# Bostanabad-Research-Group/GP-Plus

Measured on AMD Instinct MI355X. Metric: MLL evals/sec (fwd+grad), NxN exact GP, N=20k d=8, higher is better.
Workload: dtype f64; 1 GPU; C2: synthetic Borehole (Sobol seed 0, unique rows, z-scored) N=20000 d=8 fp64, GP_Plus Rough_RBF exact GP at theta1, one replica per GPU (restart-parallel); N=20000, d=8, streams_per_gpu=1

## Files before the change

### gp-plus_amd/_lib.py

```python
from __future__ import annotations

import ctypes
import os
import subprocess
from ctypes import POINTER, c_char_p, c_double, c_int, c_int32, c_int64, c_size_t, c_void_p
from pathlib import Path

import torch

_PKG_DIR = Path(__file__).resolve().parent
_LIB_PATH = _PKG_DIR / "libgpp_hip.so"
_CSRC = _PKG_DIR / "csrc"

_SIGNATURES = {
    "gpp_version": (c_char_p, []),
    "gpp_create": (c_int, [POINTER(c_void_p), c_int]),
    "gpp_destroy": (c_int, [c_void_p]),
    "gpp_set_stream": (c_int, [c_void_p, c_void_p]),
    "gpp_internal_stream": (c_int, [c_void_p, c_int, POINTER(c_void_p)]),
    "gpp_set_option": (c_int, [c_void_p, c_int, c_int]),
    "gpp_workspace_bytes": (c_size_t, [c_void_p, c_int, c_int64, c_int64, c_int, c_int]),
    "gpp_set_workspace": (c_int, [c_void_p, c_void_p, c_size_t]),
    "gpp_kernel_build": (c_int, [c_void_p, c_void_p, c_int64, c_int, c_void_p, c_void_p, c_void_p, c_void_p, c_int,
                                 c_double, c_int, c_int, c_int, c_void_p, c_int64, c_int64, c_int64]),
    "gpp_cross_kernel": (c_int, [c_void_p, c_void_p, c_int64, c_void_p, c_int64, c_int, c_void_p, c_void_p, c_int,
                                 c_int, c_void_p, c_int64]),
    "gpp_potrf": (c_int, [c_void_p, c_void_p, c_int64, c_int64, c_void_p, c_int64, c_void_p]),
    "gpp_potrf_ws": (c_int, [c_void_p, c_void_p, c_int64, c_int64, c_void_p, c_int64, c_void_p, c_int64, c_void_p]),
    "gpp_trtri": (c_int, [c_void_p, c_void_p, c_int64, c_int64, c_void_p, c_int64, c_void_p, c_int64]),
    "gpp_lauum": (c_int, [c_void_p, c_void_p, c_int64, c_int64, c_void_p, c_int64]),
    "gpp_post_cov_train": (c_int, [c_void_p, c_void_p, c_int64, c_int64, c_void_p, c_void_p, c_int, c_void_p, c_double, c_void_p,
                                   c_int64]),
    "gpp_syrk_rows": (c_int, [c_void_p, c_void_p, c_int64, c_void_p, c_int64, c_int64, c_int64, c_int64, c_int64, c_int, c_int]),
    "gpp_gemm_lower_cols": (c_int, [c_void_p, c_void_p, c_int64, c_void_p, c_int64, c_void_p, c_int64, c_int64, c_int64, c_double,
                                    c_double, c_int64, c_int64, c_int, c_int, c_int64, c_int64, c_int]),
    "gpp_shard_list_begin": (c_int, [c_void_p, c_int64, c_int64, c_int, c_int, c_void_p, c_int64, c_void_p, c_void_p, c_int64, c_void_p,
                                     c_void_p, c_void_p, c_void_p, c_int64, c_void_p, c_int, POINTER(c_int)]),
    "gpp_shard_piece_cols": (c_int64, []),
    "gpp_shard_list_gate": (c_int, [c_void_p, c_void_p, c_int, c_int]),
    "gpp_shard_list_signal": (c_int, [c_void_p, c_void_p, c_int, c_int]),
    "gpp_shard_list_end": (c_int, [c_void_p]),
    "gpp_set_comm": (c_int, [c_void_p, c_void_p, c_int, c_int]),
    "gpp_comm_unique_id": (c_int, [c_void_p]),
    "gpp_comm_init_rccl": (c_int, [c_void_p, c_void_p, c_int, c_int]),
    "gpp_shard_buffer_doubles": (c_size_t, [c_int64, c_int64, c_int, c_int, c_int]),
    "gpp_shard_eval": (c_int, [c_void_p, c_int64, c_int64, c_void_p, c_int, c_void_p, c_void_p, c_void_p, c_void_p, c_int, c_int, c_int,
                               c_double, c_int, c_int, c_void_p, POINTER(c_int)]),
    "gpp_push_create": (c_int, [c_int, c_int, c_int, c_int64, POINTER(c_void_p), c_void_p]),
    "gpp_push_connect": (c_int, [c_void_p, c_void_p]),
    "gpp_push_send": (c_int, [c_void_p, c_void_p, c_int64, c_void_p, c_int, c_int, POINTER(c_void_p), POINTER(c_int64), POINTER(c_int64),
                              POINTER(c_int64), POINTER(c_int64), POINTER(c_int64)]),
    "gpp_push_recv": (c_int, [c_void_p, c_void_p, c_int64, c_void_p, c_int, c_int, POINTER(c_void_p), POINTER(c_int64), POINTER(c_int64),
                              POINTER(c_int64), POINTER(c_int64), POINTER(c_int64)]),
    "gpp_push_ack": (c_int, [c_void_p, c_void_p, c_int64]),
    "gpp_push_info": (c_int, [c_void_p, POINTER(c_int64), POINTER(c_int)]),
    "gpp_push_destroy": (c_int, [c_void_p, c_int]),
    "gpp_shard_back_list": (c_int, [c_void_p, c_int64, c_int64, c_int, c_int, c_void_p, c_int64, c_void_p, c_void_p, c_int64, c_void_p,
                                    c_void_p, c_int, POINTER(c_int)]),
    "gpp_trmv_lower_cols": (c_int, [c_void_p, c_void_p, c_int64, c_int64, c_void_p, c_void_p, c_int64, c_int, c_int, c_int, c_int]),
    "gpp_mll_scalars": (c_int, [c_void_p, c_void_p, c_int64, c_int64, c_void_p, c_void_p]),
    "gpp_grad_reduce_cols": (c_int, [c_void_p, c_void_p, c_int64, c_int, c_void_p, c_void_p, c_void_p, c_int, c_int, c_int,
                                     c_void_p, c_void_p, c_int64, c_int, c_int64, c_int, c_int, c_void_p, c_void_p, c_void_p,
                                     c_void_p, c_int]),
    "gpp_lauum_rows": (c_int, [c_void_p, c_void_p, c_int64, c_int64, c_void_p, c_int64, c_int, c_int]),
    "gpp_lauum_rows_range": (c_int, [c_void_p, c_void_p, c_int64, c_int64, c_void_p, c_int64, c_int, c_int, c_int64, c_int64]),
    "gpp_transpose": (c_int, [c_void_p, c_void_p, c_int64, c_int64, c_int64, c_void_p, c_int64]),
    "gpp_mll_reduce": (c_int, [c_void_p, c_void_p, c_int64, c_void_p, c_int64, c_int64, c_void_p, c_void_p, c_void_p]),
    "gpp_alpha": (c_int, [c_void_p, c_void_p, c_int64, c_int64, c_void_p, c_void_p]),
    "gpp_grad_reduce": (c_int, [c_void_p, c_void_p, c_int64, c_int, c_void_p, c_void_p, c_void_p, c_int, c_int, c_int,
                                c_void_p, c_void_p, c_int64, c_int, c_void_p, c_void_p, c_void_p, c_void_p]),
    "gpp_grad_reduce_rows": (c_int, [c_void_p, c_void_p, c_int64, c_int, c_void_p, c_void_p, c_void_p, c_int, c_int, c_int,
                                     c_void_p, c_void_p, c_int64, c_int, c_int64, c_int, c_int, c_void_p, c_void_p, c_void_p,
                                     c_void_p]),
    "gpp_predict": (c_int, [c_void_p, c_void_p, c_int64, c_int64, c_void_p, c_void_p, c_int64, c_int64, c_void_p,
                            c_void_p, c_int64, c_void_p, c_void_p]),
    "gpp_predict_tn": (c_int, [c_void_p, c_void_p, c_int64, c_int64, c_void_p, c_void_p, c_int64, c_int64, c_void_p,
                               c_void_p, c_int64, c_void_p, c_void_p]),
    "gpp_cross_grad": (c_int, [c_void_p, c_void_p, c_int64, c_void_p, c_int64, c_int, c_void_p, c_void_p, c_int, c_int, c_void_p,
                               c_void_p, c_void_p, c_void_p, c_int64, c_void_p, c_int, c_void_p, c_int, c_void_p, c_void_p]),
    "gpp_gemm": (c_int, [c_void_p, c_int, c_int, c_int64, c_int64, c_int64, c_double, c_void_p, c_int64, c_void_p,
                         c_int64, c_double, c_void_p, c_int64, c_int, c_int, c_int, c_int, c_int]),
    "gpp_gemm_batched": (c_int, [c_void_p, c_int, c_int, c_int64, c_int64, c_int64, c_double, c_void_p, c_int64, c_int64,
                                 c_void_p, c_int64, c_int64, c_double, c_void_p, c_int64, c_int64, c_int, c_int, c_int, c_int,
                                 c_int, c_int]),
    "gpp_kernel_build_batched": (c_int, [c_void_p, c_void_p, c_int64, c_int64, c_int, c_void_p, c_void_p, c_void_p, c_void_p, c_int,
                                         c_double, c_int, c_int, c_int, c_void_p, c_int64, c_int64, c_int]),
    "gpp_potrf_batched": (c_int, [c_void_p, c_void_p, c_int64, c_int64, c_int64, c_void_p, c_int64, c_int64, c_void_p, c_int]),
    "gpp_trtri_batched": (c_int, [c_void_p, c_void_p, c_int64, c_int64, c_int64, c_void_p, c_int64, c_int64, c_void_p, c_int64,
                                  c_int64, c_int]),
    "gpp_lauum_batched": (c_int, [c_void_p, c_void_p, c_int64, c_int64, c_int64, c_void_p, c_int64, c_int64, c_int]),
    "gpp_mll_reduce_batched": (c_int, [c_void_p, c_void_p, c_int64, c_int64, c_void_p, c_int64, c_int64, c_int64, c_void_p,
                                       c_void_p, c_int64, c_void_p, c_int]),
    "gpp_alpha_batched": (c_int, [c_void_p, c_void_p, c_int64, c_int64, c_int64, c_void_p, c_void_p, c_int64, c_int]),
    "gpp_grad_reduce_batched": (c_int, [c_void_p, c_void_p, c_int64, c_int64, c_int, c_void_p, c_void_p, c_void_p, c_int, c_int,
                                        c_int, c_void_p, c_int64, c_void_p, c_int64, c_int64, c_int, c_void_p, c_void_p, c_void_p,
                                        c_void_p, c_int]),
}

_lib = None


class GppError(RuntimeError):
    """A libgpp_hip call returned a non-zero status."""


def build(force: bool = False) -> Path:
    if force:
        subprocess.run(["make", "-C", str(_CSRC), "clean"], check=True, capture_output=True)
    proc = subprocess.run(["make", "-C", str(_CSRC), "-j4"], capture_output=True, text=True)
    if proc.returncode != 0:
        raise RuntimeError("building libgpp_hip.so failed:\n" + proc.stdout + proc.stderr)
    return _LIB_PATH


def load() -> ctypes.CDLL:
    global _lib
    if _lib is not None:
        return _lib
    if not _LIB_PATH.exists():
        raise GppError(
            f"{_LIB_PATH} not found: the HIP extension is required (build it with "
            f"`make -C {_CSRC}` or `python -c 'import __graft_entry__ as g; g.build()'`); there is no CPU fallback."
        )
    lib = ctypes.CDLL(os.fspath(_LIB_PATH))
    for name, (restype, argtypes) in _SIGNATURES.items():
        fn = getattr(lib, name)
        fn.restype = restype
        fn.argtypes = argtypes
    _lib = lib
    return lib


def exported_symbols() -> list:
    return sorted(_SIGNATURES)


def check(status: int, what: str) -> None:
    if status == 0:
        return
    if status < 0:
        raise GppError(f"{what}: bad argument #{-status}")
    raise GppError(f"{what}: HIP runtime error {status - 1000}")
```

### gp-plus_amd/backend.py

```python
from __future__ import annotations

import atexit
import ctypes
import os
import threading
import weakref
from typing import Dict, Optional, Tuple

import torch

from . import _lib, settings
from ._lib import GppError, check

KIND_RBF, KIND_MATERN32, KIND_MATERN52 = 0, 1, 2
UPLO_FULL, UPLO_LOWER, UPLO_UPPER = 0, 1, 2
OPT_COOP_PANEL, OPT_PANEL_FAULT, OPT_PANEL_TIMEOUT_MS, OPT_EXEC_SCHED, OPT_DAG_SCHED = 1, 2, 3, 4, 5
OP_MLL_EVAL, OP_PREDICT, OP_PREDICT_GRAD = 0, 1, 2
MAX_FEATURES = 64


def _check_features(D: int) -> None:
    if D < 1 or D > MAX_FEATURES:
        raise GppError(f"the covariance kernels take 1..{MAX_FEATURES} feature columns per point (got {D})")

_contexts: Dict[Tuple[int, int], "GppContext"] = {}
_contexts_lock = threading.Lock()


def _ptr(t: Optional[torch.Tensor]) -> Optional[int]:
    return None if t is None else t.data_ptr()


def _need(t: torch.Tensor, dtype, name: str) -> None:
    if not t.is_cuda:
        raise GppError(f"{name} must live on the GPU (got {t.device}); libgpp_hip has no CPU path")
    if t.dtype != dtype:
        raise GppError(f"{name} must be {dtype} (got {t.dtype})")
    if not t.is_contiguous() and t.dim() == 1:
        raise GppError(f"{name} must be contiguous")


INFO_PANEL_TIMEOUT = 1 << 30
INFO_EXEC_TIMEOUT = (1 << 30) | (1 << 29)


def check_status(info: int) -> None:
    if info >= INFO_PANEL_TIMEOUT:
        what = "an executor launch" if info & (1 << 29) else "the cooperative panel kernel"
        raise GppError(f"gpp_potrf: {what} timed out waiting for one of its work-groups (another kernel holding the stream's CUs "
                       "for seconds, or a caller-supplied CU-masked stream with fewer CUs than the launch assumed); "
                       "GPP_COOP_PANEL=0 selects the leaf-step factorisation, GPP_DAG_SCHED=0 the launch-per-product one")


def panel_timed_out(ctx: "GppContext", info: int) -> bool:
    if info < INFO_PANEL_TIMEOUT:
        return False
    import warnings

    ms = info & 0xFFFFF
    if info & (1 << 29):
        if not ctx.dag_sched:
            check_status(info)
        warnings.warn(f"libgpp_hip: an executor launch timed out after {ms} ms (another tenant of this GPU held part of its CUs, or "
                      "dispatches are serialised); this context now factors with one launch per product", RuntimeWarning)
        ctx.set_option(OPT_DAG_SCHED, 0)
        return True
    if not ctx.coop_panel:
        check_status(info)
    warnings.warn(f"libgpp_hip: a cooperative panel launch timed out after {ms} ms (another tenant of this GPU held part "
                  "of its CUs); this context now factors with leaf-step launches", RuntimeWarning)
    ctx.set_option(OPT_COOP_PANEL, 0)
    return True


def square_buffer(n: int, device) -> torch.Tensor:
    ld = max(16, (n + 15) // 16 * 16)
    return torch.empty((n, ld), dtype=torch.float64, device=device)[:, :n]


def _ld(m: torch.Tensor) -> int:
    if m.dim() != 2 or m.stride(1) != 1:
        raise GppError("matrix must be 2-D with unit column stride")
    return m.stride(0) if m.shape[0] > 1 else max(m.shape[1], m.stride(0))


def _on_own_device(fn):
    import functools

    @functools.wraps(fn)
    def wrapper(self, *args, **kwargs):
        if torch.cuda.current_device() == self.index:
            return fn(self, *args, **kwargs)
        with torch.cuda.device(self.index):
            return fn(self, *args, **kwargs)

    return wrapper


class GppContext:
    def __init__(self, device: torch.device):
        if device.type != "cuda":
            raise GppError("GppContext needs a cuda (HIP) device; there is no CPU fallback")
        if not torch.cuda.is_available():
            raise GppError("no GPU visible to PyTorch: the HIP path cannot run")
        self.lib = _lib.load()
        self.device = device
        self.index = device.index if device.index is not None else torch.cuda.current_device()
        h = ctypes.c_void_p()
        with torch.cuda.device(self.index):
            check(self.lib.gpp_create(ctypes.byref(h), self.index), "gpp_create")
        self.h = h
        self.coop_panel = settings.ENV_COOP_PANEL
        self.dag_sched = settings.ENV_DAG_SCHED
        if any(os.environ.get(v, "0") not in ("", "0") for v in ("HIP_LAUNCH_BLOCKING", "AMD_SERIALIZE_KERNEL", "CUDA_LAUNCH_BLOCKING")):
            self.set_option(OPT_DAG_SCHED, 0)
        self._ws: Optional[torch.Tensor] = None

    def _stream(self) -> None:
        s = torch.cuda.current_stream(self.index).cuda_stream
        check(self.lib.gpp_set_stream(self.h, ctypes.c_void_p(s)), "gpp_set_stream")

    def set_option(self, option: int, value: int) -> None:
        check(self.lib.gpp_set_option(self.h, int(option), int(value)), "gpp_set_option")
        if option == OPT_COOP_PANEL:
            self.coop_panel = bool(value)
        elif option in (OPT_DAG_SCHED, OPT_EXEC_SCHED):
            self.dag_sched = bool(value)

    @_on_own_device
    def internal_streams(self):
        if getattr(self, "_istreams", None) is None:
            out = []
            for which in (0, 1, 2):
                p = ctypes.c_void_p()
                check(self.lib.gpp_internal_stream(self.h, which, ctypes.byref(p)), "gpp_internal_stream")
                out.append(torch.cuda.ExternalStream(p.value, device=self.device))
            self._istreams = tuple(out)
        return self._istreams

    @_on_own_device
    def ensure_workspace(self, op: int, N: int, M: int, D: int, S: int) -> None:
        need = int(self.lib.gpp_workspace_bytes(self.h, op, N, M, D, S))
        if self._ws is None or self._ws.numel() < need:
            self._ws = torch.empty(need, dtype=torch.uint8, device=self.device)
            check(self.lib.gpp_set_workspace(self.h, self._ws.data_ptr(), self._ws.numel()), "gpp_set_workspace")

    def _check_groups(self, grp: torch.Tensor, N: int, S: int) -> None:
        _need(grp, torch.int32, "grp")
        if grp.numel() != N:
            raise GppError(f"noise-group index has {grp.numel()} entries for {N} points (stale fidel_indices?)")
        seen = getattr(self, "_grp_ok", None)
        if seen is None or seen[0]() is not grp or seen[1:] != (grp._version, N, S):
            lo, hi = int(grp.min()), int(grp.max())
            if lo < 0 or hi >= max(S, 1):
                raise GppError(f"noise-group index out of range: values in [{lo}, {hi}] for {S} noise levels")
            self._grp_ok = (weakref.ref(grp), grp._version, N, S)

    @_on_own_device
    def kernel_build(self, U, w, sf2, tau, grp, out, *, jitter=0.0, kind=KIND_RBF, d_split=0, uplo=UPLO_FULL,
                     row0=0, nrows=None):
        N, D = U.shape
        _check_features(D)
        for t, n in ((U, "U"), (w, "w"), (sf2, "sf2"), (out, "Ky")):
            _need(t, torch.float64, n)
        if tau is not None:
            _need(tau, torch.float64, "tau")
        S = 0 if tau is None else tau.numel()
        if grp is not None:
            self._check_groups(grp, N, S)
        if not U.is_contiguous():
            raise GppError("U must be contiguous")
        self._stream()
        check(self.lib.gpp_kernel_build(self.h, U.data_ptr(), N, D, w.data_ptr(), sf2.data_ptr(), _ptr(tau), _ptr(grp), S,
                                        float(jitter), kind, d_split, uplo, out.data_ptr(), _ld(out), row0,
                                        N - row0 if nrows is None else nrows), "gpp_kernel_build")
        return out

    @_on_own_device
    def cross_kernel(self, Ua, Ub, w, sf2, out, *, kind=KIND_RBF, d_split=0):
        _check_features(Ua.shape[1])
        for t, n in ((Ua, "Ua"), (Ub, "Ub"), (w, "w"), (sf2, "sf2"), (out, "Kab")):
            _need(t, torch.float64, n)
        if not (Ua.is_contiguous() and Ub.is_contiguous()):
            raise GppError("Ua/Ub must be contiguous")
        self._stream()
        check(self.lib.gpp_cross_kernel(self.h, Ua.data_ptr(), Ua.shape[0], Ub.data_ptr(), Ub.shape[0], Ua.shape[1],
                                        w.data_ptr(), sf2.data_ptr(), kind, d_split, out.data_ptr(), _ld(out)),
              "gpp_cross_kernel")
        return out

    @_on_own_device
    def potrf(self, A, Linv, info, T=None):
        _need(A, torch.float64, "A"); _need(Linv, torch.float64, "Linv"); _need(info, torch.int32, "info")
        self._stream()
        if T is None:
            check(self.lib.gpp_potrf(self.h, A.data_ptr(), A.shape[0], _ld(A), Linv.data_ptr(), _ld(Linv), info.data_ptr()),
                  "gpp_potrf")
        else:
            check(self.lib.gpp_potrf_ws(self.h, A.data_ptr(), A.shape[0], _ld(A), Linv.data_ptr(), _ld(Linv), T.data_ptr(),
                                        _ld(T), info.data_ptr()), "gpp_potrf_ws")

    @_on_own_device
    def trtri(self, U, Linv, T):
        self._stream()
        check(self.lib.gpp_trtri(self.h, U.data_ptr(), U.shape[0], _ld(U), Linv.data_ptr(), _ld(Linv), T.data_ptr(), _ld(T)),
              "gpp_trtri")

    @_on_own_device
    def lauum(self, Linv, Kinv):
        self._stream()
        check(self.lib.gpp_lauum(self.h, Linv.data_ptr(), Linv.shape[0], _ld(Linv), Kinv.data_ptr(), _ld(Kinv)), "gpp_lauum")

    @_on_own_device
    def post_cov_train(self, Kinv, tau, grp, d, out, *, jitter=0.0):
        N = Kinv.shape[0]
        for t, n in ((Kinv, "Kinv"), (tau, "tau"), (out, "A")):
            _need(t, torch.float64, n)
        if d is not None:
            _need(d, torch.float64, "d")
            if d.numel() != N or not d.is_contiguous():
                raise GppError(f"d must be a contiguous vector of {N} doubles")
        if grp is not None:
            self._check_groups(grp, N, tau.numel())
        if out.shape[0] != N or out.shape[1] != N:
            raise GppError("post_cov_train: shapes do not match")
        self._stream()
        check(self.lib.gpp_post_cov_train(self.h, Kinv.data_ptr(), N, _ld(Kinv), tau.data_ptr(), _ptr(grp), tau.numel(), _ptr(d),
                                          float(jitter), out.data_ptr(), _ld(out)), "gpp_post_cov_train")
        return out

    @_on_own_device
    def syrk_rows(self, Urow, C, nb, first_block, rank, nranks):
        self._stream()
        check(self.lib.gpp_syrk_rows(self.h, Urow.data_ptr(), _ld(Urow), C.data_ptr(), _ld(C), C.shape[0], Urow.shape[0], nb,
                                     first_block, rank, nranks), "gpp_syrk_rows")

    @_on_own_device
    def shard_list_begin(self, N, nb, rank, nranks, A, Kc, Lc, D, W, info, workers=0) -> bool:
        self._stream()
        used = ctypes.c_int(0)
        check(self.lib.gpp_shard_list_begin(self.h, N, nb, rank, nranks, A.data_ptr(), _ld(A), Kc.data_ptr(), Lc.data_ptr(), _ld(Kc),
                                            D.data_ptr(), W[0].data_ptr(), W[1].data_ptr(), W[2].data_ptr(), _ld(W[0]),
                                            info.data_ptr(), int(workers), ctypes.byref(used)), "gpp_shard_list_begin")
        return bool(used.value)

    def shard_messages(self, N: int, nb: int, k: int):
        o, o2 = k * nb, min((k + 2) * nb, N)
        W = int(self.lib.gpp_shard_piece_cols()) or N
        return [(o, o2)] + [(c, min(c + W, N)) for c in range(o2, N, W)]

    @_on_own_device
    def shard_list_gate(self, stream, tail: int, k: int) -> None:
        check(self.lib.gpp_shard_list_gate(self.h, ctypes.c_void_p(stream.cuda_stream), int(tail), k), "gpp_shard_list_gate")

    @_on_own_device
    def shard_list_signal(self, stream, tail: int, k: int) -> None:
        check(self.lib.gpp_shard_list_signal(self.h, ctypes.c_void_p(stream.cuda_stream), int(tail), k), "gpp_shard_list_signal")

    @_on_own_device
    def shard_list_end(self) -> None:
        self._stream()
        check(self.lib.gpp_shard_list_end(self.h), "gpp_shard_list_end")

    @_on_own_device
    def shard_back_list(self, N, nb, rank, nranks, A, Kc, Lc, D, info, workers=0) -> bool:
        self._stream()
        used = ctypes.c_int(0)
        check(self.lib.gpp_shard_back_list(self.h, N, nb, rank, nranks, A.data_ptr(), _ld(A), Kc.data_ptr(), Lc.data_ptr(), _ld(Kc),
                                           D.data_ptr(), info.data_ptr(), int(workers), ctypes.byref(used)), "gpp_shard_back_list")
        return bool(used.value)

    @_on_own_device
    def gemm_lower_cols(self, A, B, C, alpha, beta, nb, first_block, rank, nranks, row0=0, row1=None, compact=False):
        M, K = A.shape[1], A.shape[0]
        if compact:
            if B.shape[0] != K or C.shape[0] != M:
                raise GppError("gemm_lower_cols: shapes do not match")
        elif A.shape != B.shape or C.shape[0] != C.shape[1] or C.shape[0] != M:
            raise GppError("gemm_lower_cols: shapes do not match")
        self._stream()
        check(self.lib.gpp_gemm_lower_cols(self.h, A.data_ptr(), _ld(A), B.data_ptr(), _ld(B), C.data_ptr(), _ld(C), M,
                                           K, float(alpha), float(beta), nb, first_block, rank, nranks, row0,
                                           M if row1 is None else row1, 1 if compact else 0),
              "gpp_gemm_lower_cols")

    @_on_own_device
    def trmv_lower_cols(self, T, x, y, nb, rank, nranks, trans=False, compact=False):
        for t, n in ((x, "x"), (y, "y")):
            _need(t, torch.float64, n)
        if trans:
            self.ensure_workspace(OP_MLL_EVAL, T.shape[0], 0, 1, 1)
        self._stream()
        check(self.lib.gpp_trmv_lower_cols(self.h, T.data_ptr(), _ld(T), T.shape[0], x.data_ptr(), y.data_ptr(), nb, rank, nranks,
                                           1 if trans else 0, 1 if compact else 0), "gpp_trmv_lower_cols")

    @_on_own_device
    def mll_scalars(self, U, z, out3):
        self._stream()
        check(self.lib.gpp_mll_scalars(self.h, U.data_ptr(), _ld(U), U.shape[0], z.data_ptr(), out3.data_ptr()), "gpp_mll_scalars")

    @_on_own_device
    def lauum_rows(self, Linv, Kinv, rank, nranks):
        self._stream()
        check(self.lib.gpp_lauum_rows(self.h, Linv.data_ptr(), Linv.shape[0], _ld(Linv), Kinv.data_ptr(), _ld(Kinv), rank, nranks),
              "gpp_lauum_rows")

    @_on_own_device
    def lauum_rows_range(self, Linv, Kinv, rank, nranks, row0, row1):
        self._stream()
        check(self.lib.gpp_lauum_rows_range(self.h, Linv.data_ptr(), Linv.shape[0], _ld(Linv), Kinv.data_ptr(), _ld(Kinv), rank,
                                            nranks, row0, row1), "gpp_lauum_rows_range")

    @_on_own_device
    def transpose(self, src, dst):
        if src.shape[0] != dst.shape[1] or src.shape[1] != dst.shape[0]:
            raise GppError("transpose: shapes do not match")
        self._stream()
        check(self.lib.gpp_transpose(self.h, src.data_ptr(), src.stride(0), src.shape[0], src.shape[1], dst.data_ptr(), dst.stride(0)),
              "gpp_transpose")

    @_on_own_device
    def mll_reduce(self, L, Linv, r, z, out3):
        for t, n in ((r, "r"), (z, "z"), (out3, "out3")):
            _need(t, torch.float64, n)
        self._stream()
        check(self.lib.gpp_mll_reduce(self.h, L.data_ptr(), _ld(L), Linv.data_ptr(), _ld(Linv), L.shape[0], r.data_ptr(),
                                      z.data_ptr(), out3.data_ptr()), "gpp_mll_reduce")

    @_on_own_device
    def alpha(self, Linv, z, alpha):
        N = Linv.shape[0]
        self._stream()
        check(self.lib.gpp_alpha(self.h, Linv.data_ptr(), _ld(Linv), N, z.data_ptr(), alpha.data_ptr()), "gpp_alpha")

    @_on_own_device
    def grad_reduce(self, U, w, sf2, grp, S, alpha, Kinv, dU, g_w, g_sf2, g_tau, g_U, *, kind=KIND_RBF, d_split=0):
        N, D = U.shape
        if grp is not None:
            self._check_groups(grp, N, S)
        self.ensure_workspace(OP_MLL_EVAL, N, 0, D, S)
        self._stream()
        check(self.lib.gpp_grad_reduce(self.h, U.data_ptr(), N, D, w.data_ptr(), sf2.data_ptr(), _ptr(grp), S, kind,
                                       d_split, alpha.data_ptr(), Kinv.data_ptr(), _ld(Kinv), dU, g_w.data_ptr(),
                                       g_sf2.data_ptr(), g_tau.data_ptr(), _ptr(g_U)), "gpp_grad_reduce")

    @_on_own_device
    def grad_reduce_rows(self, U, w, sf2, grp, S, alpha, Kinv, dU, nb, rank, nranks, g_w, g_sf2, g_tau, g_U, *,
                         kind=KIND_RBF, d_split=0):
        N, D = U.shape
        if grp is not None:
            self._check_groups(grp, N, S)
        self.ensure_workspace(OP_MLL_EVAL, N, 0, D, S)
        self._stream()
        check(self.lib.gpp_grad_reduce_rows(self.h, U.data_ptr(), N, D, w.data_ptr(), sf2.data_ptr(), _ptr(grp), S, kind,
                                            d_split, alpha.data_ptr(), Kinv.data_ptr(), _ld(Kinv), dU, nb, rank, nranks,
                                            g_w.data_ptr(), g_sf2.data_ptr(), g_tau.data_ptr(), _ptr(g_U)),
              "gpp_grad_reduce_rows")

    @_on_own_device
    def grad_reduce_cols(self, U, w, sf2, grp, S, alpha, Kinv, dU, nb, rank, nranks, g_w, g_sf2, g_tau, g_U, *,
                         kind=KIND_RBF, d_split=0, compact=False):
        N, D = U.shape
        if grp is not None:
            self._check_groups(grp, N, S)
# ... 167 lines not shown
```

### gp-plus_amd/csrc/gpp_api.hip

```cpp
#include "../../include/gpp.h"
#include "gpp_internal.h"

#include <algorithm>
#include <cmath>
#include <cstdio>
#include <cstdlib>
#include <cstring>
#include <new>

const GppEnv& gpp_env() {
  static const GppEnv env = [] {
    auto num = [](const char* name, long long unset) { const char* v = getenv(name); return v ? atoll(v) : unset; };
    GppEnv e;
    e.coop_panel = num("GPP_COOP_PANEL", 1) != 0;
    e.dag_sched = num("GPP_DAG_SCHED", 1) != 0;
    e.dag_phased = num("GPP_DAG_PHASED", 0) != 0;
    e.shard_list = num("GPP_SHARD_LIST", 1) != 0;
    e.shard_workers = (int)num("GPP_SHARD_WORKERS", 0);
    e.shard_fill = (int)num("GPP_SHARD_FILL", -1);
    e.shard_timeout_ms = num("GPP_SHARD_TIMEOUT_MS", 60000);
    const int64_t cols = num("GPP_SHARD_PIECE_COLS", 8192);
    e.shard_piece_cols = cols <= 0 ? (int64_t)0 : std::max<int64_t>(GPP_TILE, cols / GPP_TILE * GPP_TILE);
    e.sharded_force_collectives = num("GPP_SHARDED_FORCE_COLLECTIVES", 0) != 0;
    e.exec_verbose = getenv("GPP_EXEC_VERBOSE") != nullptr;
// ... 313 lines not shown
      HIP_TRY(hipStreamWaitEvent(cf, R_prev, 0));
      const int64_t t128 = ((nb + 127) / 128) * ((o + 127) / 128);
      HIP_TRY(trtri_level(cf, cm.A, cm.ld, cm.Li, cm.ldi, T, ldt, 0, o + nb, o, [](int64_t) { return false; }, 1, 0, 0, 0,
                          t128 < 640 ? 64 : 0, D));
    }
    if (rem == 0) {
      if (be_wait) HIP_TRY(hipStreamWaitEvent(cu.s, be_wait, 0));
      break;
    }
    const int64_t nb2 = std::min(bh, rem), rest = rem - nb2;
    auto row_solve = [&](int64_t c0, int64_t nc) -> hipError_t {
      if (!T) return trsm_rec(cu, c0, nc, o, nb);
      GemmArgs gt = mk(cm.Li + o * cm.ldi + o, cm.ldi, cm.A + o * cm.ld + c0, cm.ld, T + o * ldt + c0, ldt, nb, nc, nb, 1.0,
                       0.0);
      gt.a_mask = 1; gt.khi_mode = 1;
      gt.row_reverse = 1;
      HIP_TRY(gpp_launch_gemm(cu.s, 2, gt, 1));
      return hipMemcpy2DAsync(cm.A + o * cm.ld + c0, cm.ld * sizeof(double), T + o * ldt + c0, ldt * sizeof(double),
                              nc * sizeof(double), nb, hipMemcpyDeviceToDevice, cu.s);
    };
    const double* Urow = cm.A + o * cm.ld;
    HIP_TRY(row_solve(o + nb, nb2));
    GemmArgs g = mk(Urow + (o + nb), cm.ld, Urow + (o + nb), cm.ld, cm.A + (o + nb) * cm.ld + (o + nb), cm.ld, nb2, nb2, nb,
                    -1.0, 1.0);
    g.c_lower = 2;
    HIP_TRY(gpp_launch_gemm(cu.s, 2, g, 1));
    hipEvent_t S = next_event(h);
    HIP_TRY(hipEventRecord(S, cu.s));
    if (rest > 0) HIP_TRY(row_solve(o + nb + nb2, rest));
    hipEvent_t R = nullptr;
    if (border) {
      R = next_event(h);
      HIP_TRY(hipEventRecord(R, cu.s));
    }
    const bool merge_upd = nb2 % NBLK == 0;
    if (rest > 0 && !merge_upd) {
      GemmArgs g2 = mk(Urow + (o + nb), cm.ld, Urow + (o + nb + nb2), cm.ld, cm.A + (o + nb) * cm.ld + (o + nb + nb2), cm.ld,
                       nb2, rest, nb, -1.0, 1.0);
      HIP_TRY(gpp_launch_gemm(cu.s, 2, g2, 1));
    }
    HIP_TRY(hipStreamWaitEvent(cp.s, S, 0));
    if (be_wait) {
      HIP_TRY(hipStreamWaitEvent(cu.s, be_wait, 0));
      be_wait = nullptr;
    }
    if (rest > 0 && merge_upd) {
      GemmArgs g3 = mk(Urow + (o + nb), cm.ld, Urow + (o + nb), cm.ld, cm.A + (o + nb) * cm.ld + (o + nb), cm.ld, rem, rem, nb,
                       -1.0, 1.0);
      g3.c_lower = 2;
      g3.skip_lead = (int)nb2;
      int64_t rA = ((SPLIT_ELEMS / rem + NBLK - 1) / NBLK) * NBLK;
      rA = std::max(rA, nb2);
      if (split_upd && rem - rA >= 2048) {
        pend.rows_ready = next_event(h);
        HIP_TRY(hipEventRecord(pend.rows_ready, cu.s));
        GemmArgs a2 = mk(Urow + (o + nb), cm.ld, Urow + (o + nb + rA), cm.ld, cm.A + (o + nb) * cm.ld + (o + nb + rA), cm.ld,
                         rA, rem - rA, nb, -1.0, 1.0);
        HIP_TRY(gpp_launch_gemm(cu.s, 2, a2, 1, NBLK, NBLK));
        GemmArgs a1 = g3;
        a1.M = a1.N = (int)rA;
        HIP_TRY(hipStreamWaitEvent(cf, pend.rows_ready, 0));
        HIP_TRY(gpp_launch_gemm(cf, 2, a1, 1, NBLK, NBLK));
        hipEvent_t A1 = next_event(h);
        HIP_TRY(hipEventRecord(A1, cf));
        HIP_TRY(hipStreamWaitEvent(cu.s, A1, 0));
        pend.g = mk(Urow + (o + nb + rA), cm.ld, Urow + (o + nb + rA), cm.ld, cm.A + (o + nb + rA) * cm.ld + (o + nb + rA),
                    cm.ld, rem - rA, rem - rA, nb, -1.0, 1.0);
        pend.g.c_lower = 2;
        pend.rows_masked = rA;
        pend.on = true;
      } else {
        HIP_TRY(gpp_launch_gemm(cu.s, 2, g3, 1, NBLK, NBLK));
      }
    } else if (rest > 0) {
      GemmArgs g3 = mk(Urow + (o + nb + nb2), cm.ld, Urow + (o + nb + nb2), cm.ld,
                       cm.A + (o + nb + nb2) * cm.ld + (o + nb + nb2), cm.ld, rest, rest, nb, -1.0, 1.0);
      g3.c_lower = 2;
      HIP_TRY(gpp_launch_gemm(cu.s, 2, g3, 1));
    }
    R_prev = R;
  }
  if (pend.on) return hipErrorUnknown;
  hipEvent_t E = next_event(h);
  HIP_TRY(hipEventRecord(E, cu.s));
  HIP_TRY(hipStreamWaitEvent(cm.s, E, 0));
  if (border) {
    hipEvent_t F = next_event(h);
    HIP_TRY(hipEventRecord(F, cf));
    HIP_TRY(hipStreamWaitEvent(cm.s, F, 0));
    h->inv_nblocks = 1;
    h->inv_o[0] = 0;
    h->inv_n[0] = N;
  }
  return hipSuccess;
}

void dag_note_inverted(gpp_handle_s* h, const DagPlan* P, int64_t N) {
  h->inv_nblocks = 0;
  if (P->inv_rows > 0) {
    h->inv_o[0] = 0;
    h->inv_n[0] = std::min(P->inv_rows, N);
    h->inv_nblocks = 1;
  }
  for (int b = 0; b < P->B && h->inv_nblocks < 128; ++b) {
    const int64_t o = (int64_t)P->tb[b] * NBLK, rows = std::min<int64_t>((int64_t)P->tb[b + 1] * NBLK, N) - o;
    if (o < P->inv_rows) continue;
    h->inv_o[h->inv_nblocks] = o;
    h->inv_n[h->inv_nblocks] = rows;
    ++h->inv_nblocks;
  }
}

hipError_t dag_abort(gpp_handle_s* h, const DagPlan* P) {
  if (!h->full_stream || !P || !P->d_counters) return hipErrorInvalidValue;
  HIP_TRY(gpp_launch_fill_i32(h->full_stream, P->d_counters, 1, 1));
  return hipStreamSynchronize(h->full_stream);
}

inline int dag_fuse(int64_t N) { return N >= 14336 ? 4 : N >= 11264 ? 2 : 1; }

struct PlanKey {
  int64_t N, nb, ld, ldi, ldt;
  int flags;
  int64_t inv_rows;
  int rank, nranks, workers;
};
template <typename Make>
DagPlan* dag_plan_cached(gpp_handle_s* h, const PlanKey& k, Make make) {
  DagPlan* P = nullptr;
  int lru = 0;
  for (int i = 0; i < GPP_DAG_PLANS; ++i) {
    DagPlan* q = h->dag_plans[i];
    if (q && q->N == k.N && q->nb == k.nb && q->ld == k.ld && q->ldi == k.ldi && q->ldt == k.ldt && q->flags == k.flags &&
        q->inv_rows == k.inv_rows && q->rank == k.rank && q->nranks == k.nranks && q->workers == k.workers)
      P = q;
    if (!q) lru = i;
    else if (h->dag_plans[lru] && q->stamp < h->dag_plans[lru]->stamp) lru = i;
  }
  if (!P) {
    P = make();
    if (!P) return nullptr;
    if (h->dag_plans[lru]) gpp_dag_free(h->dag_plans[lru]);
    h->dag_plans[lru] = P;
  }
  P->stamp = ++h->dag_clock;
  return P;
}

constexpr int64_t DAG_MIN_N = 6912;
constexpr int64_t DAG_MAX_N = 65536;
constexpr int64_t DAG_INV_MAX_N = 19456;
constexpr int64_t DAG_NB = 1024;

hipError_t potrf_dag(gpp_handle_s* h, const Ctx& cm, int64_t N, double* T, int64_t ldt, bool* used) {
  *used = false;
  if (!gpp_env().dag_sched || !h->dag_sched || !h->coop_panel || !T || N < DAG_MIN_N || N > DAG_MAX_N) return hipSuccess;
  HIP_TRY(ensure_streams(h));
  if (h->cu_split != 1) return hipSuccess;
  const int64_t nb = DAG_NB;
  if (!panel_fits(h, nb) || !panel_fits(h, nb + 256)) return hipSuccess;
  int64_t inv_rows = N;
  if (N > DAG_INV_MAX_N) {
    inv_rows = 0;
    for (int64_t r = 2 * nb; r <= (int64_t)(0.42 * (double)N); r *= 2) inv_rows = r;
  }
  const int flags = inv_rows > 0 ? DAG_INV : 0;
  DagPlan* P = dag_plan_cached(h, PlanKey{N, nb, cm.ld, cm.ldi, ldt, flags, inv_rows, 0, 1, 0}, [&]() -> DagPlan* {
    DagTuning tune = gpp_dag_default_tuning();
    tune.workers = 2 * (h->ncu - h->panel_cus);
    tune.fill = 2 * h->panel_cus;
    tune.inv_rows = inv_rows;
    tune.fuse = dag_fuse(N);
    DagPlan* Q = gpp_dag_plan(N, nb, cm.ld, cm.ldi, ldt, 0, flags, tune);
    if (!Q) return nullptr;
    for (int b = 0; b < Q->B; ++b) {
      const int64_t rows = std::min<int64_t>((int64_t)Q->tb[b + 1] * NBLK, N) - (int64_t)Q->tb[b] * NBLK;
      if (!panel_fits(h, rows)) {
        gpp_dag_free(Q);
        return nullptr;
      }
    }
    if (gpp_dag_upload(Q) != hipSuccess) {
      (void)hipGetLastError();
      gpp_dag_free(Q);
      h->dag_sched = 0;
      return nullptr;
    }
    return Q;
  });
  if (!P) return hipSuccess;
  Ctx cp = cm, cu = cm;
  cp.s = h->panel_stream;
  cu.s = h->upd_stream;
  HIP_TRY(gpp_launch_fill_i32(cm.s, P->d_counters, P->ncounters, 0));
  DagBases bases{{reinterpret_cast<char*>(cm.A), reinterpret_cast<char*>(cm.Li), reinterpret_cast<char*>(T), nullptr}};
  HIP_TRY(gpp_launch_dag_bind(cm.s, P->d_groups, P->d_groups_abs, (int)P->groups.size(), bases));
  hipEvent_t ev = next_event(h);
  HIP_TRY(hipEventRecord(ev, cm.s));
  HIP_TRY(hipStreamWaitEvent(cp.s, ev, 0));
  HIP_TRY(hipStreamWaitEvent(cu.s, ev, 0));
  const long long budget = (long long)(h->panel_timeout_ms > 0 ? h->panel_timeout_ms : 500) * 100000 * 4;
  DagLaunch dl{};
  dl.groups = P->d_groups_abs; dl.tasks = P->d_tasks; dl.ntasks = (int)P->tasks.size();
  dl.counters = P->d_counters; dl.info = cm.info; dl.budget = budget;
  dl.max_tasks = 0; dl.quit_id = -1; dl.quit_val = 0; dl.ticket_limit = 0;
  dl.trace = P->d_trace; dl.tag = 0;
  if (gpp_env().dag_phased) {
    const int wgs = 2 * h->ncu;
    for (int b = 0; b < P->B; ++b) {
      const int64_t o = (int64_t)P->tb[b] * NBLK, rows = std::min<int64_t>((int64_t)P->tb[b + 1] * NBLK, N) - o;
      HIP_TRY(launch_panel(h, cm, o, rows, std::min(64, h->ncu)));
      HIP_TRY(gpp_launch_exec_signal(cm.s, P->d_counters, P->c_pd + b));
      DagLaunch pl = dl;
      pl.ticket_limit = b + 1 < P->B ? P->level_first[b + 1] : 0;
      pl.tag = b;
      if (b + 1 == P->B || pl.ticket_limit > 0) HIP_TRY(gpp_launch_dag(cm.s, wgs, pl));
    }
    HIP_TRY(hipEventRecord(P->last_use, cm.s));
    dag_note_inverted(h, P, N);
    *used = true;
    return hipSuccess;
  }
  HIP_TRY(gpp_launch_dag(cu.s, 2 * (h->ncu - h->panel_cus), dl));
  auto enqueue_panel_stream = [&]() -> hipError_t {
    for (const DagPlan::Op& op : P->stream_ops) {
      const int64_t o = op.kind < 3 ? (int64_t)P->tb[op.arg] * NBLK : 0;
      if (op.kind == 0) {
        HIP_TRY(gpp_launch_exec_gate(cp.s, P->d_counters, P->c_g1d + op.arg, P->gate_target[op.arg], cm.info, budget));
      } else if (op.kind == 1) {
        const int64_t rows = std::min<int64_t>((int64_t)P->tb[op.arg + 1] * NBLK, N) - o;
        HIP_TRY(launch_panel(h, cp, o, rows, h->panel_cus));
      } else if (op.kind == 2) {
        HIP_TRY(gpp_launch_exec_signal(cp.s, P->d_counters, P->c_pd + op.arg));
      } else {
        DagLaunch fl = dl;
        fl.max_tasks = op.arg;
        fl.quit_id = op.n >= 0 ? P->c_g1d + op.n : -1;
        fl.quit_val = 1;
        fl.ticket_limit = op.lim;
        fl.tag = op.n >= 0 ? op.n : P->B;
        HIP_TRY(gpp_launch_dag(cp.s, 2 * h->panel_cus, fl));
      }
    }
    return hipSuccess;
  };
  const hipError_t perr = enqueue_panel_stream();
  if (perr != hipSuccess) {
    (void)hipGetLastError();
    (void)dag_abort(h, P);
  }
  hipEvent_t E = next_event(h), F = next_event(h);
  HIP_TRY(hipEventRecord(E, cu.s));
  HIP_TRY(hipEventRecord(F, cp.s));
  HIP_TRY(hipStreamWaitEvent(cm.s, E, 0));
  HIP_TRY(hipStreamWaitEvent(cm.s, F, 0));
  HIP_TRY(hipEventRecord(P->last_use, cm.s));
  if (perr != hipSuccess) return perr;
  dag_note_inverted(h, P, N);
  *used = true;
  return hipSuccess;
}

inline int64_t owned_cols(int64_t N, int64_t nb, int rank, int nranks) {
  const int64_t nblk = (N + nb - 1) / nb;
  int64_t cols = 0;
  for (int64_t b = rank; b < nblk; b += nranks) cols += std::min(nb, N - b * nb);
  return cols;
}

int check_mat(const void* p, int64_t ld, int64_t n, int argi) {
  if (!p) return -argi;
  if (!aligned16(p) || (ld & 1) || ld < n) return -(argi + 1);
  return 0;
}

}

extern "C" {

#ifndef GPP_SRC_HASH
#define GPP_SRC_HASH "unknown"
#endif
const char* gpp_version(void) { return "gpp_hip 0.3 (gfx950, fp64 MFMA) src " GPP_SRC_HASH; }

#ifdef GPP_PANEL_STAMP
int gpp_debug_panel_flags(gpp_handle_t h, int* out, int nints, int* next_slot) {
  if (next_slot) *next_slot = h->panel_next % GPP_PANEL_RING;
  return (int)hipMemcpy(out, h->panel_flags, (size_t)nints * sizeof(int), hipMemcpyDeviceToHost);
}
#endif

static DagPlan* dag_mru(gpp_handle_t h) {
  DagPlan* P = nullptr;
  if (h)
    for (int i = 0; i < GPP_DAG_PLANS; ++i)
      if (h->dag_plans[i] && (!P || h->dag_plans[i]->stamp > P->stamp)) P = h->dag_plans[i];
  return P;
}
int gpp_debug_dag_info(gpp_handle_t h, int64_t* info8) {
  const DagPlan* P = dag_mru(h);
  if (!P) return -1;
  info8[8] = P->inv_rows;
  info8[9] = P->N;
  info8[0] = (int64_t)P->tasks.size(); info8[1] = (int64_t)P->groups.size(); info8[2] = P->B; info8[3] = P->nt;
  info8[4] = P->ncounters; info8[5] = (int64_t)(P->sim_ms * 1000.0); info8[6] = (int64_t)(P->sim_busy * 1000.0); info8[7] = P->flags;
  return 0;
}
int gpp_debug_dag_counters(gpp_handle_t h, int* out, int nmax) {
  DagPlan* P = dag_mru(h);
  if (!P || !P->d_counters) return -1;
  if (hipDeviceSynchronize() != hipSuccess) return 1;
  std::vector<int> c(P->ncounters);
  if (hipMemcpy(c.data(), P->d_counters, c.size() * sizeof(int), hipMemcpyDeviceToHost) != hipSuccess) return 2;
  int n = 0;
  auto put = [&](int v) { if (n < nmax) out[n++] = v; };
  put(c[0]); put(c[1]); put(P->B);
  for (int b = 0; b < P->B; ++b) put(c[P->c_pd + b]);
  for (int b = 0; b < P->B; ++b) put(c[P->c_g1d + b]);
  if (P->flags & DAG_SHARD) {
    for (int b = 0; b < P->B; ++b) put(c[P->c_cph + b]);
    for (int b = 0; b < P->B; ++b) put(c[P->c_cpt + b * P->GP]);
    for (int b = 0; b < P->B; ++b) put(c[P->c_art + b * P->GP]);
  }
  return n;
}
int gpp_debug_dag_trace(gpp_handle_t h, int on) {
  DagPlan* P = dag_mru(h);
  if (!P) return -1;
  if (hipDeviceSynchronize() != hipSuccess) return 1;
  if (on && !P->d_trace) {
    if (hipMalloc(&P->d_trace, 4 * P->tasks.size() * sizeof(unsigned long long)) != hipSuccess) return 2;
    (void)hipMemset(P->d_trace, 0, 4 * P->tasks.size() * sizeof(unsigned long long));
  } else if (!on && P->d_trace) {
    (void)hipFree(P->d_trace);
    P->d_trace = nullptr;
  }
  return 0;
}
int gpp_debug_dag_fetch(gpp_handle_t h, void* tasks, void* trace) {
  const DagPlan* P = dag_mru(h);
  if (!P) return -1;
  if (hipDeviceSynchronize() != hipSuccess) return 1;
  if (tasks) memcpy(tasks, P->tasks.data(), P->tasks.size() * sizeof(DagTask));
  if (trace) {
    if (!P->d_trace) return 2;
    if (hipMemcpy(trace, P->d_trace, 4 * P->tasks.size() * sizeof(unsigned long long), hipMemcpyDeviceToHost) != hipSuccess) return 3;
  }
  return 0;
}

int gpp_create(gpp_handle_t* out, int device) {
  if (!out) return -1;
  int ndev = 0;
  hipError_t e = hipGetDeviceCount(&ndev);
  if (e != hipSuccess) return rc(e);
  if (device < 0 || device >= ndev) return -2;
  e = hipSetDevice(device);
  if (e != hipSuccess) return rc(e);
  gpp_handle_s* h = new (std::nothrow) gpp_handle_s();
  if (!h) return rc(hipErrorOutOfMemory);
  h->device = device;
  h->stream = nullptr;
  h->ws = nullptr;
  h->ws_bytes = 0;
  h->panel_stream = nullptr;
  h->upd_stream = nullptr;
  h->fill_stream = nullptr;
  h->full_stream = nullptr;
  h->cu_split = -1;
  h->panel_cus = 0;
  h->n_events = 0;
  h->ev_next = 0;
  h->inv_N = 0;
  h->inv_nblocks = 0;
  h->panel_flags = nullptr;
  h->panel_next = 0;
  h->coop_panel = gpp_env().coop_panel ? 1 : 0;
  h->panel_fault = 0;
  h->panel_timeout_ms = 500;
  for (int i = 0; i < GPP_DAG_PLANS; ++i) h->dag_plans[i] = nullptr;
  h->shard_cur = nullptr;
  h->shard_info = nullptr;
  h->shard_ready = nullptr;
  h->dag_clock = 0;
  h->dag_sched = 1;
  h->ncu = 0;
  if (hipDeviceGetAttribute(&h->ncu, hipDeviceAttributeMultiprocessorCount, device) != hipSuccess || h->ncu < 2) {
    (void)hipGetLastError();
    h->ncu = 0;
  }
  h->cap_next = 0;
  h->handoff = nullptr;
  if (hipMalloc(reinterpret_cast<void**>(&h->panel_flags), (GPP_PANEL_RING + GPP_PANEL_CAP_RING) * gpp_panel_flag_bytes()) != hipSuccess ||
      hipMemset(h->panel_flags, 0, (GPP_PANEL_RING + GPP_PANEL_CAP_RING) * gpp_panel_flag_bytes()) != hipSuccess) {
    (void)hipGetLastError();
    if (h->panel_flags) (void)hipFree(h->panel_flags);
    h->panel_flags = nullptr;
  }
  *out = h;
  return 0;
}

int gpp_destroy(gpp_handle_t h) {
  if (!h) return -1;
  for (hipStream_t s : {h->panel_stream, h->upd_stream, h->fill_stream, h->full_stream})
    if (s) (void)hipStreamSynchronize(s);
  if (h->full_stream) (void)hipStreamDestroy(h->full_stream);
  if (h->fill_stream) (void)hipStreamDestroy(h->fill_stream);
  if (h->upd_stream) (void)hipStreamDestroy(h->upd_stream);
  if (h->panel_stream) (void)hipStreamDestroy(h->panel_stream);
  for (int i = 0; i < h->n_events; ++i) (void)hipEventDestroy(h->events[i]);
  if (h->handoff) (void)hipEventDestroy(h->handoff);
  if (h->shard_ready) (void)hipEventDestroy(h->shard_ready);
  if (h->panel_flags) (void)hipFree(h->panel_flags);
  for (int i = 0; i < GPP_DAG_PLANS; ++i)
    if (h->dag_plans[i]) gpp_dag_free(h->dag_plans[i]);
  gpp_shard_release_comm(h);
  delete h;
  return 0;
}

int gpp_set_stream(gpp_handle_t h, void* stream) {
  if (!h) return -1;
  hipStream_t s = reinterpret_cast<hipStream_t>(stream);
  if (s != h->stream) {
    hipStreamCaptureStatus a = hipStreamCaptureStatusNone, b = hipStreamCaptureStatusNone;
    if (hipStreamIsCapturing(h->stream, &a) != hipSuccess || hipStreamIsCapturing(s, &b) != hipSuccess) {
      (void)hipGetLastError();
      a = b = hipStreamCaptureStatusActive;
    }
    auto internal = [&](hipStream_t q) { return q && (q == h->panel_stream || q == h->upd_stream || q == h->fill_stream || q == h->full_stream); };
    if (a == hipStreamCaptureStatusNone && b == hipStreamCaptureStatusNone && !internal(s) && !internal(h->stream)) {
      if (!h->handoff) GPP_TRY(hipEventCreateWithFlags(&h->handoff, hipEventDisableTiming));
      GPP_TRY(hipEventRecord(h->handoff, h->stream));
      GPP_TRY(hipStreamWaitEvent(s, h->handoff, 0));
    }
    h->stream = s;
  }
  return 0;
}

int gpp_set_option(gpp_handle_t h, int option, int value) {
  if (!h) return -1;
  if (option == GPP_OPT_COOP_PANEL) h->coop_panel = value ? 1 : 0;
  else if (option == GPP_OPT_PANEL_FAULT) h->panel_fault = value ? 1 : 0;
  else if (option == GPP_OPT_DAG_SCHED || option == GPP_OPT_EXEC_SCHED) h->dag_sched = value ? 1 : 0;
  else if (option == GPP_OPT_PANEL_TIMEOUT_MS) {
    if (value < 1 || value > 60000) return -3;
    h->panel_timeout_ms = value;
  } else return -2;
  return 0;
// ... 61 lines not shown
  hipStream_t sm = h->stream, sp = h->panel_stream, su = h->upd_stream;
  GPP_TRY(gpp_launch_fill_i32(sm, P->d_counters, P->ncounters, 0));
  DagBases bases{{reinterpret_cast<char*>(A), reinterpret_cast<char*>(Kc), reinterpret_cast<char*>(Lc), reinterpret_cast<char*>(D),
                  reinterpret_cast<char*>(W0), reinterpret_cast<char*>(W1), reinterpret_cast<char*>(W2), nullptr}};
  GPP_TRY(gpp_launch_dag_bind(sm, P->d_groups, P->d_groups_abs, (int)P->groups.size(), bases));
  if (!h->shard_ready) GPP_TRY(hipEventCreateWithFlags(&h->shard_ready, hipEventDisableTiming));
  hipEvent_t ev = h->shard_ready;
  GPP_TRY(hipEventRecord(ev, sm));
  GPP_TRY(hipStreamWaitEvent(sp, ev, 0));
  GPP_TRY(hipStreamWaitEvent(su, ev, 0));
  const long long budget = shard_budget(h);
  DagLaunch dl{};
  dl.groups = P->d_groups_abs; dl.tasks = P->d_tasks; dl.ntasks = (int)P->tasks.size();
  dl.counters = P->d_counters; dl.info = info; dl.budget = budget;
  dl.max_tasks = 0; dl.quit_id = -1; dl.quit_val = 0; dl.ticket_limit = 0;
  dl.trace = P->d_trace; dl.tag = 0;
  if (dl.ntasks > 0) GPP_TRY(gpp_launch_dag(su, nworkers, dl));
  Ctx cp{sp, A, ld, D, nb, info};
  auto enqueue_panel_stream = [&]() -> int {
    for (const DagPlan::Op& op : P->stream_ops) {
      const int b = op.arg;
      const int64_t o = (int64_t)b * nb, rows = std::min(nb, N - o);
      if (op.kind == 0) {
        GPP_TRY(gpp_launch_exec_gate(sp, P->d_counters, P->c_g1d + b, P->gate_target[b], info, budget));
      } else if (op.kind == 1) {
        Ctx cb = cp;
        cb.A = A + o * ld + o;
        cb.Li = D + (int64_t)b * nb * nb;
        GPP_TRY(launch_panel_at(h, cb, o, rows, h->panel_cus));
      } else if (op.kind == 2) {
        GPP_TRY(gpp_launch_exec_signal(sp, P->d_counters, P->c_pd + b));
      } else {
        DagLaunch fl = dl;
        fl.max_tasks = op.arg;
        fl.quit_id = op.n >= 0 ? P->c_g1d + op.n : -1;
        fl.quit_val = 1;
        fl.ticket_limit = op.lim;
        fl.tag = op.n >= 0 ? op.n : P->B;
        GPP_TRY(gpp_launch_dag(sp, std::max(P->fill, 1), fl));
      }
    }
    return 0;
  };
  const int erc = enqueue_panel_stream();
  h->shard_cur = P;
  h->shard_info = info;
  if (erc != 0) {
    (void)hipGetLastError();
    (void)dag_abort(h, P);
    return erc;
  }
  *used = 1;
  return 0;
}

static int shard_pieces(const DagPlan* P, int k) {
  const int hi = P->tb[std::min(k + 2, P->B)];
  return hi >= P->nt ? 0 : (P->nt - hi + P->piece_tiles - 1) / P->piece_tiles;
}
int gpp_shard_list_gate(gpp_handle_t h, void* stream, int tail, int k) {
  if (!h || !h->shard_cur) return -1;
  const DagPlan* P = h->shard_cur;
  if (k < 0 || k >= P->B || k % P->nranks != P->rank) return -4;
  if (tail < 0 || tail > shard_pieces(P, k)) return -3;
  hipStream_t s = reinterpret_cast<hipStream_t>(stream);
  const long long budget = shard_budget(h);
  GPP_TRY(hipStreamWaitEvent(s, h->shard_ready, 0));
  GPP_TRY(gpp_launch_exec_gate(s, P->d_counters, P->c_pd + k, 1, h->shard_info, budget));
  const int piece = k * P->GP + tail - 1;
  const int target = tail ? P->cpt_target[piece] : P->cph_target[k];
  if (target > 0) GPP_TRY(gpp_launch_exec_gate(s, P->d_counters, tail ? P->c_cpt + piece : P->c_cph + k, target, h->shard_info, budget));
  return 0;
}

int gpp_shard_list_signal(gpp_handle_t h, void* stream, int tail, int k) {
  if (!h || !h->shard_cur) return -1;
  const DagPlan* P = h->shard_cur;
  if (k < 0 || k >= P->B || k % P->nranks == P->rank) return -4;
  if (tail < 0 || tail > shard_pieces(P, k)) return -3;
  GPP_TRY(hipStreamWaitEvent(reinterpret_cast<hipStream_t>(stream), h->shard_ready, 0));
  return rc(gpp_launch_exec_signal(reinterpret_cast<hipStream_t>(stream), P->d_counters, tail ? P->c_art + k * P->GP + tail - 1 : P->c_pd + k));
}

int gpp_shard_list_end(gpp_handle_t h) {
  if (!h || !h->shard_cur) return -1;
  DagPlan* P = h->shard_cur;
  h->shard_cur = nullptr;
  hipEvent_t E = next_event(h), F = next_event(h);
  GPP_TRY(hipEventRecord(E, h->upd_stream));
  GPP_TRY(hipEventRecord(F, h->panel_stream));
  GPP_TRY(hipStreamWaitEvent(h->stream, E, 0));
  GPP_TRY(hipStreamWaitEvent(h->stream, F, 0));
  GPP_TRY(hipEventRecord(P->last_use, h->stream));
  return 0;
}

int gpp_shard_back_list(gpp_handle_t h, int64_t N, int64_t nb, int rank, int nranks, const double* A, int64_t ld, double* Kc, double* Lc,
                        int64_t ldc, const double* D, int32_t* info, int workers, int* used) {
  if (!h) return -1;
  if (!used) return -14;
  *used = 0;
  if (N < 2 || nb < 128 || nb % 128 != 0) return -2;
  if (rank < 0 || nranks < 1 || rank >= nranks) return -4;
  if (int e = check_mat(A, ld, N, 6)) return e;
  if (!Kc || !aligned16(Kc)) return -8;
  if (!Lc || !aligned16(Lc)) return -9;
  const int64_t wc = ((N + nb - 1) / nb - rank + nranks - 1) / nranks * nb;
  if ((ldc & 1) || ldc < wc) return -10;
  if (!D || !aligned16(D)) return -11;
  if (!info) return -12;
  const GppEnv& env = gpp_env();
  if (!env.shard_list || !h->dag_sched || N < SHARD_LIST_MIN_N || N > DAG_MAX_N || h->shard_cur) return 0;
  if (workers <= 0 && env.shard_workers > 0) workers = 2 * env.shard_workers;
  GPP_TRY(ensure_streams(h));
  const int flags = DAG_SHARD | DAG_BACK;
  const int nworkers = workers > 0 ? workers : 2 * h->ncu;
  DagPlan* P = dag_plan_cached(h, PlanKey{N, nb, ld, ldc, ld, flags, 0, rank, nranks, workers}, [&]() -> DagPlan* {
    DagTuning tune = gpp_dag_default_tuning();
    tune.workers = nworkers;
    tune.fill = 0;
    tune.inv_rows = 0;
    tune.fuse = dag_fuse(N);
    DagPlan* Q = gpp_dag_plan(N, nb, ld, ldc, ld, 0, flags, tune, rank, nranks);
    if (!Q) return nullptr;
    Q->workers = workers;
    if (Q->tasks.empty() || gpp_dag_upload(Q) != hipSuccess) {
      (void)hipGetLastError();
      gpp_dag_free(Q);
      return nullptr;
    }
    return Q;
  });
  if (!P) return 0;
  hipStream_t sm = h->stream;
  GPP_TRY(gpp_launch_fill_i32(sm, P->d_counters, P->ncounters, 0));
  DagBases bases{{const_cast<char*>(reinterpret_cast<const char*>(A)), reinterpret_cast<char*>(Kc), reinterpret_cast<char*>(Lc),
                  const_cast<char*>(reinterpret_cast<const char*>(D)), nullptr, nullptr, nullptr, nullptr}};
  GPP_TRY(gpp_launch_dag_bind(sm, P->d_groups, P->d_groups_abs, (int)P->groups.size(), bases));
  DagLaunch dl{};
  dl.groups = P->d_groups_abs; dl.tasks = P->d_tasks; dl.ntasks = (int)P->tasks.size();
  dl.counters = P->d_counters; dl.info = info;
  dl.budget = shard_budget(h);
  dl.max_tasks = 0; dl.quit_id = -1; dl.quit_val = 0; dl.ticket_limit = 0;
  dl.trace = P->d_trace; dl.tag = 0;
  GPP_TRY(gpp_launch_dag(sm, nworkers, dl));
  GPP_TRY(hipEventRecord(P->last_use, sm));
  *used = 1;
  return 0;
}

size_t gpp_workspace_bytes(gpp_handle_t h, int op, int64_t N, int64_t M, int D, int S) {
  (void)h;
  if (op == GPP_OP_MLL_EVAL) {
    return std::max(gpp_grad_ws_bytes(N, D, S, D), gpp_trmv_t_ws_bytes(N)) + 256;
  }
  if (op == GPP_OP_PREDICT) return 256;
  if (op == GPP_OP_PREDICT_GRAD) return gpp_pgrad_ws_bytes(M, N, D, D, S) + 256;
  return 0;
}

int gpp_set_workspace(gpp_handle_t h, void* ws, size_t bytes) {
  if (!h) return -1;
  if (ws && !aligned16(ws)) return -2;
  h->ws = ws;
  h->ws_bytes = bytes;
  return 0;
}

int gpp_kernel_build(gpp_handle_t h, const double* U, int64_t N, int D, const double* w, const double* sf2,
                     const double* tau, const int32_t* grp, int S, double jitter, int kind, int d_split, int uplo,
                     double* Ky, int64_t ld, int64_t row0, int64_t nrows) {
  if (!h) return -1;
  if (!U) return -2;
  if (N < 0) return -3;
  if (D < 1 || D > 64) return -4;
  if (!w) return -5;
  if (!sf2) return -6;
  if (tau && S < 1) return -9;
  if (kind < 0 || kind > 2) return -11;
  if (d_split < 0 || d_split > D) return -12;
  if (uplo != GPP_UPLO_FULL && uplo != GPP_UPLO_LOWER && uplo != GPP_UPLO_UPPER) return -13;
  if (!Ky) return -14;
  if (ld < N) return -15;
  if (row0 < 0 || nrows < 0 || row0 + nrows > N || (row0 % 64) != 0) return -16;
  if (uplo == GPP_UPLO_UPPER && (row0 != 0 || nrows != N)) return -16;
  GPP_TRY(gpp_launch_kernel_build(h->stream, U, N, D, w, sf2, tau, grp, S, jitter, kind, d_split, uplo, Ky, ld, row0, nrows));
  return 0;
}

int gpp_cross_kernel(gpp_handle_t h, const double* Ua, int64_t Ma, const double* Ub, int64_t Nb, int D, const double* w,
                     const double* sf2, int kind, int d_split, double* Kab, int64_t ld) {
  if (!h) return -1;
  if (!Ua) return -2;
  if (Ma < 0) return -3;
  if (!Ub) return -4;
  if (Nb < 0) return -5;
  if (D < 1 || D > 64) return -6;
  if (!w) return -7;
  if (!sf2) return -8;
  if (kind < 0 || kind > 2) return -9;
  if (d_split < 0 || d_split > D) return -10;
  if (!Kab) return -11;
  if (ld < Nb) return -12;
  GPP_TRY(gpp_launch_cross_kernel(h->stream, Ua, Ma, Ub, Nb, D, w, sf2, kind, d_split, Kab, ld));
  return 0;
}

int gpp_potrf_ws(gpp_handle_t h, double* A, int64_t N, int64_t ld, double* Linv, int64_t ldi, double* T, int64_t ldt,
                 int32_t* info_dev) {
  if (!h) return -1;
  if (N < 0) return -3;
  if (int r = check_mat(A, ld, N, 2)) return r;
  if (int r = check_mat(Linv, ldi, N, 5)) return r;
  if (T) {
    if (int r = check_mat(T, ldt, N, 7)) return r;
  }
  if (!info_dev) return -9;
  GPP_TRY(gpp_launch_fill_i32(h->stream, info_dev, 1, 0));
  Ctx c{h->stream, A, ld, Linv, ldi, info_dev};
  h->inv_N = N;
  h->inv_nblocks = 0;
  const int64_t la_min = T ? BORDER_MIN_N : 6 * LOOKAHEAD_NB;
  bool dag_used = false;
  GPP_TRY(potrf_dag(h, c, N, T, ldt, &dag_used));
  if (dag_used) return 0;
  if (N >= la_min) {
    GPP_TRY(potrf_lookahead(h, c, N, LOOKAHEAD_NB, T, ldt));
  } else if (panel_fits(h, N)) {
    int wgs = h->ncu;
    if (h->cu_split == 1 && h->stream == h->panel_stream) wgs = h->panel_cus;
    else if (h->cu_split == 1 && (h->stream == h->upd_stream || h->stream == h->fill_stream)) wgs = h->ncu - h->panel_cus;
    else if (h->stream) {
      uint32_t mask[32] = {0};
      if (hipExtStreamGetCUMask(h->stream, 32, mask) == hipSuccess) {
        int cus = 0;
        for (int c = 0; c < h->ncu && c < 1024; ++c) cus += (mask[c >> 5] >> (c & 31)) & 1u;
        if (cus >= 2 && cus < wgs) wgs = cus;
      } else {
        (void)hipGetLastError();
      }
    }
    GPP_TRY(launch_panel(h, c, 0, N, wgs));
    h->inv_nblocks = 1;
    h->inv_o[0] = 0;
    h->inv_n[0] = N;
  } else {
    GPP_TRY(potrf_rec(c, 0, N));
  }
  return 0;
}

int gpp_potrf(gpp_handle_t h, double* A, int64_t N, int64_t ld, double* Linv, int64_t ldi, int32_t* info_dev) {
  const int r = gpp_potrf_ws(h, A, N, ld, Linv, ldi, nullptr, 0, info_dev);
  return r == -9 ? -7 : r;
}

int gpp_trtri(gpp_handle_t h, const double* U, int64_t N, int64_t ld, double* Linv, int64_t ldi, double* T, int64_t ldt) {
  if (!h) return -1;
  if (N < 0) return -3;
  if (int r = check_mat(U, ld, N, 2)) return r;
  if (int r = check_mat(Linv, ldi, N, 5)) return r;
  if (int r = check_mat(T, ldt, N, 7)) return r;
  const bool have = (h->inv_N == N && h->inv_nblocks > 0);
  for (int64_t s = NBLK; s < N; s *= 2) {
    auto skip = [&](int64_t b) {
      if (!have) return false;
      for (int i = 0; i < h->inv_nblocks; ++i)
        if (b >= h->inv_o[i] && b + 2 * s <= h->inv_o[i] + h->inv_n[i]) return true;
      for (int i = 0; i < h->inv_nblocks; ++i)
        if (b >= h->inv_o[i] && h->inv_o[i] + h->inv_n[i] == N && b + s < N) return true;
      return false;
    };
    GPP_TRY(trtri_level(h->stream, U, ld, Linv, ldi, T, ldt, 0, N, s, skip));
  }
  h->inv_N = 0;
  return 0;
}

int gpp_lauum(gpp_handle_t h, const double* Linv, int64_t N, int64_t ldi, double* Kinv, int64_t ldk) {
  if (!h) return -1;
  if (N < 0) return -3;
  if (int r = check_mat(Linv, ldi, N, 2)) return r;
  if (int r = check_mat(Kinv, ldk, N, 5)) return r;
  GemmArgs g = mk(Linv, ldi, Linv, ldi, Kinv, ldk, N, N, N, 1.0, 0.0);
  g.a_mask = 2; g.b_mask = 2; g.klo_mode = 3; g.c_lower = 1; g.tag = 1;
  const int t = N <= 2560 ? 32 : N <= 5120 ? 64 : NBLK;
  GPP_TRY(gpp_launch_gemm(h->stream, 2, g, 1, t, t));
  return 0;
}

int gpp_post_cov_train(gpp_handle_t h, const double* Kinv, int64_t N, int64_t ldk, const double* tau, const int32_t* grp, int S,
                       const double* d, double jitter, double* A, int64_t lda) {
  if (!h) return -1;
  if (N < 0) return -3;
  if (int r = check_mat(Kinv, ldk, N, 2)) return r;
  if (!tau) return -5;
  if (S < 1) return -7;
  if (int r = check_mat(A, lda, N, 10)) return r;
  if (A == Kinv && lda != ldk) return -11;
  GPP_TRY(gpp_launch_post_cov_train(h->stream, Kinv, ldk, N, tau, grp, d, jitter, A, lda));
  return 0;
}

int gpp_lauum_rows(gpp_handle_t h, const double* Linv, int64_t N, int64_t ldi, double* Kinv, int64_t ldk, int rank, int nranks) {
  if (!h) return -1;
  if (N < 0) return -3;
  if (int r = check_mat(Linv, ldi, N, 2)) return r;
  if (int r = check_mat(Kinv, ldk, N, 5)) return r;
  if (nranks < 1 || rank < 0 || rank >= nranks) return -7;
  GemmArgs g = mk(Linv, ldi, Linv, ldi, Kinv, ldk, N, N, N, 1.0, 0.0);
  g.a_mask = 2; g.b_mask = 2; g.klo_mode = 3; g.c_lower = 1; g.tag = 1;
  g.row_mod = nranks; g.row_off = rank;
  GPP_TRY(gpp_launch_gemm(h->stream, 2, g, 1, NBLK, NBLK));
  return 0;
}

int gpp_lauum_rows_range(gpp_handle_t h, const double* Linv, int64_t N, int64_t ldi, double* Kinv, int64_t ldk, int rank,
                         int nranks, int64_t row0, int64_t row1) {
  if (!h) return -1;
  if (N < 0) return -3;
  if (int r = check_mat(Linv, ldi, N, 2)) return r;
  if (int r = check_mat(Kinv, ldk, N, 5)) return r;
  if (nranks < 1 || rank < 0 || rank >= nranks) return -7;
  if (row0 < 0 || row1 < row0 || row1 > N || (row0 % NBLK) != 0) return -9;
  if (row1 == row0) return 0;
  GemmArgs g = mk(Linv, ldi, Linv, ldi, Kinv, ldk, N, N, N, 1.0, 0.0);
  g.a_mask = 2; g.b_mask = 2; g.klo_mode = 3; g.c_lower = 1; g.tag = 1;
  g.row_mod = nranks; g.row_off = rank;
  const int64_t t0 = row0 / NBLK, t1 = (row1 + NBLK - 1) / NBLK;
  auto first_i = [&](int64_t t) { return t <= rank ? (int64_t)0 : (t - rank + nranks - 1) / nranks; };
  g.row_i0 = (int)first_i(t0);
  g.row_i1 = (int)first_i(t1);
  if (g.row_i1 <= g.row_i0) return 0;
  GPP_TRY(gpp_launch_gemm(h->stream, 2, g, 1, NBLK, NBLK));
  return 0;
}

int gpp_transpose(gpp_handle_t h, const double* src, int64_t lds, int64_t rows, int64_t cols, double* dst, int64_t ldd) {
  if (!h) return -1;
  if (!src || lds < cols) return -2;
  if (rows < 0 || cols < 0) return -4;
  if (!dst || ldd < rows) return -6;
  GPP_TRY(gpp_launch_transpose(h->stream, src, lds, rows, cols, dst, ldd));
  return 0;
}

int gpp_syrk_rows(gpp_handle_t h, const double* Urow, int64_t ldu, double* C, int64_t ldc, int64_t Nt, int64_t K, int64_t nb,
                  int64_t first_block, int rank, int nranks) {
  if (!h) return -1;
  if (!Urow || !aligned16(Urow) || (ldu & 1)) return -2;
  if (!C || !aligned16(C) || (ldc & 1)) return -4;
  if (Nt < 0 || K < 0) return -6;
  if (nb < NBLK || nb % NBLK != 0) return -8;
  if (first_block < 0) return -9;
  if (nranks < 1 || rank < 0 || rank >= nranks) return -10;
  if (Nt == 0 || K == 0) return 0;
  GemmArgs g = mk(Urow, ldu, Urow, ldu, C, ldc, Nt, Nt, K, -1.0, 1.0);
  g.c_lower = 2;
  g.own_mod = nranks;
  g.own_bt = (int)(nb / NBLK);
  g.own_off = (int)(((first_block - rank) % nranks + nranks) % nranks);
  GPP_TRY(gpp_launch_gemm(h->stream, 2, g, 1, NBLK, NBLK));
  return 0;
}

int gpp_gemm_lower_cols(gpp_handle_t h, const double* A, int64_t lda, const double* B, int64_t ldb, double* C, int64_t ldc,
                        int64_t M, int64_t K, double alpha, double beta, int64_t nb, int64_t first_block, int rank, int nranks,
                        int64_t row0, int64_t row1, int compact) {
  if (!h) return -1;
  if (!A || !aligned16(A) || (lda & 1)) return -2;
  if (!B || !aligned16(B) || (ldb & 1)) return -4;
  if (!C || !aligned16(C) || (ldc & 1)) return -6;
  if (M < 0 || K < 0) return -8;
  if (nb < NBLK || nb % NBLK != 0) return -12;
  if (first_block < 0) return -13;
  if (nranks < 1 || rank < 0 || rank >= nranks) return -14;
  if (row0 < 0 || row1 < row0 || row1 > M || row0 % NBLK != 0) return -16;
  if (M == 0 || K == 0 || row1 == row0) return 0;
  GemmArgs g = mk(A, lda, B, ldb, C, ldc, M, M, K, alpha, beta);
  g.c_lower = 1;
  g.row_t0 = (int)(row0 / NBLK);
  g.row_t1 = (int)((row1 + NBLK - 1) / NBLK);
  g.own_mod = nranks;
  g.own_bt = (int)(nb / NBLK);
  g.own_off = (int)(((first_block - rank) % nranks + nranks) % nranks);
  g.compact_bc = compact ? 1 : 0;
  GPP_TRY(gpp_launch_gemm(h->stream, 2, g, 1, NBLK, NBLK));
  return 0;
}

int gpp_trmv_lower_cols(gpp_handle_t h, const double* T, int64_t ldt, int64_t N, const double* x, double* y, int64_t nb, int rank,
                        int nranks, int trans, int compact) {
  if (!h) return -1;
  if (N < 0) return -4;
  if (int q = check_mat(T, ldt, compact ? std::min<int64_t>(N, ldt) : N, 2)) return q;
  if (!x || !aligned16(x)) return -5;
  if (!y) return -6;
  if (nb < 64 || nb % 64 != 0) return -7;
  if (nranks < 1 || rank < 0 || rank >= nranks) return -8;
  if (trans != 0 && trans != 1) return -10;
  if (trans && (!h->ws || h->ws_bytes < gpp_trmv_t_ws_bytes(N))) return -1;
  if (compact && nranks >= 1 && rank >= 0 && ldt < owned_cols(N, nb, rank, nranks)) return -3;
  GPP_TRY(gpp_launch_trmv_lower_cols(h->stream, T, ldt, N, x, y, nb, rank, nranks, trans, h->ws, h->ws_bytes, compact));
  return 0;
}

int gpp_mll_scalars(gpp_handle_t h, const double* U, int64_t ld, int64_t N, const double* z, double* out3) {
  if (!h) return -1;
  if (N < 0) return -4;
  if (int q = check_mat(U, ld, N, 2)) return q;
  if (!z) return -5;
  if (!out3) return -6;
  GPP_TRY(gpp_launch_mll_scalars(h->stream, U, ld, N, z, out3));
  return 0;
}

int gpp_mll_reduce(gpp_handle_t h, const double* U, int64_t ld, const double* Linv, int64_t ldi, int64_t N,
                   const double* r, double* z, double* out3) {
  if (!h) return -1;
  if (N < 0) return -6;
  if (int q = check_mat(U, ld, N, 2)) return q;
  if (int q = check_mat(Linv, ldi, N, 4)) return q;
  if (!r || !aligned16(r)) return -7;
  if (!z) return -8;
  if (!out3) return -9;
  GPP_TRY(gpp_launch_trmv_lower(h->stream, Linv, ldi, N, r, z));
  GPP_TRY(gpp_launch_mll_scalars(h->stream, U, ld, N, z, out3));
  return 0;
}

int gpp_alpha(gpp_handle_t h, const double* Linv, int64_t ldi, int64_t N, const double* z, double* alpha) {
  if (!h) return -1;
  if (N < 0) return -4;
  if (int q = check_mat(Linv, ldi, N, 2)) return q;
  if (!z || !aligned16(z)) return -5;
  if (!alpha) return -6;
  GPP_TRY(gpp_launch_trmv_upper(h->stream, Linv, ldi, N, z, alpha));
  return 0;
}

// ... 320 lines not shown
```

### gp-plus_amd/csrc/gpp_build.hip

```cpp
#include "gpp_internal.h"

#include <atomic>

namespace {

constexpr int TB = 64;
constexpr int DMAX = 64;

__device__ __forceinline__ double kfun(double r2_rbf, double r2_mat, int kind, const GppExpConsts& ec) {
  double v = gpp_exp_nonpos(-r2_rbf, ec);
  if (kind == 1) {
    const double r = sqrt(3.0 * 2.0 * r2_mat);
    v *= (1.0 + r) * gpp_exp_nonpos(-r, ec);
  } else if (kind == 2) {
    const double r = sqrt(5.0 * 2.0 * r2_mat);
    v *= (1.0 + r + r * r * (1.0 / 3.0)) * gpp_exp_nonpos(-r, ec);
  }
  return v;
}

template <bool MAT>
__global__ __launch_bounds__(256) void gpp_cov_tile(const double* __restrict__ Ua, int64_t Ma, const double* __restrict__ Ub,
                                                    int64_t Nb, int D, const double* __restrict__ w,
                                                    const double* __restrict__ sf2p, const double* __restrict__ tau,
                                                    const int32_t* __restrict__ grp, double jitter, int kind, int d_split,
                                                    int lower, int add_diag, double* __restrict__ K, int64_t ld,
                                                    int64_t row0, int tiles_n, int64_t tile_row0, int64_t sU, int64_t sK,
                                                    int S) {
  extern __shared__ __attribute__((aligned(16))) double cov_smem[];
  double* sa = cov_smem;
  double* sb = cov_smem + (size_t)D * TB;
  {
    const int64_t b = blockIdx.y;
    Ua += b * sU;
    Ub += b * sU;
    w += b * D;
    sf2p += b;
    if (tau) tau += b * S;
    K += b * sK;
  }
  int64_t ti, tj;
  {
    const int64_t t = blockIdx.x;
    if (lower) {
      const double base = 0.5 * (double)tile_row0 * (double)(tile_row0 + 1);
      int64_t r = (int64_t)((sqrt(8.0 * ((double)t + base) + 1.0) - 1.0) * 0.5);
      while ((r + 1) * (r + 2) / 2 - (int64_t)base <= t) ++r;
      while (r * (r + 1) / 2 - (int64_t)base > t) --r;
      ti = r;
      tj = t - (r * (r + 1) / 2 - (int64_t)base);
      if (lower == 2) {
        const int64_t q = ti;
        ti = tj;
        tj = q;
      }
    } else {
      ti = tile_row0 + t / tiles_n;
      tj = t % tiles_n;
    }
  }
  const int tid = threadIdx.x;
  const int64_t i0 = ti * TB, j0 = tj * TB;

  for (int e = tid; e < D * TB; e += 256) {
    const int d = e / TB, r = e - d * TB;
    const double sw = sqrt(w[d]);
    sa[d * TB + r] = (i0 + r < Ma) ? Ua[(i0 + r) * D + d] * sw : 0.0;
    sb[d * TB + r] = (j0 + r < Nb) ? Ub[(j0 + r) * D + d] * sw : 0.0;
  }
  __syncthreads();

  const int ty = tid >> 4, tx = tid & 15;
  double r2a[4][4], r2b[MAT ? 4 : 1][MAT ? 4 : 1];
#pragma unroll
  for (int a = 0; a < 4; ++a)
#pragma unroll
    for (int b = 0; b < 4; ++b) {
      r2a[a][b] = 0.0;
      if (MAT) r2b[a][b] = 0.0;
    }
  const int dsp = (!MAT || kind == 0) ? D : d_split;
  for (int d = 0; d < D; ++d) {
    typedef double v2d __attribute__((ext_vector_type(2)));
    const v2d a01 = reinterpret_cast<const v2d*>(sa + d * TB + 4 * ty)[0], a23 = reinterpret_cast<const v2d*>(sa + d * TB + 4 * ty)[1];
    const v2d b01 = *reinterpret_cast<const v2d*>(sb + d * TB + 2 * tx), b23 = *reinterpret_cast<const v2d*>(sb + d * TB + 32 + 2 * tx);
    const double ua[4] = {a01.x, a01.y, a23.x, a23.y}, ub[4] = {b01.x, b01.y, b23.x, b23.y};
    if (!MAT || d < dsp) {
#pragma unroll
      for (int a = 0; a < 4; ++a)
#pragma unroll
        for (int b = 0; b < 4; ++b) {
          const double df = ua[a] - ub[b];
          r2a[a][b] = fma(df, df, r2a[a][b]);
        }
    } else if constexpr (MAT) {
#pragma unroll
      for (int a = 0; a < 4; ++a)
#pragma unroll
        for (int b = 0; b < 4; ++b) {
          const double df = ua[a] - ub[b];
          r2b[a][b] = fma(df, df, r2b[a][b]);
        }
    }
  }
  const double sf2 = *sf2p;
  const GppExpConsts ec = gpp_exp_consts();
#pragma unroll
  for (int a = 0; a < 4; ++a) {
    const int64_t i = i0 + 4 * ty + a;
    if (i >= Ma || i < row0) continue;
    double v[4];
#pragma unroll
    for (int b = 0; b < 4; ++b) {
      const int64_t j = j0 + 2 * tx + (b & 1) + ((b >> 1) << 5);
      double x = sf2 * (MAT ? kfun(r2a[a][b], r2b[MAT ? a : 0][MAT ? b : 0], kind, ec) : gpp_exp_nonpos(-r2a[a][b], ec));
      if (add_diag && i == j) x += (tau ? tau[grp ? grp[i] : 0] : 0.0) + jitter;
      v[b] = x;
    }
#pragma unroll
    for (int h = 0; h < 2; ++h) {
      double* out = K + i * ld + j0 + 2 * tx + 32 * h;
      const int64_t jrem = Nb - (j0 + 2 * tx + 32 * h);
      if (jrem >= 2 && ((reinterpret_cast<uintptr_t>(out) & 15) == 0)) {
        typedef double v2d __attribute__((ext_vector_type(2)));
        v2d p0 = {v[2 * h], v[2 * h + 1]};
        *reinterpret_cast<v2d*>(out) = p0;
      } else {
        if (jrem >= 1) out[0] = v[2 * h];
        if (jrem >= 2) out[1] = v[2 * h + 1];
      }
    }
  }
}

}

static hipError_t cov_lds_optin(int D) {
  if ((size_t)2 * D * TB * sizeof(double) <= 48 * 1024) return hipSuccess;
  static std::atomic<bool> done[64];
  int dev = 0;
  hipError_t e = hipGetDevice(&dev);
  if (e != hipSuccess) return e;
  if (dev >= 0 && dev < 64 && done[dev]) return hipSuccess;
  e = hipFuncSetAttribute(reinterpret_cast<const void*>(gpp_cov_tile<false>), hipFuncAttributeMaxDynamicSharedMemorySize,
                          2 * DMAX * TB * (int)sizeof(double));
  if (e == hipSuccess)
    e = hipFuncSetAttribute(reinterpret_cast<const void*>(gpp_cov_tile<true>), hipFuncAttributeMaxDynamicSharedMemorySize,
                            2 * DMAX * TB * (int)sizeof(double));
  if (e == hipSuccess && dev >= 0 && dev < 64) done[dev] = true;
  return e;
}

hipError_t gpp_launch_kernel_build(hipStream_t s, const double* U, int64_t N, int D, const double* w, const double* sf2,
                                   const double* tau, const int32_t* grp, int S, double jitter, int kind, int d_split,
                                   int uplo, double* Ky, int64_t ld, int64_t row0, int64_t nrows, int batch, int64_t sU,
                                   int64_t sK) {
  if (N <= 0 || nrows <= 0 || batch <= 0) return hipSuccess;
  if (D > DMAX) return hipErrorInvalidValue;
  if (hipError_t e = cov_lds_optin(D); e != hipSuccess) return e;
  const int64_t tr0 = row0 / TB;
  const int64_t tr1 = (row0 + nrows + TB - 1) / TB;
  const int tiles_n = (int)((N + TB - 1) / TB);
  int64_t nt;
  if (uplo) nt = tr1 * (tr1 + 1) / 2 - tr0 * (tr0 + 1) / 2;
  else nt = (tr1 - tr0) * tiles_n;
  auto* fn = kind == 0 ? gpp_cov_tile<false> : gpp_cov_tile<true>;
  hipLaunchKernelGGL(fn, dim3((unsigned)nt, (unsigned)batch), dim3(256), (size_t)2 * D * TB * sizeof(double), s, U, row0 + nrows, U, N, D, w, sf2, tau,
                     grp, jitter, kind, d_split, uplo, 1, Ky, ld, row0, tiles_n, tr0, sU, sK, S);
  return hipGetLastError();
}

hipError_t gpp_launch_cross_kernel(hipStream_t s, const double* Ua, int64_t Ma, const double* Ub, int64_t Nb, int D,
                                   const double* w, const double* sf2, int kind, int d_split, double* Kab, int64_t ld) {
  if (Ma <= 0 || Nb <= 0) return hipSuccess;
  if (D > DMAX) return hipErrorInvalidValue;
  if (hipError_t e = cov_lds_optin(D); e != hipSuccess) return e;
  const int tiles_n = (int)((Nb + TB - 1) / TB);
  const int64_t tiles_m = (Ma + TB - 1) / TB;
  auto* fn = kind == 0 ? gpp_cov_tile<false> : gpp_cov_tile<true>;
  hipLaunchKernelGGL(fn, dim3((unsigned)(tiles_m * tiles_n)), dim3(256), (size_t)2 * D * TB * sizeof(double), s, Ua, Ma, Ub, Nb, D, w, sf2,
                     (const double*)nullptr, (const int32_t*)nullptr, 0.0, kind, d_split, 0, 0, Kab, ld, (int64_t)0,
                     tiles_n, (int64_t)0, (int64_t)0, (int64_t)0, 0);
  return hipGetLastError();
}

namespace {

constexpr int PC_T = 128;
constexpr int PC_Q = 64;

__global__ __launch_bounds__(256) void gpp_post_cov_tile(const double* Kinv, int64_t ldk, int64_t N, const double* __restrict__ tau,
                                                         const int32_t* __restrict__ grp, const double* __restrict__ d,
                                                         double jitter, double* A, int64_t lda) {
  __shared__ double s[PC_Q][PC_Q + 1];
  typedef double v2d __attribute__((ext_vector_type(2)));
  int64_t ti, tj;
  {
    const int64_t t = blockIdx.x;
    int64_t r = (int64_t)((sqrt(8.0 * (double)t + 1.0) - 1.0) * 0.5);
    while ((r + 1) * (r + 2) / 2 <= t) ++r;
    while (r * (r + 1) / 2 > t) --r;
    tj = r;
    ti = t - r * (r + 1) / 2;
  }
  const int tid = threadIdx.x;
  const int lc = (tid & 31) * 2, lr = tid >> 5;
  for (int q = 0; q < 4; ++q) {
    const int qa = q >> 1, qb = q & 1;
    if (ti == tj && qa > qb) continue;
    const int64_t i0 = ti * PC_T + qa * PC_Q, j0 = tj * PC_T + qb * PC_Q;
    if (i0 >= N || j0 >= N) continue;
    __syncthreads();
#pragma unroll
    for (int k = 0; k < 8; ++k) {
      const int jr = lr + 8 * k;
      const int64_t j = j0 + jr, i = i0 + lc;
      double x0 = 0.0, x1 = 0.0;
      if (j < N) {
        const double* p = Kinv + j * ldk + i;
        if (i + 1 < N && i + 1 <= j) {
          const v2d v = *reinterpret_cast<const v2d*>(p);
          x0 = v.x;
          x1 = v.y;
        } else {
          if (i < N && i <= j) x0 = p[0];
          if (i + 1 < N && i + 1 <= j) x1 = p[1];
        }
      }
      s[lc][jr] = x0;
      s[lc + 1][jr] = x1;
    }
    __syncthreads();
    const int64_t j = j0 + lc;
    const double tj0 = j < N ? tau[grp ? grp[j] : 0] : 0.0;
    const double tj1 = j + 1 < N ? tau[grp ? grp[j + 1] : 0] : 0.0;
#pragma unroll
    for (int k = 0; k < 8; ++k) {
      const int ir = lr + 8 * k;
      const int64_t i = i0 + ir;
      if (i >= N) continue;
      const double tv = tau[grp ? grp[i] : 0];
      double v0 = -tv * s[ir][lc] * tj0, v1 = -tv * s[ir][lc + 1] * tj1;
      const double dg = tv + (d ? d[i] : 0.0) + jitter;
      if (i == j) v0 += dg;
      if (i == j + 1) v1 += dg;
      double* o = A + i * lda + j;
      const bool w0 = j < N && j >= i, w1 = j + 1 < N && j + 1 >= i;
      if (w0 && w1) {
        const v2d v = {v0, v1};
        *reinterpret_cast<v2d*>(o) = v;
      } else {
        if (w0) o[0] = v0;
        if (w1) o[1] = v1;
      }
    }
  }
}

}

hipError_t gpp_launch_post_cov_train(hipStream_t s, const double* Kinv, int64_t ldk, int64_t N, const double* tau, const int32_t* grp,
                                     const double* d, double jitter, double* A, int64_t lda) {
  if (N <= 0) return hipSuccess;
  const int64_t nt = (N + PC_T - 1) / PC_T;
  hipLaunchKernelGGL(gpp_post_cov_tile, dim3((unsigned)(nt * (nt + 1) / 2)), dim3(256), 0, s, Kinv, ldk, N, tau, grp, d, jitter, A,
                     lda);
  return hipGetLastError();
}
```

### gp-plus_amd/csrc/gpp_gemm.hip

```cpp
#include "../../include/gpp.h"
#include "gpp_internal.h"

#include <algorithm>
#include <atomic>
#include <cstdlib>

typedef double v2d __attribute__((ext_vector_type(2)));
typedef double v4d __attribute__((ext_vector_type(4)));

namespace {

constexpr int BK16 = 16;
constexpr int ldt_mc(int T, int BK = 16) { return BK == 16 ? T + 16 : T + 4; }
constexpr int LDK = BK16 + 2;

__device__ __forceinline__ bool keep_elem(int mask, int k, int row) {
  return (mask == 0) | ((mask == 1) & (k <= row)) | ((mask == 2) & (k >= row));
}

template <int T>
__device__ __forceinline__ unsigned load_kc(const double* __restrict__ P, int64_t ld, int R, int r0, int kb, int kend,
                                            int mask, int tid, v2d (&reg)[T / 32]) {
  unsigned keep = 0;
  const double* ptr[T / 32];
#pragma unroll
  for (int i = 0; i < T / 32; ++i) {
    const int v = tid + 256 * i;
    const int gr = r0 + (v >> 3);
    const int gk = kb + ((v & 7) << 1);
    const bool v0 = (gr < R) & (gk < kend);
    const bool k0 = v0 & keep_elem(mask, gk, gr);
    const bool k1 = v0 & (gk + 1 < kend) & keep_elem(mask, gk + 1, gr);
    keep |= (k0 ? 1u : 0u) << (2 * i);
    keep |= (k1 ? 1u : 0u) << (2 * i + 1);
    ptr[i] = v0 ? P + (int64_t)gr * ld + gk : P;
  }
#pragma unroll
  for (int i = 0; i < T / 32; ++i) reg[i] = *reinterpret_cast<const v2d*>(ptr[i]);
  return keep;
}
template <int T, bool SEL>
__device__ __forceinline__ void store_kc(double* __restrict__ s, int tid, const v2d (&reg)[T / 32], unsigned keep) {
#pragma unroll
  for (int i = 0; i < T / 32; ++i) {
    const int v = tid + 256 * i;
    v2d t = reg[i];
    if (SEL) {
      t.x = ((keep >> (2 * i)) & 1u) ? t.x : 0.0;
      t.y = ((keep >> (2 * i + 1)) & 1u) ? t.y : 0.0;
    }
    *reinterpret_cast<v2d*>(s + (v >> 3) * LDK + ((v & 7) << 1)) = t;
  }
}

template <int T, int BK, int NTH = 256>
__device__ __forceinline__ unsigned load_mc(const double* __restrict__ P, int64_t ld, int R, int r0, int kb, int kend,
                                            int mask, int tid, v2d (&reg)[BK * T / (2 * NTH)], const double* __restrict__ dummy) {
  constexpr int NV = BK * T / (2 * NTH);
  unsigned keep = 0;
  const double* ptr[NV];
#pragma unroll
  for (int i = 0; i < NV; ++i) {
    const int v = tid + NTH * i;
    const int gk = kb + v / (T / 2);
    const int gr = r0 + ((v % (T / 2)) << 1);
    const bool v0 = (gk < kend) & (gr < R);
    const bool k0 = v0 & keep_elem(mask, gk, gr);
    const bool k1 = v0 & (gr + 1 < R) & keep_elem(mask, gk, gr + 1);
    keep |= (k0 ? 1u : 0u) << (2 * i);
    keep |= (k1 ? 1u : 0u) << (2 * i + 1);
    ptr[i] = v0 ? P + (int64_t)gk * ld + gr : dummy;
  }
#pragma unroll
  for (int i = 0; i < NV; ++i) reg[i] = *reinterpret_cast<const v2d*>(ptr[i]);
  return keep;
}
template <int T, int BK, bool SEL, int NTH = 256>
__device__ __forceinline__ void store_mc(double* __restrict__ s, int tid, const v2d (&reg)[BK * T / (2 * NTH)], unsigned keep) {
#pragma unroll
  for (int i = 0; i < BK * T / (2 * NTH); ++i) {
    const int v = tid + NTH * i;
    v2d t = reg[i];
    if (SEL) {
      t.x = ((keep >> (2 * i)) & 1u) ? t.x : 0.0;
      t.y = ((keep >> (2 * i + 1)) & 1u) ? t.y : 0.0;
    }
    *reinterpret_cast<v2d*>(s + (v / (T / 2)) * ldt_mc(T, BK) + ((v % (T / 2)) << 1)) = t;
  }
}

template <int T, int BK>
__device__ __forceinline__ bool chunk_is_interior(int r0, int R, int kb, int kend, int mask) {
  if (r0 + T > R || kb + BK > kend) return false;
  if (mask == 1) return kb + BK - 1 <= r0;
  if (mask == 2) return kb >= r0 + T - 1;
  return true;
}
template <int T, int BK>
__device__ __forceinline__ bool chunk_in_range(int r0, int R, int kb, int kend) {
  return r0 + T <= R && kb + BK <= kend;
}
template <int T, int BK, int NTH = 256>
__device__ __forceinline__ unsigned mask_bits_mc(int r0, int kb, int mask, int tid) {
  unsigned keep = 0;
#pragma unroll
  for (int i = 0; i < BK * T / (2 * NTH); ++i) {
    const int v = tid + NTH * i;
    const int gk = kb + v / (T / 2);
    const int gr = r0 + ((v % (T / 2)) << 1);
    keep |= (keep_elem(mask, gk, gr) ? 1u : 0u) << (2 * i);
    keep |= (keep_elem(mask, gk, gr + 1) ? 1u : 0u) << (2 * i + 1);
  }
  return keep;
}
template <int T, bool KC, int BK, int NTH = 256>
__device__ __forceinline__ void thread_offsets(int64_t ld, int tid, unsigned (&off)[BK * T / (2 * NTH)]) {
#pragma unroll
  for (int i = 0; i < BK * T / (2 * NTH); ++i) {
    const int v = tid + NTH * i;
    if (KC) off[i] = (unsigned)(((int64_t)(v >> 3) * ld + ((v & 7) << 1)) * 8);
    else off[i] = (unsigned)(((int64_t)(v / (T / 2)) * ld + ((v % (T / 2)) << 1)) * 8);
  }
}
template <int NV>
__device__ __forceinline__ void load_fast(const double* __restrict__ ubase, const unsigned (&off)[NV], v2d (&reg)[NV]) {
#pragma unroll
  for (int i = 0; i < NV; ++i)
    reg[i] = *reinterpret_cast<const v2d*>(reinterpret_cast<const char*>(ubase) + off[i]);
}

struct GemmNoHook {
  __device__ __forceinline__ void operator()() const {}
};
template <int VAR, int WTM, int WTN, int TAG, int BK, int NBUF, int WR, class P, class H = GemmNoHook>
__device__ __forceinline__ void gemm_tile(const P& p, const int tm, const int tn, const double* __restrict__ A,
                                          const double* __restrict__ B, double* __restrict__ C, double* C2,
                                          double* __restrict__ smem, H before_epilogue = H()) {
  static_assert(BK == 16 || VAR == 2, "wide K chunks are implemented for row-contiguous (TN) operands only");
  static_assert(BK % 16 == 0 && (NBUF == 1 || NBUF == 2), "bad staging parameters");
  static_assert(WR == 2 || (WR == 4 && VAR == 2 && BK == 16 && NBUF == 2 && WTM == 64 && WTN == 64), "the tall tile is TN only");
  constexpr int NTH = 128 * WR;
  constexpr bool A_KC = (VAR != 2);
  constexpr bool B_KC = (VAR == 0);
  constexpr int TM = WR * WTM, TN = 2 * WTN;
  constexpr int LDA = ldt_mc(TM, BK), LDB = ldt_mc(TN, BK);
  constexpr int TX = TM > TN ? TM : TN;
  constexpr int OPSZ = (BK * ldt_mc(TX, BK) > TX * LDK) ? BK * ldt_mc(TX, BK) : TX * LDK;
  constexpr int OPA = (WR == 2) ? OPSZ : BK * LDA, OPB = (WR == 2) ? OPSZ : BK * LDB;
  constexpr int NVA = BK * TM / (2 * NTH), NVB = BK * TN / (2 * NTH);
  constexpr int RB = WTM / 4, CB = WTN / 16;

  const int tid = threadIdx.x;
  const int wave = tid >> 6, lane = tid & 63;
  const int wm = (wave >> 1) * WTM, wn = (wave & 1) * WTN;
  const int li = lane & 15, lk = lane >> 4;
  const int row0 = tm * TM, col0 = tn * TN;
  const double* __restrict__ Bd = B;
  double* __restrict__ Cd = C;
  if (p.compact_bc) {
    const int b = tn / p.own_bt, q = (b + p.own_off) / p.own_mod;
    const int64_t bias = (int64_t)(q - b) * p.own_bt * TN;
    B += bias;
    C += bias;
  }

  int klo = 0;
  if (p.klo_mode == 1) klo = row0;
  else if (p.klo_mode == 2) klo = col0;
  else if (p.klo_mode == 3) klo = row0 > col0 ? row0 : col0;
  int khi = p.K;
  if (p.khi_mode == 1) khi = min(p.K, row0 + TM);
  else if (p.khi_mode == 2) khi = min(p.K, col0 + TN);
  const int nch = khi > klo ? (khi - klo + BK - 1) / BK : 0;

  static_assert(RB % 4 == 0, "wave tile rows must be a multiple of 16");
  v4d acc4[RB / 4][CB];
#pragma unroll
  for (int a = 0; a < RB / 4; ++a)
#pragma unroll
    for (int b = 0; b < CB; ++b) acc4[a][b] = (v4d){0.0, 0.0, 0.0, 0.0};

  v2d ra[NVA], rb[NVB];
  unsigned ka = 0, kb_ = 0;
  unsigned offa[NVA], offb[NVB];
  thread_offsets<TM, A_KC, BK, NTH>(p.lda, tid, offa);
  thread_offsets<TN, B_KC, BK, NTH>(p.ldb, tid, offb);
  const double* __restrict__ ubaseA = A_KC ? A + (int64_t)row0 * p.lda : A + row0;
  const double* __restrict__ ubaseB = B_KC ? B + (int64_t)col0 * p.ldb : B + col0;
  const int64_t stepA = A_KC ? 1 : p.lda, stepB = B_KC ? 1 : p.ldb;

  const int Mld = (VAR == 2 && p.pad_ok) ? ((p.M + TM - 1) / TM) * TM : p.M;
  const int Nld = (VAR == 2 && p.pad_ok) ? ((p.N + TN - 1) / TN) * TN : p.N;
  int pa = 0, pb = 0;
  auto stage_load = [&](int kb) {
    pa = pb = 0;
    if constexpr (VAR == 2) {
      if (chunk_in_range<TM, BK>(row0, Mld, kb, khi)) pa = chunk_is_interior<TM, BK>(row0, Mld, kb, khi, p.a_mask) ? 1 : 2;
      if (chunk_in_range<TN, BK>(col0, Nld, kb, khi)) pb = chunk_is_interior<TN, BK>(col0, Nld, kb, khi, p.b_mask) ? 1 : 2;
    }
    if (pa) {
      load_fast<NVA>(ubaseA + (int64_t)kb * stepA, offa, ra);
      if (pa == 2) ka = mask_bits_mc<TM, BK, NTH>(row0, kb, p.a_mask, tid);
    } else {
      if constexpr (A_KC) ka = load_kc<TM>(A, p.lda, p.M, row0, kb, khi, p.a_mask, tid, ra);
      else ka = load_mc<TM, BK, NTH>(A, p.lda, p.M, row0, kb, khi, p.a_mask, tid, ra, A);
    }
    if (pb) {
      load_fast<NVB>(ubaseB + (int64_t)kb * stepB, offb, rb);
      if (pb == 2) kb_ = mask_bits_mc<TN, BK, NTH>(col0, kb, p.b_mask, tid);
    } else {
      if constexpr (B_KC) kb_ = load_kc<TN>(B, p.ldb, p.N, col0, kb, khi, p.b_mask, tid, rb);
      else kb_ = load_mc<TN, BK, NTH>(B, p.ldb, p.N, col0, kb, khi, p.b_mask, tid, rb, Bd);
    }
  };
  auto stage_store = [&](double* da, double* db) {
    if (pa == 1) {
      if constexpr (A_KC) store_kc<TM, false>(da, tid, ra, 0); else store_mc<TM, BK, false, NTH>(da, tid, ra, 0);
    } else {
      if constexpr (A_KC) store_kc<TM, true>(da, tid, ra, ka); else store_mc<TM, BK, true, NTH>(da, tid, ra, ka);
    }
    if (pb == 1) {
      if constexpr (B_KC) store_kc<TN, false>(db, tid, rb, 0); else store_mc<TN, BK, false, NTH>(db, tid, rb, 0);
    } else {
      if constexpr (B_KC) store_kc<TN, true>(db, tid, rb, kb_); else store_mc<TN, BK, true, NTH>(db, tid, rb, kb_);
    }
  };

  auto kpos = [&](int c) { return p.k_reverse ? klo + (nch - 1 - c) * BK : klo + c * BK; };
  if (nch > 0) {
    stage_load(kpos(0));
    stage_store(smem, smem + OPA);
  }
  __syncthreads();

  auto compute = [&](int cur) {
    const double* sa = smem + cur * (OPA + OPB) + (A_KC ? (wm + li) * LDK + lk : wm + li + lk * LDA);
    const double* sb = smem + cur * (OPA + OPB) + OPA + (B_KC ? (wn + li) * LDK + lk : wn + li + lk * LDB);
#pragma unroll
    for (int kk = 0; kk < BK / 4; ++kk) {
      double bf[CB], af[RB / 4];
#pragma unroll
      for (int b = 0; b < CB; ++b) bf[b] = B_KC ? sb[16 * b * LDK + kk * 4] : sb[kk * 4 * LDB + 16 * b];
#pragma unroll
      for (int a = 0; a < RB / 4; ++a) af[a] = A_KC ? sa[16 * a * LDK + kk * 4] : sa[kk * 4 * LDA + 16 * a];
#pragma unroll
      for (int a = 0; a < RB / 4; ++a)
#pragma unroll
        for (int b = 0; b < CB; ++b)
          acc4[a][b] = __builtin_amdgcn_mfma_f64_16x16x4f64(af[a], bf[b], acc4[a][b], 0, 0, 0);
    }
  };

  int ca = 0, cb = 0;
  constexpr bool SPLIT = (VAR == 2 && RB == 16 && CB == 4 && BK == 16);
  if constexpr (SPLIT) {
    if (row0 + TM <= Mld && col0 + TN <= Nld && nch > 1) {
      int k_lo = klo, k_hi = khi;
      if (p.a_mask == 1) k_hi = min(k_hi, row0 + 1);
      if (p.a_mask == 2) k_lo = max(k_lo, row0 + TM - 1);
      if (p.b_mask == 1) k_hi = min(k_hi, col0 + 1);
      if (p.b_mask == 2) k_lo = max(k_lo, col0 + TN - 1);
      int j_lo = (k_lo - klo + BK - 1) / BK, j_hi = (k_hi - klo) / BK;
      j_lo = max(j_lo, 0);
      j_hi = min(j_hi, nch);
      if (j_hi > j_lo) {
        const int ci_lo = p.k_reverse ? nch - j_hi : j_lo, ci_hi = p.k_reverse ? nch - j_lo : j_hi;
        ca = max(ci_lo - 1, 0);
        cb = min(ci_hi - 1, nch - 1);
        if (cb < ca) ca = cb = 0;
      }
    }
  }
  auto general_iter = [&](int c) {
    const int cur = (NBUF == 2) ? (c & 1) : 0;
    const bool more = (c + 1 < nch);
    if (more) stage_load(kpos(c + 1));
    compute(cur);
    if (NBUF == 1) __syncthreads();
    if (more) {
      const int nxt = (NBUF == 2) ? (cur ^ 1) : 0;
      stage_store(smem + nxt * (OPA + OPB), smem + nxt * (OPA + OPB) + OPA);
    }
    __syncthreads();
  };
  int c = 0;
  for (; c < ca; ++c) general_iter(c);
  if constexpr (SPLIT) {
    for (; c < cb; ++c) {
      const int cur = (NBUF == 2) ? (c & 1) : 0, nxt = (NBUF == 2) ? (cur ^ 1) : 0;
      const int kb = kpos(c + 1);
      load_fast<NVA>(ubaseA + (int64_t)kb * stepA, offa, ra);
      load_fast<NVB>(ubaseB + (int64_t)kb * stepB, offb, rb);
      if constexpr (TAG == 1) __builtin_amdgcn_s_setprio(1);
      compute(cur);
      if constexpr (TAG == 1) __builtin_amdgcn_s_setprio(0);
      if (NBUF == 1) __syncthreads();
      store_mc<TM, BK, false, NTH>(smem + nxt * (OPA + OPB), tid, ra, 0);
      store_mc<TN, BK, false, NTH>(smem + nxt * (OPA + OPB) + OPA, tid, rb, 0);
      __syncthreads();
    }
  }
  for (; c < nch; ++c) general_iter(c);
  before_epilogue();

  const double alpha = p.alpha, beta = p.beta;
  constexpr int GA = RB < 4 ? RB : 4;
#pragma unroll
  for (int a0 = 0; a0 < RB; a0 += GA) {
    double cold[GA][CB];
    if (beta != 0.0) {
#pragma unroll
      for (int a = 0; a < GA; ++a) {
        const int m = row0 + wm + 4 * (a0 + a) + lk;
#pragma unroll
        for (int b = 0; b < CB; ++b) {
          const int n = col0 + wn + 16 * b + li;
          const bool ok = (m < p.M) && (n < p.N) && (p.c_lower == 0 || (p.c_lower == 1 ? n <= m : n >= m));
          const double* src = ok ? C + (int64_t)m * p.ldc + n : Cd;
          cold[a][b] = *src;
        }
      }
    }
#pragma unroll
    for (int a = 0; a < GA; ++a) {
      const int m = row0 + wm + 4 * (a0 + a) + lk;
#pragma unroll
      for (int b = 0; b < CB; ++b) {
        const int n = col0 + wn + 16 * b + li;
        const bool ok = (m < p.M) && (n < p.N) && (p.c_lower == 0 || (p.c_lower == 1 ? n <= m : n >= m));
        double v = alpha * acc4[(a0 + a) >> 2][b][(a0 + a) & 3];
        if (beta != 0.0) v = fma(beta, cold[a][b], v);
        if (ok) {
          C[(int64_t)m * p.ldc + n] = v;
          if (C2)
            C2[(int64_t)n * p.ldc2 + m] = v;
        }
      }
    }
  }
}

template <int VAR, int WTM, int WTN, int TAG = 0, int BK = 16, int NBUF = 2, int WR = 2>
__global__ __launch_bounds__(128 * WR, ((VAR == 2 && !(BK > 16 && WTM >= 64)) || WTM < 64) ? 2 : 1) void gpp_gemm_f64(GemmArgs p) {
  constexpr int TM = WR * WTM, TN = 2 * WTN;
  extern __shared__ __attribute__((aligned(16))) double smem[];
  int tm, tn;
  if (p.swz) {
    const int b = blockIdx.x, xcd = b & 7, i = b >> 3;
    const int S = (i >> 6) * 8 + xcd, w = i & 63;
    const int super_n = (p.tiles_n + 7) >> 3;
    const int sm = S / super_n, sn = S - sm * super_n;
    tm = sm * 8 + (w >> 3);
    tn = sn * 8 + (w & 7);
    if (tm >= p.tiles_m || tn >= p.tiles_n) return;
    if ((p.c_lower == 1 && tn > tm) || (p.c_lower == 2 && tn < tm)) return;
  } else {
    const int t = (p.batch_fast ? (int)(blockIdx.x / (unsigned)p.nbatch) : (int)blockIdx.x) + (int)p.tile_base;
    if (p.c_lower == 1 && p.row_mod >= 1) {
      const float a = 0.5f * (float)p.row_mod, b = (float)p.row_off + 1.f - a;
      int i = (int)((-b + sqrtf(b * b + 4.f * a * (float)t)) / (2.f * a));
      auto S = [&](int q) { return q * (p.row_off + 1) + p.row_mod * (q * (q - 1) / 2); };
      while (S(i + 1) <= t) ++i;
      while (S(i) > t) --i;
      tm = p.row_off + p.row_mod * i;
      tn = t - S(i);
    } else if (p.c_lower == 1 && TM == 2 * TN) {
      tm = (int)((sqrtf(4.f * (float)t + 1.f) - 1.f) * 0.5f);
      while ((tm + 1) * (tm + 2) <= t) ++tm;
      while (tm * (tm + 1) > t) --tm;
      tn = t - tm * (tm + 1);
      if (tn >= p.tiles_n) return;
    } else if (p.c_lower) {
      tm = (int)((sqrtf(8.f * (float)t + 1.f) - 1.f) * 0.5f);
      while ((tm + 1) * (tm + 2) / 2 <= t) ++tm;
      while (tm * (tm + 1) / 2 > t) --tm;
      tn = t - tm * (tm + 1) / 2;
      if (p.c_lower == 1 && p.own_mod > 1 && (tn / p.own_bt + p.own_off) % p.own_mod != 0) return;
      if (p.c_lower == 2) {
        const int q = tm;
        tm = tn;
        tn = q;
        if (p.own_mod > 1 && (tm / p.own_bt + p.own_off) % p.own_mod != 0) return;
        if ((tn + 1) * TN <= p.skip_lead) return;
        if (p.row_limit > 0 && tm * TM >= p.row_limit) return;
      }
    } else if (p.col_major) {
      tn = t / p.tiles_m;
      tm = t - tn * p.tiles_m;
    } else {
      tm = t / p.tiles_n;
      tn = t - tm * p.tiles_n;
      if (p.row_reverse) tm = p.tiles_m - 1 - tm;
    }
  }
  const int64_t bi = p.batch_fast ? (int64_t)(blockIdx.x % (unsigned)p.nbatch) : (int64_t)blockIdx.y;
  gemm_tile<VAR, WTM, WTN, TAG, BK, NBUF, WR>(p, tm, tn, p.A + bi * p.sA + (int64_t)blockIdx.z * p.zA, p.B + bi * p.sB + (int64_t)blockIdx.z * p.zB,
                                             p.C + bi * p.sC + (int64_t)blockIdx.z * p.zC,
                                             p.C2 ? p.C2 + bi * p.sC2 + (int64_t)blockIdx.z * p.zC2 : nullptr, smem);

}

constexpr size_t gemm_lds_bytes(int var, int tm, int tn, int bk, int nbuf) {
  const int tx = tm > tn ? tm : tn;
  const int mc = bk * ldt_mc(tx, bk), kc = tx * LDK;
  return (size_t)nbuf * 2 * ((var != 2 && kc > mc) ? kc : mc) * sizeof(double);
}
template <int VAR, int WTM, int WTN, int TAG, int BK, int NBUF>
hipError_t launch_inst(hipStream_t s, dim3 grid, const GemmArgs& a) {
  constexpr size_t bytes = gemm_lds_bytes(VAR, 2 * WTM, 2 * WTN, BK, NBUF);
  auto* fn = gpp_gemm_f64<VAR, WTM, WTN, TAG, BK, NBUF>;
  if (bytes > 48 * 1024) {
    static std::atomic<bool> attr_set[64];
    int dev = 0;
    hipError_t e = hipGetDevice(&dev);
    if (e != hipSuccess) return e;
    if (dev < 0 || dev >= 64 || !attr_set[dev]) {
      e = hipFuncSetAttribute(reinterpret_cast<const void*>(fn), hipFuncAttributeMaxDynamicSharedMemorySize, (int)bytes);
      if (e != hipSuccess) return e;
      if (dev >= 0 && dev < 64) attr_set[dev] = true;
    }
  }
  hipLaunchKernelGGL(fn, grid, dim3(256), bytes, s, a);
  return hipGetLastError();
}
#ifndef GPP_SMALL_BK
#define GPP_SMALL_BK 64
#endif
template <int VAR>
hipError_t launch_var(hipStream_t s, int tm, int tn, dim3 grid, const GemmArgs& a) {
  constexpr int SBK = (VAR == 2) ? GPP_SMALL_BK : 16;
  constexpr int SNB = (VAR == 2 && GPP_SMALL_BK > 16) ? 1 : 2;
  if (tm == 128 && tn == 128 && a.tag == 1 && VAR == 2) return launch_inst<2, 64, 64, 1, 16, 2>(s, grid, a);
  if (tm == 128 && tn == 128) return launch_inst<VAR, 64, 64, 0, 16, 2>(s, grid, a);
  if (tm == 64 && tn == 64) return launch_inst<VAR, 32, 32, 0, SBK, SNB>(s, grid, a);
  if (tm == 32 && tn == 32) return launch_inst<VAR, 16, 16, 0, SBK, SNB>(s, grid, a);
  if (tm == 128 && tn == 32) return launch_inst<VAR, 64, 16, 0, SBK, SNB>(s, grid, a);
  return hipErrorInvalidValue;
}


#define GPP_AS4 __attribute__((address_space(4)))
typedef const GemmArgs GPP_AS4 CGemmArgs;

__device__ __forceinline__ int exec_load(const int* p) { return __hip_atomic_load(p, __ATOMIC_RELAXED, __HIP_MEMORY_SCOPE_AGENT); }

__device__ __forceinline__ bool exec_poll(int* counters, int w0, int v0, int w1, int v1, long long budget, int32_t* info,
                                          int status = GPP_INFO_EXEC_TIMEOUT) {
  long long t0 = 0;
  bool timed = false;
  for (;;) {
    const bool r0 = w0 < 0 || exec_load(counters + w0) >= v0;
    const bool r1 = w1 < 0 || exec_load(counters + w1) >= v1;
    if (r0 & r1) return true;
    if (!timed) {
      t0 = (long long)wall_clock64();
      timed = true;
    }
    const long long waited = (long long)wall_clock64() - t0;
    if (exec_load(counters) != 0) return false;
    if (waited > budget) {
      const long long ms = waited / 100000;
      __hip_atomic_store(counters, 1, __ATOMIC_RELAXED, __HIP_MEMORY_SCOPE_AGENT);
      atomicCAS(info, 0, status | (int)(ms > 0xFFFFF ? 0xFFFFF : ms));
      return false;
    }
    __builtin_amdgcn_s_sleep(2);
  }
}

typedef const DagTask GPP_AS4 CDagTask;
__global__ __launch_bounds__(64) void gpp_dag_bind(const GemmArgs* rel, GemmArgs* abs, int n, DagBases bases) {
  const int g = blockIdx.x * 64 + threadIdx.x;
  if (g >= n) return;
  GemmArgs a = rel[g];
  auto base = [&](int b) {
    return b == 0 ? bases.p[0] : b == 1 ? bases.p[1] : b == 2 ? bases.p[2] : b == 3 ? bases.p[3] : b == 4 ? bases.p[4] : b == 5 ? bases.p[5]
                                                                                                     : b == 6 ? bases.p[6] : bases.p[7];
  };
  a.A = reinterpret_cast<const double*>(base(a.buf[0]) + reinterpret_cast<uintptr_t>(a.A));
  a.B = reinterpret_cast<const double*>(base(a.buf[1]) + reinterpret_cast<uintptr_t>(a.B));
  a.C = reinterpret_cast<double*>(base(a.buf[2]) + reinterpret_cast<uintptr_t>(a.C));
  a.C2 = a.buf[3] >= 0 ? reinterpret_cast<double*>(base(a.buf[3]) + reinterpret_cast<uintptr_t>(a.C2)) : nullptr;
  abs[g] = a;
}
__global__ __launch_bounds__(256, 2) void gpp_dag_f64(DagLaunch e) {
  extern __shared__ __attribute__((aligned(16))) double smem[];
  __shared__ int s_idx, s_ok;
  const int tid = threadIdx.x;
#pragma clang diagnostic push
#pragma clang diagnostic ignored "-Wold-style-cast"
  CDagTask* tasks = (CDagTask*)e.tasks;
  CGemmArgs* groups = (CGemmArgs*)e.groups;
#pragma clang diagnostic pop
  int pre = -2;
  auto take = [&](int done_after) -> int {
    if (e.max_tasks > 0 && done_after >= e.max_tasks) return -1;
    if (e.quit_id >= 0 && (exec_load(e.counters) != 0 || exec_load(e.counters + e.quit_id) >= e.quit_val)) return -1;
    if (e.ticket_limit <= 0) return __hip_atomic_fetch_add(e.counters + 1, 1, __ATOMIC_RELAXED, __HIP_MEMORY_SCOPE_AGENT);
    int old = exec_load(e.counters + 1);
    while (old < e.ticket_limit &&
           !__hip_atomic_compare_exchange_strong(e.counters + 1, &old, old + 1, __ATOMIC_RELAXED, __ATOMIC_RELAXED, __HIP_MEMORY_SCOPE_AGENT)) {
    }
    return old < e.ticket_limit ? old : -1;
  };
  for (int done = 0;; ++done) {
    if (tid == 0) {
      s_idx = pre != -2 ? pre : take(done);
      pre = -2;
    }
    __syncthreads();
    const int idx = __builtin_amdgcn_readfirstlane(s_idx);
    __syncthreads();
    if (idx < 0 || idx >= e.ntasks) break;
    if (e.trace && tid == 0) {
      e.trace[4 * (size_t)idx] = wall_clock64();
      e.trace[4 * (size_t)idx + 3] = (unsigned long long)blockIdx.x | ((unsigned long long)(unsigned)e.tag << 32);
    }
    const int w0 = tasks[idx].wait_id[0], w1 = tasks[idx].wait_id[1], w2 = tasks[idx].wait_id[2];
    if (w0 >= 0 || w1 >= 0 || w2 >= 0) {
      if (tid == 0) {
        const int v0 = tasks[idx].wait_val[0], v1 = tasks[idx].wait_val[1], v2 = tasks[idx].wait_val[2];
        const int c0 = w0 >= 0 ? exec_load(e.counters + w0) : v0, c1 = w1 >= 0 ? exec_load(e.counters + w1) : v1,
                  c2 = w2 >= 0 ? exec_load(e.counters + w2) : v2;
        bool ok = (c0 >= v0) & (c1 >= v1) & (c2 >= v2);
        if (!ok) {
          ok = exec_poll(e.counters, w0, v0, w1, v1, e.budget, e.info, GPP_INFO_EXEC_TIMEOUT);
          if (ok && w2 >= 0) ok = exec_poll(e.counters, w2, v2, -1, 0, e.budget, e.info, GPP_INFO_EXEC_TIMEOUT);
        }
        s_ok = ok ? 1 : 0;
      }
      __syncthreads();
      const int ok = s_ok;
      __builtin_amdgcn_fence(__ATOMIC_ACQUIRE, "agent");
      __syncthreads();
      if (!ok) break;
    }
    if (e.trace && tid == 0) e.trace[4 * (size_t)idx + 1] = wall_clock64();
    const CGemmArgs& p = groups[tasks[idx].group];
    const int tm = tasks[idx].tm, tn = tasks[idx].tn;
    if (p.op == 0) {
      auto ahead = [&]() {
        if (tid == 0) pre = take(done + 1);
      };
      if (p.etile == 64) gemm_tile<2, 32, 32, 0, 64, 1, 2>(p, tm, tn, p.A, p.B, p.C, p.C2, smem);
      else gemm_tile<2, 64, 64, 0, 16, 2, 2>(p, tm, tn, p.A, p.B, p.C, p.C2, smem, ahead);
    } else {
      const int c = tn * 128 + ((tid & 63) << 1), r4 = tid >> 6;
      if (c < p.N) {
        const bool pair = c + 1 < p.N;
        for (int r0 = 0; r0 < p.M; r0 += 32) {
          v2d v[8];
#pragma unroll
          for (int q = 0; q < 8; ++q) {
            const int r = r0 + 4 * q + r4;
            const double* src = p.B + (int64_t)(r < p.M ? r : 0) * p.ldb + c;
            if (pair) v[q] = *reinterpret_cast<const v2d*>(src);
            else v[q] = (v2d){*src, 0.0};
          }
#pragma unroll
          for (int q = 0; q < 8; ++q) {
            const int r = r0 + 4 * q + r4;
            if (r < p.M) {
              double* dst = p.C + (int64_t)r * p.ldc + c;
              if (pair) *reinterpret_cast<v2d*>(dst) = v[q];
              else *dst = v[q].x;
            }
          }
        }
      }
    }
    const int i0 = tasks[idx].inc_id[0], i1 = tasks[idx].inc_id[1];
    if (i0 >= 0 || i1 >= 0) {
      asm volatile("s_waitcnt vmcnt(0)" ::: "memory");
      __syncthreads();
      if (tid == 0) {
        __builtin_amdgcn_fence(__ATOMIC_RELEASE, "agent");
        asm volatile("s_waitcnt vmcnt(0)" ::: "memory");
        if (i0 >= 0) __hip_atomic_fetch_add(e.counters + i0, (int)tasks[idx].inc_val[0], __ATOMIC_RELAXED, __HIP_MEMORY_SCOPE_AGENT);
        if (i1 >= 0) __hip_atomic_fetch_add(e.counters + i1, (int)tasks[idx].inc_val[1], __ATOMIC_RELAXED, __HIP_MEMORY_SCOPE_AGENT);
      }
    }
    if (e.trace) {
      asm volatile("s_waitcnt vmcnt(0)" ::: "memory");
      if (tid == 0) e.trace[4 * (size_t)idx + 2] = wall_clock64();
    }
  }
}

__global__ __launch_bounds__(64) void gpp_exec_gate(int* counters, int id, int target, int32_t* info, long long budget) {
  if (threadIdx.x == 0) (void)exec_poll(counters, id, target, -1, 0, budget, info);
}
__global__ __launch_bounds__(64) void gpp_exec_signal(int* counters, int id) {
  if (threadIdx.x == 0) {
    __builtin_amdgcn_fence(__ATOMIC_RELEASE, "agent");
    asm volatile("s_waitcnt vmcnt(0)" ::: "memory");
    __hip_atomic_fetch_add(counters + id, 1, __ATOMIC_RELAXED, __HIP_MEMORY_SCOPE_AGENT);
  }
}

}

hipError_t gpp_launch_gemm(hipStream_t s, int variant, const GemmArgs& a_in, int batch, int tile_m, int tile_n) {
  GemmArgs a = a_in;
  if (a.M <= 0 || a.N <= 0 || batch <= 0) return hipSuccess;
  auto ntiles = [&](int T) -> int64_t {
    const int64_t tm = (a.M + T - 1) / T, tn = (a.N + T - 1) / T;
    return (a.c_lower ? tm * (tm + 1) / 2 : tm * tn) * batch * (a.batch2 > 1 ? a.batch2 : 1);
  };
  if (tile_m == 0) {
    constexpr int64_t t128 = 256, t64 = 192;
    const int64_t cus = a.cu_hint > 0 ? a.cu_hint : 256;
    if (ntiles(128) * 256 >= t128 * cus) tile_m = 128;
    else if (ntiles(64) * 256 >= t64 * cus) tile_m = 64;
    else tile_m = 32;
    tile_n = tile_m;
  }
  if (a.c_lower && tile_m != tile_n) return hipErrorInvalidValue;
  a.tiles_m = (a.M + tile_m - 1) / tile_m;
  a.tiles_n = (a.N + tile_n - 1) / tile_n;
  int64_t nt = a.c_lower ? (int64_t)a.tiles_m * (a.tiles_m + 1) / 2 : (int64_t)a.tiles_m * a.tiles_n;
  a.tile_base = 0;
  if (a.c_lower == 1 && (a.row_mod > 1 || a.row_i1 > 0)) {
    if (a.row_mod < 1) { a.row_mod = 1; a.row_off = 0; }
    if (a.row_off < 0 || a.row_off >= a.row_mod) return hipErrorInvalidValue;
    const int64_t rows = a.tiles_m > a.row_off ? (a.tiles_m - a.row_off + a.row_mod - 1) / a.row_mod : 0;
    auto S = [&](int64_t i) { return i * (a.row_off + 1) + (int64_t)a.row_mod * (i * (i - 1) / 2); };
    const int64_t i0 = std::min<int64_t>(std::max(a.row_i0, 0), rows), i1 = a.row_i1 > 0 ? std::min<int64_t>(a.row_i1, rows) : rows;
    if (i1 <= i0) return hipSuccess;
    a.tile_base = S(i0);
    nt = S(i1) - S(i0);
  } else {
    a.row_mod = 0;
    if (a.c_lower == 1 && a.row_t1 > 0) {
      const int64_t t0 = std::min<int64_t>(std::max(a.row_t0, 0), a.tiles_m), t1 = std::min<int64_t>(a.row_t1, a.tiles_m);
      if (t1 <= t0) return hipSuccess;
      a.tile_base = t0 * (t0 + 1) / 2;
      nt = t1 * (t1 + 1) / 2 - a.tile_base;
    }
  }
  a.swz = 0;
  if (false && nt >= 1024) {
    const int64_t n_super = (int64_t)((a.tiles_m + 7) / 8) * ((a.tiles_n + 7) / 8);
    nt = ((n_super + 7) / 8) * 8 * 64;
    a.swz = 1;
  }
  const int batch2 = a.batch2 > 1 ? a.batch2 : 1;
  dim3 grid((unsigned)nt, (unsigned)batch, (unsigned)batch2);
  if (a.batch_fast && batch > 1 && !a.swz && nt * batch < (int64_t)1 << 31) {
    a.nbatch = batch;
    grid = dim3((unsigned)(nt * batch), 1u, (unsigned)batch2);
  } else {
    a.batch_fast = 0;
  }
  switch (variant) {
    case 0: return launch_var<0>(s, tile_m, tile_n, grid, a);
    case 1: return launch_var<1>(s, tile_m, tile_n, grid, a);
    case 2: return launch_var<2>(s, tile_m, tile_n, grid, a);
    default: return hipErrorInvalidValue;
  }
}

hipError_t gpp_launch_dag_bind(hipStream_t s, const GemmArgs* rel, GemmArgs* abs, int n, const DagBases& bases) {
  if (n <= 0) return hipSuccess;
  hipLaunchKernelGGL(gpp_dag_bind, dim3((unsigned)((n + 63) / 64)), dim3(64), 0, s, rel, abs, n, bases);
  return hipGetLastError();
}
hipError_t gpp_launch_dag(hipStream_t s, int nworkers, const DagLaunch& e) {
  if (nworkers <= 0) return hipSuccess;
  constexpr size_t b128 = gemm_lds_bytes(2, 128, 128, 16, 2), b64 = gemm_lds_bytes(2, 64, 64, 64, 1);
  constexpr size_t bytes = b128 > b64 ? b128 : b64;
  static std::atomic<bool> attr_set[64];
  int dev = 0;
  hipError_t err = hipGetDevice(&dev);
  if (err != hipSuccess) return err;
  if (dev < 0 || dev >= 64 || !attr_set[dev]) {
    err = hipFuncSetAttribute(reinterpret_cast<const void*>(gpp_dag_f64), hipFuncAttributeMaxDynamicSharedMemorySize, (int)bytes);
    if (err != hipSuccess) return err;
    if (dev >= 0 && dev < 64) attr_set[dev] = true;
  }
  hipLaunchKernelGGL(gpp_dag_f64, dim3((unsigned)nworkers), dim3(256), bytes, s, e);
  return hipGetLastError();
}
hipError_t gpp_launch_exec_gate(hipStream_t s, int* counters, int id, int target, int32_t* info, long long budget) {
  hipLaunchKernelGGL(gpp_exec_gate, dim3(1), dim3(64), 0, s, counters, id, target, info, budget);
  return hipGetLastError();
}
hipError_t gpp_launch_exec_signal(hipStream_t s, int* counters, int id) {
  hipLaunchKernelGGL(gpp_exec_signal, dim3(1), dim3(64), 0, s, counters, id);
  return hipGetLastError();
}
```

### gp-plus_amd/csrc/gpp_internal.h

```cpp
#pragma once
#include <hip/hip_runtime.h>
#include <stdint.h>
#include <stddef.h>
#include <vector>
#include "../../include/gpp.h"

#define GPP_TILE 128
#define GPP_DAG_PLANS 20

struct gpp_handle_s {
  int device;
  hipStream_t stream;
  void* ws;
  size_t ws_bytes;
  hipStream_t panel_stream;
  hipStream_t upd_stream;
  hipStream_t full_stream;
  hipStream_t fill_stream;
  int panel_cus;
  int cu_split;
  hipEvent_t events[16];
  int n_events, ev_next;
  int64_t inv_N;
  int inv_nblocks;
  int64_t inv_o[128], inv_n[128];
  char* panel_flags;
  int panel_next;
  int cap_next;
  hipEvent_t handoff;
  int ncu;
  int coop_panel;
  int panel_fault;
  int panel_timeout_ms;
  struct DagPlan* dag_plans[GPP_DAG_PLANS];
  uint64_t dag_clock;
  struct DagPlan* shard_cur;
  int32_t* shard_info;
  hipEvent_t shard_ready;
  int dag_sched;
  gpp_comm_t comm;
  int comm_rank, comm_nranks;
  void* rccl_comm;
  hipStream_t comm_stream;
  hipEvent_t comm_event;
};
extern "C" void gpp_shard_release_comm(gpp_handle_s* h);

struct GppEnv {
  bool coop_panel;
  bool dag_sched;
  bool dag_phased;
  bool shard_list;
  int shard_workers;
  int shard_fill;
  long long shard_timeout_ms;
  int64_t shard_piece_cols;
  bool sharded_force_collectives;
  bool exec_verbose;
  int dag_dump;
  bool dag_check_verbose;
};
const GppEnv& gpp_env();
constexpr int GPP_PANEL_RING = 8;
constexpr int GPP_PANEL_CAP_RING = 16;

#ifdef __HIPCC__
struct GppExpConsts {
  double log2e, ln2_hi, ln2_lo, c[11];
};
__device__ __forceinline__ GppExpConsts gpp_exp_consts() {
  GppExpConsts k = {1.44269504088896338700e+00, 6.93147180369123816490e-01, 1.90821492927058770002e-10,
                    {2.08767569878680989792e-09,
                     2.50521083854417187751e-08,
                     2.75573192239858906526e-07,
                     2.75573192239858906526e-06,
                     2.48015873015873015873e-05,
                     1.98412698412698412698e-04,
                     1.38888888888888888889e-03,
                     8.33333333333333333333e-03,
                     4.16666666666666666667e-02,
                     1.66666666666666666667e-01,
                     0.5}};
  asm volatile("" : "+s"(k.log2e), "+s"(k.ln2_hi), "+s"(k.ln2_lo));
#pragma unroll
  for (int i = 0; i < 10; ++i) asm volatile("" : "+s"(k.c[i]));
  return k;
}
__device__ __forceinline__ double gpp_exp_nonpos(double x, const GppExpConsts& k) {
  x = (x < -800.0) ? -800.0 : x;
  const double n = __builtin_rint(x * k.log2e);
  double r = __builtin_fma(-n, k.ln2_hi, x);
  r = __builtin_fma(-n, k.ln2_lo, r);
  double p = k.c[0];
#pragma unroll
  for (int i = 1; i < 11; ++i) p = __builtin_fma(p, r, k.c[i]);
  p = __builtin_fma(p, r, 1.0);
  p = __builtin_fma(p, r, 1.0);
  return __builtin_ldexp(p, (int)n);
}
#endif

struct GemmArgs {
  const double* A;
  const double* B;
  double* C;
  int64_t lda, ldb, ldc;
  int M, N, K;
  double alpha, beta;
  int a_mask, b_mask;
  int klo_mode, khi_mode;
  int c_lower;
  int64_t sA, sB, sC;
  int64_t zA, zB, zC, zC2;
  int batch2;
  int tiles_m, tiles_n;
  double* C2;
  int64_t ldc2, sC2;
  int k_reverse;
  int tag;
  int col_major;
  int row_reverse;
  int swz;
  int own_mod, own_off, own_bt;
  int skip_lead;
  int row_limit;
  int batch_fast, nbatch;
  int row_i0, row_i1;
  int64_t tile_base;
  int row_t0, row_t1;
  int cu_hint;
  int row_mod, row_off;
  int op;
  int compact_bc;
  int etile;
  int buf[4];
  int pad_ok;
};
hipError_t gpp_launch_gemm(hipStream_t s, int variant, const GemmArgs& a, int batch, int tile_m = 0, int tile_n = 0);

hipError_t gpp_launch_exec_gate(hipStream_t s, int* counters, int id, int target, int32_t* info, long long budget);
hipError_t gpp_launch_exec_signal(hipStream_t s, int* counters, int id);

struct DagTask {
  int32_t group;
  int16_t tm, tn;
  int32_t wait_id[3];
  int32_t wait_val[3];
  int32_t inc_id[2];
  int32_t kind;
  int16_t inc_val[2];
};
static_assert(sizeof(DagTask) == 48, "the device reads 48-byte task records");
struct DagLaunch {
  const GemmArgs* groups;
  const DagTask* tasks;
  int ntasks;
  int* counters;
  int32_t* info;
  long long budget;
  int max_tasks;
  int quit_id, quit_val;
  int ticket_limit;
  unsigned long long* trace;
  int tag;
};
hipError_t gpp_launch_dag(hipStream_t s, int nworkers, const DagLaunch& e);
struct DagBases { char* p[8]; };
hipError_t gpp_launch_dag_bind(hipStream_t s, const GemmArgs* rel, GemmArgs* abs, int n, const DagBases& bases);

enum { DK_S = 0, DK_U = 1, DK_CP = 2, DK_XB = 3, DK_XA = 4, DK_SH = 5, DK_UD = 6, DK_NKINDS = 7 };
struct DagTuning {
  double t0_big, tc_big;
  double t0_64, tc_64;
  double t0_32, tc_32;
  double t_copy;
  double t_panel0, t_panel_leaf;
  double t_gate;
  int chain_tile;
  int workers;
  int fill;
  int fuse;
  int64_t inv_rows;
  int64_t piece_cols;
};
struct DagPlan {
  int64_t N = 0, nb = 0, ld = 0, ldi = 0, ldt = 0, ldk = 0, inv_rows = 0;
  int rank = 0, nranks = 1, workers = 0, fill = 0;
  int c_cph = 0, c_cpt = 0, c_art = 0;
  int piece_tiles = 0, GP = 1;
  std::vector<int> cph_target, cpt_target;
  int flags = 0;
  int B = 0, nt = 0;
  std::vector<int> tb;
  std::vector<GemmArgs> groups;
  std::vector<DagTask> tasks;
  struct Op { int kind, arg, n, lim; };
  std::vector<Op> stream_ops;
  std::vector<int> gate_target;
  std::vector<int> level_first;
  int ncounters = 0;
  int c_pd = 0, c_g1d = 0;
  double sim_ms = 0, sim_busy = 0;
  GemmArgs* d_groups = nullptr;
  GemmArgs* d_groups_abs = nullptr;
  DagTask* d_tasks = nullptr;
  int* d_counters = nullptr;
  unsigned long long* d_trace = nullptr;
  hipEvent_t last_use = nullptr;
  uint64_t stamp = 0;
};
enum { DAG_INV = 1, DAG_SHARD = 4, DAG_BACK = 8 };
DagPlan* gpp_dag_plan(int64_t N, int64_t nb, int64_t ld, int64_t ldi, int64_t ldt, int64_t ldk, int flags, const DagTuning& tune,
                      int rank = 0, int nranks = 1);
DagTuning gpp_dag_default_tuning();
hipError_t gpp_dag_upload(DagPlan* P);
void gpp_dag_free(DagPlan* P);

hipError_t gpp_launch_fill_i32(hipStream_t s, int32_t* p, int n, int32_t value);
size_t gpp_panel_flag_bytes();
int gpp_panel_max_leaves();
hipError_t gpp_launch_panel(hipStream_t s, double* A, int64_t lda, double* Linv, int64_t ldi, int n, int32_t* info, int row_offset,
                            int* flags, int max_wgs, int timeout_ms);
hipError_t gpp_launch_leaf(hipStream_t s, double* A, int64_t lda, double* Linv, int64_t ldi, int n, int32_t* info,
                           int row_offset, int batch = 1, int64_t sA = 0, int64_t sLi = 0);

hipError_t gpp_launch_kernel_build(hipStream_t s, const double* U, int64_t N, int D, const double* w, const double* sf2,
                                   const double* tau, const int32_t* grp, int S, double jitter, int kind, int d_split,
                                   int uplo, double* Ky, int64_t ld, int64_t row0, int64_t nrows, int batch = 1,
                                   int64_t sU = 0, int64_t sK = 0);
hipError_t gpp_launch_cross_kernel(hipStream_t s, const double* Ua, int64_t Ma, const double* Ub, int64_t Nb, int D,
                                   const double* w, const double* sf2, int kind, int d_split, double* Kab, int64_t ld);
hipError_t gpp_launch_post_cov_train(hipStream_t s, const double* Kinv, int64_t ldk, int64_t N, const double* tau, const int32_t* grp,
                                     const double* d, double jitter, double* A, int64_t lda);

hipError_t gpp_launch_trmv_lower(hipStream_t s, const double* T, int64_t ldt, int64_t N, const double* x, double* y,
                                 int batch = 1, int64_t sT = 0, int64_t sv = 0);
hipError_t gpp_launch_trmv_upper(hipStream_t s, const double* T, int64_t ldt, int64_t N, const double* x, double* y,
                                 int batch = 1, int64_t sT = 0, int64_t sv = 0);
hipError_t gpp_launch_mll_scalars(hipStream_t s, const double* L, int64_t ld, int64_t N, const double* z, double* out3,
                                  int batch = 1, int64_t sL = 0, int64_t sv = 0);
size_t gpp_grad_ws_bytes(int64_t N, int D, int S, int dU);
hipError_t gpp_launch_grad_reduce(hipStream_t s, const double* U, int64_t N, int D, const double* w, const double* sf2,
                                  const int32_t* grp, int S, int kind, int d_split, const double* alpha,
                                  const double* Kinv, int64_t ldk, int dU, double* g_w, double* g_sf2, double* g_tau,
                                  double* g_U, void* ws, size_t ws_bytes, int shard_nb = 0, int shard_rank = 0,
                                  int shard_nranks = 1, int batch = 1, int64_t sU = 0, int64_t sK = 0, int64_t sv = 0,
                                  int shard_cols = 0);
hipError_t gpp_launch_trmv_lower_cols(hipStream_t s, const double* T, int64_t ldt, int64_t N, const double* x, double* y,
                                      int64_t nb, int rank, int nranks, int trans, void* ws, size_t ws_bytes, int compact = 0);
size_t gpp_trmv_t_ws_bytes(int64_t N);
hipError_t gpp_launch_transpose(hipStream_t s, const double* src, int64_t lds, int64_t rows, int64_t cols, double* dst, int64_t ldd);
size_t gpp_pgrad_ws_bytes(int64_t M, int64_t N, int D, int dA, int dB);
hipError_t gpp_launch_cross_grad(hipStream_t s, const double* Ua, int64_t M, const double* Ub, int64_t N, int D, const double* w,
                                 const double* sf2, int kind, int d_split, const double* gmean, const double* alpha,
                                 const double* gvar, const double* B, int64_t ldb, double* g_Ua, int dA, double* g_Ub, int dB,
                                 double* g_w, double* g_sf2, void* ws, size_t ws_bytes);
hipError_t gpp_launch_predict_reduce(hipStream_t s, const double* Ksn, int64_t lds, const double* V, int64_t ldv,
                                     int64_t M, int64_t N, const double* alpha, const double* kss, double* mean_out,
                                     double* var_out);
```

### gp-plus_amd/csrc/gpp_reduce.hip

```cpp
#include "gpp_internal.h"

#include <algorithm>

typedef double v2d __attribute__((ext_vector_type(2)));

namespace {

__device__ __forceinline__ double wave_sum(double v) {
#pragma unroll
  for (int o = 32; o > 0; o >>= 1) v += __shfl_xor(v, o);
  return v;
}

__global__ __launch_bounds__(256) void gpp_trmv_lower(const double* __restrict__ T, int64_t ldt, int64_t N,
                                                      const double* __restrict__ x, double* __restrict__ y, int64_t sT,
                                                      int64_t sv) {
  const int wave = threadIdx.x >> 6, lane = threadIdx.x & 63;
  const int64_t i = (int64_t)blockIdx.x * 4 + wave;
  if (i >= N) return;
  T += (int64_t)blockIdx.y * sT;
  x += (int64_t)blockIdx.y * sv;
  y += (int64_t)blockIdx.y * sv;
  const double* row = T + i * ldt;
  double acc = 0.0;
// ... 606 lines not shown
  }
  __syncthreads();
  for (int e = tid; e < dA * GT; e += 256) {
    const int d = e / GT, r = e - d * GT;
    if (i0 + r < M) gApart[((int64_t)c * M + i0 + r) * dA + d] = accA[e];
  }
  const int nrec = D + 1;
  const int64_t wg = t * CN + c;
  for (int q = 0; q < nrec; ++q) {
    double v = my_sf2;
    if (q < D) v = (lane == 0) ? wacc[wave * DT + q] : 0.0;
    __syncthreads();
    red[tid] = v;
    __syncthreads();
    for (int o = 128; o > 0; o >>= 1) {
      if (tid < o) red[tid] += red[tid + o];
      __syncthreads();
    }
    if (tid == 0) rec[wg * nrec + q] = red[0];
  }
}

__global__ __launch_bounds__(256) void gpp_pgrad_finish(const double* __restrict__ rec, int nwg, int D, double* __restrict__ g_w,
                                                        double* __restrict__ g_sf2) {
  __shared__ double red[256];
  const int q = blockIdx.x, nrec = D + 1, tid = threadIdx.x;
  double v = 0.0;
  for (int b = tid; b < nwg; b += 256) v += rec[(int64_t)b * nrec + q];
  red[tid] = v;
  __syncthreads();
  for (int o = 128; o > 0; o >>= 1) {
    if (tid < o) red[tid] += red[tid + o];
    __syncthreads();
  }
  if (tid == 0) {
    if (q < D && g_w) g_w[q] = red[0];
    else if (q == D && g_sf2) g_sf2[0] = red[0];
  }
}

__global__ __launch_bounds__(256) void gpp_predict_rows(const double* __restrict__ Ksn, int64_t lds, const double* __restrict__ V,
                                                        int64_t ldv, int64_t M, int64_t N, const double* __restrict__ alpha,
                                                        const double* __restrict__ kss, double* __restrict__ mean_out,
                                                        double* __restrict__ var_out) {
  const int wave = threadIdx.x >> 6, lane = threadIdx.x & 63;
  const int64_t a = (int64_t)blockIdx.x * 4 + wave;
  if (a >= M) return;
  double m = 0.0, q = 0.0;
  const double* kr = Ksn + a * lds;
  for (int64_t j = lane; j < N; j += 64) m = fma(kr[j], alpha[j], m);
  if (V) {
    const double* vr = V + a * ldv;
    for (int64_t j = lane; j < N; j += 64) q = fma(vr[j], vr[j], q);
  }
  m = wave_sum(m);
  q = wave_sum(q);
  if (lane == 0) {
    mean_out[a] = m;
    if (V && var_out) var_out[a] = kss[a] - q;
  }
}

}

hipError_t gpp_launch_trmv_lower(hipStream_t s, const double* T, int64_t ldt, int64_t N, const double* x, double* y,
                                 int batch, int64_t sT, int64_t sv) {
  if (N <= 0 || batch <= 0) return hipSuccess;
  hipLaunchKernelGGL(gpp_trmv_lower, dim3((unsigned)((N + 3) / 4), (unsigned)batch), dim3(256), 0, s, T, ldt, N, x, y, sT, sv);
  return hipGetLastError();
}

hipError_t gpp_launch_trmv_upper(hipStream_t s, const double* T, int64_t ldt, int64_t N, const double* x, double* y,
                                 int batch, int64_t sT, int64_t sv) {
  if (N <= 0 || batch <= 0) return hipSuccess;
  hipLaunchKernelGGL(gpp_trmv_upper, dim3((unsigned)((N + 3) / 4), (unsigned)batch), dim3(256), 0, s, T, ldt, N, x, y, sT, sv);
  return hipGetLastError();
}

size_t gpp_trmv_t_ws_bytes(int64_t N) { return (size_t)TRT_CHUNKS * (size_t)N * sizeof(double); }

hipError_t gpp_launch_trmv_lower_cols(hipStream_t s, const double* T, int64_t ldt, int64_t N, const double* x, double* y,
                                      int64_t nb, int rank, int nranks, int trans, void* ws, size_t ws_bytes, int compact) {
  if (N <= 0) return hipSuccess;
  if (nb < 64 || nb % 64 != 0 || nranks < 1 || rank < 0 || rank >= nranks) return hipErrorInvalidValue;
  if (trans) {
    if (!ws || ws_bytes < gpp_trmv_t_ws_bytes(N)) return hipErrorInvalidValue;
    const int64_t chunk = (((N + TRT_CHUNKS - 1) / TRT_CHUNKS) + 31) / 32 * 32;
    double* part = reinterpret_cast<double*>(ws);
    hipLaunchKernelGGL(gpp_trmv_lower_t_cols, dim3((unsigned)((N + 63) / 64), TRT_CHUNKS), dim3(256), 0, s, T, ldt, N, x, part, nb,
                       rank, nranks, chunk, compact);
    hipLaunchKernelGGL(gpp_trmv_lower_t_finish, dim3((unsigned)((N + 255) / 256)), dim3(256), 0, s, part, N, TRT_CHUNKS, y);
  } else
    hipLaunchKernelGGL(gpp_trmv_lower_cols, dim3((unsigned)((N + 3) / 4)), dim3(256), 0, s, T, ldt, N, x, y, nb, rank, nranks, compact);
  return hipGetLastError();
}

hipError_t gpp_launch_mll_scalars(hipStream_t s, const double* L, int64_t ld, int64_t N, const double* z, double* out3,
                                  int batch, int64_t sL, int64_t sv) {
  if (batch <= 0) return hipSuccess;
  hipLaunchKernelGGL(gpp_mll_scalars, dim3((unsigned)batch), dim3(1024), 0, s, L, ld, N, z, out3, sL, sv);
  return hipGetLastError();
}

size_t gpp_grad_ws_bytes(int64_t N, int D, int S, int dU) {
  (void)S;
  const int64_t T = (N + GT - 1) / GT;
  return (size_t)G_WGS * (D + 1) * sizeof(double) + (size_t)N * sizeof(double) +
         (size_t)T * N * (dU > 0 ? dU : 0) * sizeof(double) + 256;
}

hipError_t gpp_launch_grad_reduce(hipStream_t s, const double* U, int64_t N, int D, const double* w, const double* sf2,
                                  const int32_t* grp, int S, int kind, int d_split, const double* alpha,
                                  const double* Kinv, int64_t ldk, int dU, double* g_w, double* g_sf2, double* g_tau,
                                  double* g_U, void* ws, size_t ws_bytes, int shard_nb, int shard_rank, int shard_nranks,
                                  int batch, int64_t sU, int64_t sK, int64_t sv, int shard_cols) {
  if (kind < 0 || kind > 2) return hipErrorInvalidValue;
  if (batch < 1 || batch > 65535) return hipErrorInvalidValue;
  if (shard_nranks > 1 && (shard_nb < GT || shard_nb % GT != 0 || shard_rank < 0 || shard_rank >= shard_nranks))
    return hipErrorInvalidValue;
  if (D > GD_MAX || D < 1 || S > GS_MAX || S < 1 || dU > D || dU < 0) return hipErrorInvalidValue;
  if (ws_bytes < (size_t)batch * gpp_grad_ws_bytes(N, D, S, dU)) return hipErrorInvalidValue;
  const int64_t ws_stride = (int64_t)(gpp_grad_ws_bytes(N, D, S, dU) / sizeof(double));
  const int T = (int)((N + GT - 1) / GT);
  const int64_t ntiles = (int64_t)T * (T + 1) / 2;
  const int nwg = (int)(ntiles < G_WGS ? ntiles : G_WGS);
  double* rec = reinterpret_cast<double*>(ws);
  double* wdiag = rec + (size_t)G_WGS * (D + 1);
  double* gUpart = wdiag + N;
  if (shard_nranks > 1) {
    hipError_t e = hipMemsetAsync(ws, 0, (size_t)batch * ws_stride * sizeof(double), s);
    if (e != hipSuccess) return e;
  }
  auto launch = [&](auto kern) {
    hipLaunchKernelGGL(kern, dim3(nwg, batch), dim3(256), 0, s, U, N, D, w, sf2, kind, d_split, alpha, Kinv, ldk, dU, ntiles,
                       shard_nb, shard_rank, shard_nranks, shard_cols, sU, sK, sv, ws_stride, rec, wdiag, gUpart);
  };
  const bool mat = kind != 0, hasu = dU > 0;
#define GPP_GT(DT)                                                                                                   \
  (mat ? (hasu ? launch(gpp_grad_tiles<DT, true, true>) : launch(gpp_grad_tiles<DT, true, false>))                   \
       : (hasu ? launch(gpp_grad_tiles<DT, false, true>) : launch(gpp_grad_tiles<DT, false, false>)))
  if (D <= 8) GPP_GT(8);
  else if (D <= 16) GPP_GT(16);
  else if (D <= 32) GPP_GT(32);
  else GPP_GT(64);
#undef GPP_GT
  hipLaunchKernelGGL(gpp_grad_finish, dim3(D + 1 + S, batch), dim3(256), 0, s, rec, nwg, D, S, wdiag, grp, N, g_w, g_sf2, g_tau,
                     ws_stride);
  if (dU > 0)
    hipLaunchKernelGGL(gpp_gU_finish, dim3((unsigned)((N * dU + 255) / 256), batch), dim3(256), 0, s, gUpart, N, dU, T, g_U,
                       ws_stride);
  return hipGetLastError();
}

size_t gpp_pgrad_ws_bytes(int64_t M, int64_t N, int D, int dA, int dB) {
  const PgradShape p = pgrad_shape(M, N);
  const int64_t nwg = p.MT * p.CN;
  return ((size_t)nwg * (D + 1) + (size_t)p.CN * M * std::max(dA, 0) + (size_t)p.MT * N * std::max(dB, 0)) * sizeof(double);
}

hipError_t gpp_launch_cross_grad(hipStream_t s, const double* Ua, int64_t M, const double* Ub, int64_t N, int D, const double* w,
                                 const double* sf2, int kind, int d_split, const double* gmean, const double* alpha,
                                 const double* gvar, const double* B, int64_t ldb, double* g_Ua, int dA, double* g_Ub, int dB,
                                 double* g_w, double* g_sf2, void* ws, size_t ws_bytes) {
  if (kind < 0 || kind > 2 || D < 1 || D > GD_MAX) return hipErrorInvalidValue;
  if (M <= 0 || N <= 0) {
    if (g_w) if (hipError_t e = hipMemsetAsync(g_w, 0, (size_t)D * sizeof(double), s); e != hipSuccess) return e;
    if (g_sf2) if (hipError_t e = hipMemsetAsync(g_sf2, 0, sizeof(double), s); e != hipSuccess) return e;
    if (dA > 0 && M > 0) if (hipError_t e = hipMemsetAsync(g_Ua, 0, (size_t)M * dA * sizeof(double), s); e != hipSuccess) return e;
    if (dB > 0 && N > 0) if (hipError_t e = hipMemsetAsync(g_Ub, 0, (size_t)N * dB * sizeof(double), s); e != hipSuccess) return e;
    return hipSuccess;
  }
  const PgradShape p = pgrad_shape(M, N);
  if (p.MT > 65535) return hipErrorInvalidValue;
  if (ws_bytes < gpp_pgrad_ws_bytes(M, N, D, dA, dB)) return hipErrorInvalidValue;
  const int nwg = (int)(p.MT * p.CN);
  double* rec = reinterpret_cast<double*>(ws);
  double* gApart = rec + (size_t)nwg * (D + 1);
  double* gBpart = gApart + (size_t)p.CN * M * std::max(dA, 0);
  auto launch = [&](auto kern) {
    hipLaunchKernelGGL(kern, dim3((unsigned)p.CN, (unsigned)p.MT), dim3(256), 0, s, Ua, M, Ub, N, D, w, sf2, kind, d_split, gmean,
                       alpha, gvar, B, ldb, dA, dB, g_w ? 1 : 0, p.CN, rec, gApart, gBpart);
  };
  const bool mat = kind != 0;
#define GPP_PG(DT) (mat ? launch(gpp_pgrad_tiles<DT, true>) : launch(gpp_pgrad_tiles<DT, false>))
  if (D <= 8) GPP_PG(8);
  else if (D <= 16) GPP_PG(16);
  else if (D <= 32) GPP_PG(32);
  else GPP_PG(64);
#undef GPP_PG
  if (g_w || g_sf2) hipLaunchKernelGGL(gpp_pgrad_finish, dim3(D + 1), dim3(256), 0, s, rec, nwg, D, g_w, g_sf2);
  if (dA > 0)
    hipLaunchKernelGGL(gpp_gU_finish, dim3((unsigned)((M * dA + 255) / 256), 1), dim3(256), 0, s, gApart, M, dA, p.CN, g_Ua,
                       (int64_t)0);
  if (dB > 0)
    hipLaunchKernelGGL(gpp_gU_finish, dim3((unsigned)((N * dB + 255) / 256), 1), dim3(256), 0, s, gBpart, N, dB, (int)p.MT, g_Ub,
                       (int64_t)0);
  return hipGetLastError();
}

hipError_t gpp_launch_predict_reduce(hipStream_t s, const double* Ksn, int64_t lds, const double* V, int64_t ldv,
                                     int64_t M, int64_t N, const double* alpha, const double* kss, double* mean_out,
                                     double* var_out) {
  if (M <= 0) return hipSuccess;
  hipLaunchKernelGGL(gpp_predict_rows, dim3((unsigned)((M + 3) / 4)), dim3(256), 0, s, Ksn, lds, V, ldv, M, N, alpha, kss,
                     mean_out, var_out);
  return hipGetLastError();
}

namespace {
__global__ __launch_bounds__(256) void gpp_transpose_tile(const double* __restrict__ src, int64_t lds, int64_t rows, int64_t cols,
                                                          double* __restrict__ dst, int64_t ldd) {
  __shared__ double tile[64][65];
  const int64_t r0 = (int64_t)blockIdx.y * 64, c0 = (int64_t)blockIdx.x * 64;
  const int tx = threadIdx.x & 63, ty = threadIdx.x >> 6;
#pragma unroll 4
  for (int i = ty; i < 64; i += 4) {
    const int64_t r = r0 + i, c = c0 + tx;
    tile[i][tx] = (r < rows && c < cols) ? src[r * lds + c] : 0.0;
  }
  __syncthreads();
#pragma unroll 4
  for (int i = ty; i < 64; i += 4) {
    const int64_t c = c0 + i, r = r0 + tx;
    if (c < cols && r < rows) dst[c * ldd + r] = tile[tx][i];
  }
}
}

hipError_t gpp_launch_transpose(hipStream_t s, const double* src, int64_t lds, int64_t rows, int64_t cols, double* dst, int64_t ldd) {
  if (rows <= 0 || cols <= 0) return hipSuccess;
  dim3 grid((unsigned)((cols + 63) / 64), (unsigned)((rows + 63) / 64));
  hipLaunchKernelGGL(gpp_transpose_tile, grid, dim3(256), 0, s, src, lds, rows, cols, dst, ldd);
  return hipGetLastError();
}
```

### gp-plus_amd/linalg.py

```python
from __future__ import annotations

import threading
import warnings
from contextlib import contextmanager
from dataclasses import dataclass
from typing import Dict, Optional, Tuple

import torch

from .backend import (KIND_RBF, OP_MLL_EVAL, UPLO_FULL, UPLO_UPPER, GppContext, get_context, panel_timed_out, square_buffer)
from .errors import NanError, NotPSDError
from . import settings

__all__ = ["KernelSpec", "exact_mll", "ExactMLLFunction", "EvalWorkspace", "dense_kernel", "cross_kernel",
           "FactorCache", "factorize", "dense_log_prob", "predict_mean", "predict_var", "predictive_cov_upper",
           "train_post_cov_upper", "mvn_root", "mvn_draw"]


@dataclass
class KernelSpec:
    w: torch.Tensor
    sf2: torch.Tensor
    kind: int = KIND_RBF
    d_split: int = 0


class EvalWorkspace:

    def __init__(self, ctx: GppContext, N: int):
        dev = ctx.device
        self.N = N
        self.A = square_buffer(N, dev)
        self.Li = square_buffer(N, dev)
        self.Ki = square_buffer(N, dev)
        self.z = torch.empty(N, dtype=torch.float64, device=dev)
        self.alpha = torch.empty(N, dtype=torch.float64, device=dev)
        self.r = torch.empty(N, dtype=torch.float64, device=dev)
        self.out3 = torch.empty(3, dtype=torch.float64, device=dev)
        self.info = torch.zeros(1, dtype=torch.int32, device=dev)
        self.info_host = torch.zeros(1, dtype=torch.int32).pin_memory()
        self.info_event = torch.cuda.Event()
        self.epoch = 0


_workspaces: Dict[Tuple[int, int, int], EvalWorkspace] = {}
_workspaces_lock = threading.Lock()
_tls = threading.local()


@contextmanager
def eval_slot(slot: int):
    old = getattr(_tls, "slot", 0)
    _tls.slot = slot
    try:
        yield
    finally:
        _tls.slot = old


def current_slot() -> int:
    return getattr(_tls, "slot", 0)

LOOKAHEAD_MIN_N = 3840

STAGE_EVENTS = None


class _stage:
    def __init__(self, name: str):
        self.name = name

    def __enter__(self):
        if STAGE_EVENTS is not None:
            self.e0 = torch.cuda.Event(enable_timing=True)
            self.e0.record()
        return self

    def __exit__(self, *exc):
        if STAGE_EVENTS is not None:
            e1 = torch.cuda.Event(enable_timing=True)
            e1.record()
            STAGE_EVENTS.append((self.name, self.e0, e1))
        return False


def get_workspace(ctx: GppContext, N: int, slot: int = 0) -> EvalWorkspace:
    key = (ctx.index, N, slot)
    ws = _workspaces.get(key)
    if ws is None:
        with _workspaces_lock:
            for k in [k for k in _workspaces if k[0] == ctx.index and k[2] == slot]:
                del _workspaces[k]
            ws = EvalWorkspace(ctx, N)
            _workspaces[key] = ws
    return ws


def _as_f64(t: torch.Tensor, device) -> torch.Tensor:
    return t.to(device=device, dtype=torch.float64).contiguous()


def _factor(ctx: GppContext, ws: EvalWorkspace, U, w, sf2, tau, grp, kind, d_split, after=None) -> float:
    if torch.cuda.is_current_stream_capturing():
        if ws.N >= LOOKAHEAD_MIN_N:
            raise RuntimeError("graph capture of the evaluation is limited to the single-stream factorisation (N < 3840)")
        ctx.kernel_build(U, w, sf2, tau, grp, ws.A, jitter=0.0, kind=kind, d_split=d_split, uplo=UPLO_UPPER)
        ctx.potrf(ws.A, ws.Li, ws.info, ws.Ki)
        if after is not None:
            after()
        return 0.0
    jitters = [0.0] + [settings.cholesky_jitter.value() * (10 ** i) for i in range(settings.cholesky_max_tries.value())]
    attempts = list(jitters)
    while attempts:
        jit = attempts.pop(0)
        if ws.N >= LOOKAHEAD_MIN_N:
            torch.cuda.current_stream(ctx.index).synchronize()
        with _stage("kernel_build"):
            ctx.kernel_build(U, w, sf2, tau, grp, ws.A, jitter=jit, kind=kind, d_split=d_split, uplo=UPLO_UPPER)
        with _stage("potrf"):
            ctx.potrf(ws.A, ws.Li, ws.info, ws.Ki)
        ws.info_host.copy_(ws.info, non_blocking=True)
        ws.info_event.record(torch.cuda.current_stream(ctx.index))
        if after is not None:
            after()
        ws.info_event.synchronize()
        info = int(ws.info_host[0])
        if panel_timed_out(ctx, info):
            attempts.insert(0, jit)
            continue
        if info == 0:
            if jit > 0:
                warnings.warn(f"A not p.d., added jitter of {jit:.1e} to the diagonal", RuntimeWarning)
            return jit
        if jit == 0.0:
            bad = [n for n, t in (("inputs", U), ("weights", w), ("outputscale", sf2), ("noise", tau)) if not torch.isfinite(t).all()]
            if bad:
                raise NanError(f"cholesky: NaN/Inf in {', '.join(bad)} of the covariance")
    raise NotPSDError(f"Matrix not positive definite after repeatedly adding jitter up to {jitters[-1]:.1e} "
                      f"(leading minor {info}).")


class ExactMLLFunction(torch.autograd.Function):

    @staticmethod
    def forward(ctx, U, w, sf2, tau, mean, y, grp, kind, d_split, dU, slot):
        get_context(U.device)
        with torch.cuda.device(U.device):
            return ExactMLLFunction._forward(ctx, U, w, sf2, tau, mean, y, grp, kind, d_split, dU, slot)

    @staticmethod
    def _forward(ctx, U, w, sf2, tau, mean, y, grp, kind, d_split, dU, slot):
        dev = U.device
        gctx = get_context(dev)
        N, D = U.shape
        Ud, wd, sd, td = _as_f64(U.detach(), dev), _as_f64(w.detach(), dev), _as_f64(sf2.detach().reshape(1), dev), \
            _as_f64(tau.detach().reshape(-1), dev)
        S = td.numel()
        if grp is not None and grp.dtype != torch.int32:
            grp = grp.to(torch.int32)
        ws = get_workspace(gctx, N, slot)
        ws.epoch += 1
        torch.sub(_as_f64(y.detach(), dev), _as_f64(mean.detach(), dev), out=ws.r)
        need = ctx.needs_input_grad
        need_grad = any(need[:6])
        need_U = need[0] and dU > 0
        g_w = g_s = g_t = g_Ud = None
        if need_grad:
            g_w = torch.empty(D, dtype=torch.float64, device=dev)
            g_s = torch.empty(1, dtype=torch.float64, device=dev)
            g_t = torch.empty(S, dtype=torch.float64, device=dev)
            g_Ud = torch.empty(N, dU, dtype=torch.float64, device=dev) if need_U else None

        def rest():
            with _stage("trtri"):
                gctx.trtri(ws.A, ws.Li, ws.Ki)
            with _stage("mll_reduce"):
                gctx.mll_reduce(ws.A, ws.Li, ws.r, ws.z, ws.out3)
            if not need_grad:
                return
            with _stage("alpha"):
                gctx.alpha(ws.Li, ws.z, ws.alpha)
            with _stage("lauum"):
                gctx.lauum(ws.Li, ws.Ki)
            with _stage("grad_reduce"):
                gctx.grad_reduce(Ud, wd, sd, grp, S, ws.alpha, ws.Ki, dU if need_U else 0, g_w, g_s, g_t, g_Ud, kind=kind,
                                 d_split=d_split)

        _factor(gctx, ws, Ud, wd, sd, td, grp, kind, d_split, after=rest)
        ctx.saved = (g_w, g_s, g_t, g_Ud, ws.alpha.clone() if need_grad else None, (N, D, dU))
        ctx.in_dtypes = (U.dtype, w.dtype, sf2.dtype, tau.dtype, mean.dtype, y.dtype)
        ctx.shapes = (sf2.shape, tau.shape)
        return ws.out3[2].clone()

    @staticmethod
    def backward(ctx, grad_out):
        g_w, g_s, g_t, g_Ud, alpha, (N, D, dU) = ctx.saved
        need = ctx.needs_input_grad
        go = grad_out.to(torch.float64)
        g_U = None
        if need[0]:
            g_U = torch.zeros(N, D, dtype=torch.float64, device=alpha.device)
            if g_Ud is not None:
                g_U[:, :dU] = g_Ud
        dt = ctx.in_dtypes
        sf2_shape, tau_shape = ctx.shapes
        return (None if g_U is None else (go * g_U).to(dt[0]),
                (go * g_w).to(dt[1]) if need[1] else None,
                (go * g_s).reshape(sf2_shape).to(dt[2]) if need[2] else None,
                (go * g_t).reshape(tau_shape).to(dt[3]) if need[3] else None,
                (go * alpha).to(dt[4]) if need[4] else None,
                (-go * alpha).to(dt[5]) if need[5] else None,
                None, None, None, None, None)


def exact_mll(U: torch.Tensor, spec: KernelSpec, tau: torch.Tensor, mean: torch.Tensor, y: torch.Tensor,
              grp: Optional[torch.Tensor] = None, n_grad_dims: Optional[int] = None, slot: Optional[int] = None) -> torch.Tensor:
    if slot is None:
        slot = current_slot()
    if n_grad_dims is None:
        n_grad_dims = U.shape[1] if U.requires_grad else 0
    shard = settings.sharded_evaluation.value()
    if shard is not None:
        from .sharded import sharded_mll
        return sharded_mll(U, spec.w, spec.sf2, tau, mean, y, grp, spec.kind, spec.d_split, int(n_grad_dims),
                           group=shard.get("group"), nb=int(shard.get("nb", 1024)))
    return ExactMLLFunction.apply(U, spec.w, spec.sf2, tau, mean, y, grp, spec.kind, spec.d_split, int(n_grad_dims), slot)


@torch.no_grad()
def dense_kernel(U: torch.Tensor, spec: KernelSpec, tau: Optional[torch.Tensor] = None,
                 grp: Optional[torch.Tensor] = None, jitter: float = 0.0) -> torch.Tensor:
    dev = U.device
    gctx = get_context(dev)
    N = U.shape[0]
    out = square_buffer(N, dev)
    gctx.kernel_build(_as_f64(U, dev), _as_f64(spec.w, dev), _as_f64(spec.sf2.reshape(1), dev),
                      None if tau is None else _as_f64(tau.reshape(-1), dev),
                      None if grp is None else grp.to(torch.int32), out, jitter=jitter, kind=spec.kind,
                      d_split=spec.d_split, uplo=UPLO_FULL)
    return out


@torch.no_grad()
def cross_kernel(Ua: torch.Tensor, Ub: torch.Tensor, spec: KernelSpec) -> torch.Tensor:
    dev = Ua.device
    gctx = get_context(dev)
    M, N = Ua.shape[0], Ub.shape[0]
    ld = max(16, (N + 15) // 16 * 16)
    out = torch.empty((M, ld), dtype=torch.float64, device=dev)[:, :N]
    gctx.cross_kernel(_as_f64(Ua, dev), _as_f64(Ub, dev), _as_f64(spec.w, dev), _as_f64(spec.sf2.reshape(1), dev), out,
                      kind=spec.kind, d_split=spec.d_split)
    return out


class FactorCache:

    def __init__(self, gctx, L, Linv, alpha, U, spec, jitter, ws=None, z=None, refactor=None):
        self.gctx, self.L, self.Linv, self.alpha, self.U, self.spec, self.jitter = gctx, L, Linv, alpha, U, spec, jitter
        self.z = z
        self._ws, self._epoch = ws, (ws.epoch if ws is not None else 0)
        self._refactor = refactor

    def stale(self) -> bool:
        return self._ws is not None and self._ws.epoch != self._epoch

    def refresh(self) -> None:
        if not self.stale():
            return
        if self._refactor is None:
            raise RuntimeError("the prediction workspace was reused by another model and this cache cannot be rebuilt")
        tau, grp, r = self._refactor
        with torch.cuda.device(self.U.device):
            fresh = _factorize(self.U, self.spec, tau, grp, torch.zeros_like(r), r)
        self.L, self.Linv, self.alpha, self.z, self.jitter = fresh.L, fresh.Linv, fresh.alpha, fresh.z, fresh.jitter
        self._ws, self._epoch = fresh._ws, fresh._epoch


@torch.no_grad()
def factorize(U, spec: KernelSpec, tau, grp, mean, y) -> FactorCache:
    get_context(U.device)
    with torch.cuda.device(U.device):
        return _factorize(U, spec, tau, grp, mean, y)


def _factorize(U, spec: KernelSpec, tau, grp, mean, y) -> FactorCache:
    dev = U.device
    gctx = get_context(dev)
    N = U.shape[0]
    Ud, wd = _as_f64(U, dev), _as_f64(spec.w, dev)
    sd, td = _as_f64(spec.sf2.reshape(1), dev), _as_f64(tau.reshape(-1), dev)
    if grp is not None:
        grp = grp.to(torch.int32)
    ws = get_workspace(gctx, N, slot=-1)
    ws.epoch += 1
    jit = _factor(gctx, ws, Ud, wd, sd, td, grp, spec.kind, spec.d_split)
    gctx.trtri(ws.A, ws.Li, ws.Ki)
    torch.sub(_as_f64(y, dev), _as_f64(mean, dev), out=ws.r)
    gctx.mll_reduce(ws.A, ws.Li, ws.r, ws.z, ws.out3)
    gctx.alpha(ws.Li, ws.z, ws.alpha)
    return FactorCache(gctx, ws.A, ws.Li, ws.alpha.clone(), Ud, KernelSpec(wd, sd.reshape(()), spec.kind, spec.d_split), jit, ws,
                       z=ws.z.clone(), refactor=(td.clone(), None if grp is None else grp.clone(), ws.r.clone()))


@torch.no_grad()
def predict_from_cache(cache: FactorCache, Us: torch.Tensor, need_var: bool = True, need_V: bool = False):
    dev = Us.device
    gctx = cache.gctx
    M, N = Us.shape[0], cache.U.shape[0]
    mean = torch.empty(M, dtype=torch.float64, device=dev)
    if not (need_var or need_V):
        Ksn = cross_kernel(Us, cache.U, cache.spec)
        gctx.predict(cache.Linv, cache.alpha, Ksn, None, None, mean, None)
        return mean, None, None
    Kns = cross_kernel(cache.U, Us, cache.spec)
    ldv = max(16, (N + 15) // 16 * 16)
    V = torch.empty((M, ldv), dtype=torch.float64, device=dev)[:, :N]
    kss = cache.spec.sf2.reshape(1).expand(M).contiguous()
    var = torch.empty(M, dtype=torch.float64, device=dev)
    gctx.predict_tn(cache.Linv, cache.z, Kns, kss, V, mean, var)
    return mean, var, V


def _cross_backward(ctx, gmean, alpha, gvar, B):
    cache, dB = ctx.cache, ctx.dB
    Us, Utr, w, sf2 = ctx.saved_tensors
    need = ctx.needs_input_grad
    dev = cache.U.device
    Ua = _as_f64(Us.detach(), dev)
    Ub = cache.U if Utr is None else _as_f64(Utr.detach(), dev)
    M, D = Ua.shape
    N = Ub.shape[0]
    f64 = dict(dtype=torch.float64, device=dev)
    g_Ua = torch.empty(M, D, **f64) if need[0] else None
    g_Ub = torch.empty(N, dB, **f64) if need[1] and dB > 0 else None
    g_w = torch.empty(D, **f64) if need[2] else None
    g_s = torch.empty(1, **f64) if need[3] else None
    if g_Ua is not None or g_Ub is not None or g_w is not None or g_s is not None:
        cache.gctx.cross_grad(Ua, Ub, _as_f64(w.detach(), dev), _as_f64(sf2.detach().reshape(1), dev), gmean, alpha, gvar, B,
                              g_Ua, g_Ub, g_w, g_s, kind=cache.spec.kind, d_split=cache.spec.d_split)
# ... 175 lines not shown
```

### include/gpp.h

```cpp
#ifndef GPP_H
#define GPP_H

#include <stddef.h>
#include <stdint.h>

#ifdef __cplusplus
extern "C" {
#endif

typedef struct gpp_handle_s* gpp_handle_t;

#define GPP_KIND_RBF      0
#define GPP_KIND_MATERN32 1
#define GPP_KIND_MATERN52 2

#define GPP_UPLO_FULL  0
#define GPP_UPLO_LOWER 1
#define GPP_UPLO_UPPER 2

#define GPP_OP_MLL_EVAL 0
#define GPP_OP_PREDICT  1
#define GPP_OP_PREDICT_GRAD 2

const char* gpp_version(void);

int gpp_create(gpp_handle_t* out, int device);
int gpp_destroy(gpp_handle_t h);
int gpp_set_stream(gpp_handle_t h, void* stream);
int gpp_internal_stream(gpp_handle_t h, int which, void** out);
#define GPP_OPT_COOP_PANEL 1
#define GPP_OPT_PANEL_FAULT 2
#define GPP_OPT_PANEL_TIMEOUT_MS 3
#define GPP_OPT_EXEC_SCHED 4
#define GPP_OPT_DAG_SCHED 5
#define GPP_INFO_PANEL_TIMEOUT (1 << 30)
#define GPP_INFO_EXEC_TIMEOUT ((1 << 30) | (1 << 29))
int gpp_set_option(gpp_handle_t h, int option, int value);
size_t gpp_workspace_bytes(gpp_handle_t h, int op, int64_t N, int64_t M, int D, int S);
int gpp_set_workspace(gpp_handle_t h, void* ws, size_t bytes);

int gpp_kernel_build(gpp_handle_t h, const double* U, int64_t N, int D, const double* w, const double* sf2,
                     const double* tau, const int32_t* grp, int S, double jitter, int kind, int d_split,
                     int uplo, double* Ky, int64_t ld, int64_t row0, int64_t nrows);

int gpp_cross_kernel(gpp_handle_t h, const double* Ua, int64_t Ma, const double* Ub, int64_t Nb, int D,
                     const double* w, const double* sf2, int kind, int d_split, double* Kab, int64_t ld);

int gpp_potrf(gpp_handle_t h, double* A, int64_t N, int64_t ld, double* Linv, int64_t ldi, int32_t* info_dev);
int gpp_potrf_ws(gpp_handle_t h, double* A, int64_t N, int64_t ld, double* Linv, int64_t ldi, double* T, int64_t ldt,
                 int32_t* info_dev);

int gpp_trtri(gpp_handle_t h, const double* U, int64_t N, int64_t ld, double* Linv, int64_t ldi, double* T, int64_t ldt);

int gpp_lauum(gpp_handle_t h, const double* Linv, int64_t N, int64_t ldi, double* Kinv, int64_t ldk);

int gpp_post_cov_train(gpp_handle_t h, const double* Kinv, int64_t N, int64_t ldk, const double* tau, const int32_t* grp, int S,
                       const double* d, double jitter, double* A, int64_t lda);

int gpp_syrk_rows(gpp_handle_t h, const double* Urow, int64_t ldu, double* C, int64_t ldc, int64_t Nt, int64_t K, int64_t nb,
                  int64_t first_block, int rank, int nranks);

int gpp_gemm_lower_cols(gpp_handle_t h, const double* A, int64_t lda, const double* B, int64_t ldb, double* C, int64_t ldc,
                        int64_t M, int64_t K, double alpha, double beta, int64_t nb, int64_t first_block, int rank, int nranks,
                        int64_t row0, int64_t row1, int compact);

int gpp_shard_list_begin(gpp_handle_t h, int64_t N, int64_t nb, int rank, int nranks, double* A, int64_t ld, double* Kc, double* Lc,
                         int64_t ldc, double* D, double* W0, double* W1, double* W2, int64_t ldw, int32_t* info, int workers,
                         int* used);
int64_t gpp_shard_piece_cols(void);
int gpp_shard_list_gate(gpp_handle_t h, void* stream, int tail, int k);
int gpp_shard_list_signal(gpp_handle_t h, void* stream, int tail, int k);
int gpp_shard_list_end(gpp_handle_t h);

int gpp_shard_back_list(gpp_handle_t h, int64_t N, int64_t nb, int rank, int nranks, const double* A, int64_t ld, double* Kc, double* Lc,
                        int64_t ldc, const double* D, int32_t* info, int workers, int* used);

enum { GPP_COMM_SUM_F64 = 0, GPP_COMM_MAX_I32 = 1 };
#define GPP_SHARD_UNSUPPORTED 2000
typedef struct gpp_comm {
  void* user;
  int (*bcast)(void* user, void* dev_buf, size_t bytes, int root, void* stream);
  int (*allreduce)(void* user, void* dev_buf, size_t count, int kind, void* stream);
} gpp_comm_t;
typedef struct gpp_shard_buffers {
  double* A; int64_t ld;
  double* Kc; double* Lc; int64_t ldc;
  double* D;
  double* W0; double* W1; double* W2; int64_t ldw;
  double* msg;
  double* z; double* alpha; double* r;
  double* flat;
  double* out3; int32_t* info;
} gpp_shard_buffers_t;
int gpp_set_comm(gpp_handle_t h, const gpp_comm_t* comm, int rank, int nranks);
int gpp_comm_unique_id(void* out128);
int gpp_comm_init_rccl(gpp_handle_t h, const void* unique_id128, int rank, int nranks);
size_t gpp_shard_buffer_doubles(int64_t N, int64_t nb, int rank, int nranks, int which);
int gpp_shard_eval(gpp_handle_t h, int64_t N, int64_t nb, const double* U, int D, const double* w, const double* sf2, const double* tau,
                   const int32_t* grp, int S, int kind, int d_split, double jitter, int dU, int need_grad, const gpp_shard_buffers_t* b,
                   int32_t* info_host);

typedef struct gpp_push* gpp_push_t;
#define GPP_PUSH_HANDLE_BYTES 128
int gpp_push_create(int device, int rank, int nranks, int64_t slot_bytes, gpp_push_t* out, void* handle_out);
int gpp_push_connect(gpp_push_t p, const void* handles );
int gpp_push_send(gpp_push_t p, void* after_stream, int64_t seq, int32_t* status, int code, int nparts, const void* const* src,
                  const int64_t* spitch, const int64_t* offset, const int64_t* dpitch, const int64_t* width, const int64_t* height);
int gpp_push_recv(gpp_push_t p, void* stream, int64_t seq, int32_t* status, int code, int nparts, void* const* dst, const int64_t* dpitch,
                  const int64_t* offset, const int64_t* spitch, const int64_t* width, const int64_t* height);
int gpp_push_ack(gpp_push_t p, void* stream, int64_t seq);
int gpp_push_info(gpp_push_t p, int64_t* slot_bytes, int* flag_kind );
int gpp_push_destroy(gpp_push_t p, int stage);

int gpp_trmv_lower_cols(gpp_handle_t h, const double* T, int64_t ldt, int64_t N, const double* x, double* y, int64_t nb, int rank,
                        int nranks, int trans, int compact);

int gpp_mll_scalars(gpp_handle_t h, const double* U, int64_t ld, int64_t N, const double* z, double* out3);

int gpp_lauum_rows(gpp_handle_t h, const double* Linv, int64_t N, int64_t ldi, double* Kinv, int64_t ldk, int rank, int nranks);

int gpp_lauum_rows_range(gpp_handle_t h, const double* Linv, int64_t N, int64_t ldi, double* Kinv, int64_t ldk, int rank,
                         int nranks, int64_t row0, int64_t row1);

int gpp_transpose(gpp_handle_t h, const double* src, int64_t lds, int64_t rows, int64_t cols, double* dst, int64_t ldd);

int gpp_mll_reduce(gpp_handle_t h, const double* U, int64_t ld, const double* Linv, int64_t ldi, int64_t N,
                   const double* r, double* z, double* out3);

int gpp_alpha(gpp_handle_t h, const double* Linv, int64_t ldi, int64_t N, const double* z, double* alpha);

int gpp_grad_reduce(gpp_handle_t h, const double* U, int64_t N, int D, const double* w, const double* sf2,
                    const int32_t* grp, int S, int kind, int d_split, const double* alpha, const double* Kinv,
                    int64_t ldk, int dU, double* g_w, double* g_sf2, double* g_tau, double* g_U);

int gpp_grad_reduce_rows(gpp_handle_t h, const double* U, int64_t N, int D, const double* w, const double* sf2,
                         const int32_t* grp, int S, int kind, int d_split, const double* alpha, const double* Kinv,
                         int64_t ldk, int dU, int64_t nb, int rank, int nranks, double* g_w, double* g_sf2, double* g_tau,
                         double* g_U);

int gpp_grad_reduce_cols(gpp_handle_t h, const double* U, int64_t N, int D, const double* w, const double* sf2,
                         const int32_t* grp, int S, int kind, int d_split, const double* alpha, const double* Kinv,
                         int64_t ldk, int dU, int64_t nb, int rank, int nranks, double* g_w, double* g_sf2, double* g_tau,
                         double* g_U, int compact);

int gpp_predict(gpp_handle_t h, const double* Linv, int64_t ldi, int64_t N, const double* alpha, const double* Ksn,
                int64_t lds, int64_t M, const double* kss, double* V, int64_t ldv, double* mean_out, double* var_out);

int gpp_predict_tn(gpp_handle_t h, const double* Linv, int64_t ldi, int64_t N, const double* z, const double* Kns, int64_t ldk,
                   int64_t M, const double* kss, double* V, int64_t ldv, double* mean_out, double* var_out);

int gpp_cross_grad(gpp_handle_t h, const double* Ua, int64_t M, const double* Ub, int64_t N, int D, const double* w,
                   const double* sf2, int kind, int d_split, const double* gmean, const double* alpha, const double* gvar,
                   const double* B, int64_t ldb, double* g_Ua, int dA, double* g_Ub, int dB, double* g_w, double* g_sf2);

int gpp_gemm(gpp_handle_t h, int transA, int transB, int64_t M, int64_t N, int64_t K, double alpha, const double* A,
             int64_t lda, const double* B, int64_t ldb, double beta, double* C, int64_t ldc, int a_mask, int b_mask,
             int klo_mode, int khi_mode, int c_tri);

int gpp_gemm_batched(gpp_handle_t h, int transA, int transB, int64_t M, int64_t N, int64_t K, double alpha, const double* A,
                     int64_t lda, int64_t sA, const double* B, int64_t ldb, int64_t sB, double beta, double* C, int64_t ldc,
                     int64_t sC, int batch, int a_mask, int b_mask, int klo_mode, int khi_mode, int c_tri);

int gpp_kernel_build_batched(gpp_handle_t h, const double* U, int64_t sU, int64_t N, int D, const double* w, const double* sf2,
                             const double* tau, const int32_t* grp, int S, double jitter, int kind, int d_split, int uplo,
                             double* Ky, int64_t ld, int64_t sK, int batch);
int gpp_potrf_batched(gpp_handle_t h, double* A, int64_t N, int64_t ld, int64_t sA, double* Linv, int64_t ldi, int64_t sLi,
                      int32_t* info_dev, int batch);
int gpp_trtri_batched(gpp_handle_t h, const double* U, int64_t N, int64_t ld, int64_t sA, double* Linv, int64_t ldi,
                      int64_t sLi, double* T, int64_t ldt, int64_t sT, int batch);
int gpp_lauum_batched(gpp_handle_t h, const double* Linv, int64_t N, int64_t ldi, int64_t sLi, double* Kinv, int64_t ldk,
                      int64_t sK, int batch);
int gpp_mll_reduce_batched(gpp_handle_t h, const double* U, int64_t ld, int64_t sA, const double* Linv, int64_t ldi,
                           int64_t sLi, int64_t N, const double* r, double* z, int64_t sv, double* out3, int batch);
int gpp_alpha_batched(gpp_handle_t h, const double* Linv, int64_t ldi, int64_t sLi, int64_t N, const double* z, double* alpha,
                      int64_t sv, int batch);
int gpp_grad_reduce_batched(gpp_handle_t h, const double* U, int64_t sU, int64_t N, int D, const double* w, const double* sf2,
                            const int32_t* grp, int S, int kind, int d_split, const double* alpha, int64_t sv,
                            const double* Kinv, int64_t ldk, int64_t sK, int dU, double* g_w, double* g_sf2, double* g_tau,
                            double* g_U, int batch);

#ifdef __cplusplus
}
#endif
#endif
```

Baseline: 7.836 evals/s.

## Fuse LAUUM with gradient reduction and overlap kernel build with Cholesky DAG

Adds a fused LAUUM kernel whose GEMM epilogue computes the RBF hyperparameter gradient partials directly from accumulator tiles. This avoids writing the full N×N inverse and then re-reading it in a separate grad_reduce pass. It also adds a combined build+potrf entry point: the covariance build is split so only the leading panel columns are built before the DAG Cholesky starts, and the rest is built on the update stream and gated by an event. The cost is more complex synchronisation, a different floating-point reduction order for the gradients, and the fused path only covers RBF with D≤16 and no input gradients.

```diff
diff --git a/gp-plus_amd/_lib.py b/gp-plus_amd/_lib.py
--- a/gp-plus_amd/_lib.py
+++ b/gp-plus_amd/_lib.py
@@ -27,8 +27,12 @@
                                  c_int, c_void_p, c_int64]),
     "gpp_potrf": (c_int, [c_void_p, c_void_p, c_int64, c_int64, c_void_p, c_int64, c_void_p]),
     "gpp_potrf_ws": (c_int, [c_void_p, c_void_p, c_int64, c_int64, c_void_p, c_int64, c_void_p, c_int64, c_void_p]),
+    "gpp_build_potrf_ws": (c_int, [c_void_p, c_void_p, c_int64, c_int, c_void_p, c_void_p, c_void_p, c_void_p, c_int, c_double, c_int,
+                                   c_int, c_void_p, c_int64, c_void_p, c_int64, c_void_p, c_int64, c_void_p]),
     "gpp_trtri": (c_int, [c_void_p, c_void_p, c_int64, c_int64, c_void_p, c_int64, c_void_p, c_int64]),
     "gpp_lauum": (c_int, [c_void_p, c_void_p, c_int64, c_int64, c_void_p, c_int64]),
+    "gpp_lauum_grad": (c_int, [c_void_p, c_void_p, c_int64, c_int64, c_void_p, c_int, c_void_p, c_void_p, c_void_p, c_int, c_int, c_int,
+                               c_void_p, c_void_p, c_void_p, c_void_p]),
     "gpp_post_cov_train": (c_int, [c_void_p, c_void_p, c_int64, c_int64, c_void_p, c_void_p, c_int, c_void_p, c_double, c_void_p,
                                    c_int64]),
     "gpp_syrk_rows": (c_int, [c_void_p, c_void_p, c_int64, c_void_p, c_int64, c_int64, c_int64, c_int64, c_int64, c_int, c_int]),
diff --git a/gp-plus_amd/backend.py b/gp-plus_amd/backend.py
--- a/gp-plus_amd/backend.py
+++ b/gp-plus_amd/backend.py
@@ -16,6 +16,8 @@
 UPLO_FULL, UPLO_LOWER, UPLO_UPPER = 0, 1, 2
 OPT_COOP_PANEL, OPT_PANEL_FAULT, OPT_PANEL_TIMEOUT_MS, OPT_EXEC_SCHED, OPT_DAG_SCHED = 1, 2, 3, 4, 5
 OP_MLL_EVAL, OP_PREDICT, OP_PREDICT_GRAD = 0, 1, 2
+NOT_SUPPORTED = 2001
+NO_WORKSPACE = 2002
 MAX_FEATURES = 64
 
 
@@ -201,6 +203,25 @@
                                         _ld(T), info.data_ptr()), "gpp_potrf_ws")
 
     @_on_own_device
+    def build_potrf(self, U, w, sf2, tau, grp, A, Linv, info, T, *, jitter=0.0, kind=KIND_RBF, d_split=0):
+        N, D = U.shape
+        _check_features(D)
+        for t, n in ((U, "U"), (w, "w"), (sf2, "sf2"), (A, "A"), (Linv, "Linv"), (T, "T")):
+            _need(t, torch.float64, n)
+        _need(info, torch.int32, "info")
+        if tau is not None:
+            _need(tau, torch.float64, "tau")
+        S = 0 if tau is None else tau.numel()
+        if grp is not None:
+            self._check_groups(grp, N, S)
+        if not U.is_contiguous():
+            raise GppError("U must be contiguous")
+        self._stream()
+        check(self.lib.gpp_build_potrf_ws(self.h, U.data_ptr(), N, D, w.data_ptr(), sf2.data_ptr(), _ptr(tau), _ptr(grp), S,
+                                          float(jitter), kind, d_split, A.data_ptr(), _ld(A), Linv.data_ptr(), _ld(Linv),
+                                          T.data_ptr(), _ld(T), info.data_ptr()), "gpp_build_potrf_ws")
+
+    @_on_own_device
     def trtri(self, U, Linv, T):
         self._stream()
         check(self.lib.gpp_trtri(self.h, U.data_ptr(), U.shape[0], _ld(U), Linv.data_ptr(), _ld(Linv), T.data_ptr(), _ld(T)),
@@ -210,6 +231,28 @@
     def lauum(self, Linv, Kinv):
         self._stream()
         check(self.lib.gpp_lauum(self.h, Linv.data_ptr(), Linv.shape[0], _ld(Linv), Kinv.data_ptr(), _ld(Kinv)), "gpp_lauum")
+
+    @_on_own_device
+    def lauum_grad(self, Linv, U, w, sf2, grp, S, alpha, dU, g_w, g_sf2, g_tau, *, kind=KIND_RBF) -> bool:
+        N, D = U.shape
+        for t, n in ((Linv, "Linv"), (U, "U"), (w, "w"), (sf2, "sf2"), (alpha, "alpha"), (g_w, "g_w"), (g_sf2, "g_sf2"),
+                     (g_tau, "g_tau")):
+            _need(t, torch.float64, n)
+        if grp is not None:
+            self._check_groups(grp, N, S)
+        if not U.is_contiguous():
+            raise GppError("U must be contiguous")
+        self.ensure_workspace(OP_MLL_EVAL, N, 0, D, S)
+        self._stream()
+        status = self.lib.gpp_lauum_grad(self.h, Linv.data_ptr(), N, _ld(Linv), U.data_ptr(), D, w.data_ptr(), sf2.data_ptr(),
+                                         _ptr(grp), S, kind, dU, alpha.data_ptr(), g_w.data_ptr(), g_sf2.data_ptr(),
+                                         g_tau.data_ptr())
+        if status == NOT_SUPPORTED:
+            return False
+        if status == NO_WORKSPACE:
+            raise GppError("gpp_lauum_grad: the handle's scratch workspace is missing or too small")
+        check(status, "gpp_lauum_grad")
+        return True
 
     @_on_own_device
     def post_cov_train(self, Kinv, tau, grp, d, out, *, jitter=0.0):
diff --git a/gp-plus_amd/csrc/gpp_api.hip b/gp-plus_amd/csrc/gpp_api.hip
--- a/gp-plus_amd/csrc/gpp_api.hip
+++ b/gp-plus_amd/csrc/gpp_api.hip
@@ -489,7 +489,16 @@
 constexpr int64_t DAG_INV_MAX_N = 19456;
 constexpr int64_t DAG_NB = 1024;
 
-hipError_t potrf_dag(gpp_handle_s* h, const Ctx& cm, int64_t N, double* T, int64_t ldt, bool* used) {
+struct KyBuild {
+  const double *U, *w, *sf2, *tau;
+  const int32_t* grp;
+  int D, S, kind, d_split;
+  double jitter;
+  hipError_t operator()(hipStream_t s, const Ctx& c, int64_t N, int64_t c0, int64_t c1) const {
+    return gpp_launch_kernel_build(s, U, N, D, w, sf2, tau, grp, S, jitter, kind, d_split, GPP_UPLO_UPPER, c.A, c.ld, c0, c1 - c0);
+  }
+};
+hipError_t potrf_dag(gpp_handle_s* h, const Ctx& cm, int64_t N, double* T, int64_t ldt, bool* used, const KyBuild* build = nullptr) {
   *used = false;
   if (!gpp_env().dag_sched || !h->dag_sched || !h->coop_panel || !T || N < DAG_MIN_N || N > DAG_MAX_N) return hipSuccess;
   HIP_TRY(ensure_streams(h));
@@ -532,6 +541,9 @@
   HIP_TRY(gpp_launch_fill_i32(cm.s, P->d_counters, P->ncounters, 0));
   DagBases bases{{reinterpret_cast<char*>(cm.A), reinterpret_cast<char*>(cm.Li), reinterpret_cast<char*>(T), nullptr}};
   HIP_TRY(gpp_launch_dag_bind(cm.s, P->d_groups, P->d_groups_abs, (int)P->groups.size(), bases));
+  const int64_t lead = std::min<int64_t>((int64_t)P->tb[1] * NBLK, N);
+  const bool split_build = build && !gpp_env().dag_phased && lead < N;
+  if (build) HIP_TRY((*build)(cm.s, cm, N, 0, split_build ? lead : N));
   hipEvent_t ev = next_event(h);
   HIP_TRY(hipEventRecord(ev, cm.s));
   HIP_TRY(hipStreamWaitEvent(cp.s, ev, 0));
@@ -558,6 +570,13 @@
     *used = true;
     return hipSuccess;
   }
+  hipEvent_t built = nullptr;
+  if (split_build) {
+    ++h->split_builds;
+    HIP_TRY((*build)(cu.s, cu, N, lead, N));
+    built = next_event(h);
+    HIP_TRY(hipEventRecord(built, cu.s));
+  }
   HIP_TRY(gpp_launch_dag(cu.s, 2 * (h->ncu - h->panel_cus), dl));
   auto enqueue_panel_stream = [&]() -> hipError_t {
     for (const DagPlan::Op& op : P->stream_ops) {
@@ -567,6 +586,10 @@
       } else if (op.kind == 1) {
         const int64_t rows = std::min<int64_t>((int64_t)P->tb[op.arg + 1] * NBLK, N) - o;
         HIP_TRY(launch_panel(h, cp, o, rows, h->panel_cus));
+        if (built) {
+          HIP_TRY(hipStreamWaitEvent(cp.s, built, 0));
+          built = nullptr;
+        }
       } else if (op.kind == 2) {
         HIP_TRY(gpp_launch_exec_signal(cp.s, P->d_counters, P->c_pd + op.arg));
       } else {
@@ -634,6 +657,7 @@
       if (h->dag_plans[i] && (!P || h->dag_plans[i]->stamp > P->stamp)) P = h->dag_plans[i];
   return P;
 }
+int gpp_debug_split_builds(gpp_handle_t h) { return h ? h->split_builds : -1; }
 int gpp_debug_dag_info(gpp_handle_t h, int64_t* info8) {
   const DagPlan* P = dag_mru(h);
   if (!P) return -1;
@@ -1001,7 +1025,7 @@
 size_t gpp_workspace_bytes(gpp_handle_t h, int op, int64_t N, int64_t M, int D, int S) {
   (void)h;
   if (op == GPP_OP_MLL_EVAL) {
-    return std::max(gpp_grad_ws_bytes(N, D, S, D), gpp_trmv_t_ws_bytes(N)) + 256;
+    return std::max({gpp_grad_ws_bytes(N, D, S, D), gpp_trmv_t_ws_bytes(N), gpp_lauum_grad_ws_bytes(N, D)}) + 256;
   }
   if (op == GPP_OP_PREDICT) return 256;
   if (op == GPP_OP_PREDICT_GRAD) return gpp_pgrad_ws_bytes(M, N, D, D, S) + 256;
@@ -1055,8 +1079,8 @@
   return 0;
 }
 
-int gpp_potrf_ws(gpp_handle_t h, double* A, int64_t N, int64_t ld, double* Linv, int64_t ldi, double* T, int64_t ldt,
-                 int32_t* info_dev) {
+static int potrf_ws_impl(gpp_handle_t h, double* A, int64_t N, int64_t ld, double* Linv, int64_t ldi, double* T, int64_t ldt,
+                         int32_t* info_dev, const KyBuild* build) {
   if (!h) return -1;
   if (N < 0) return -3;
   if (int r = check_mat(A, ld, N, 2)) return r;
@@ -1071,8 +1095,15 @@
   h->inv_nblocks = 0;
   const int64_t la_min = T ? BORDER_MIN_N : 6 * LOOKAHEAD_NB;
   bool dag_used = false;
-  GPP_TRY(potrf_dag(h, c, N, T, ldt, &dag_used));
+  hipStreamCaptureStatus cap = hipStreamCaptureStatusNone;
+  if (build) GPP_TRY(hipStreamIsCapturing(h->stream, &cap));
+  if (build && cap != hipStreamCaptureStatusNone) {
+    GPP_TRY((*build)(h->stream, c, N, 0, N));
+    build = nullptr;
+  }
+  GPP_TRY(potrf_dag(h, c, N, T, ldt, &dag_used, build));
   if (dag_used) return 0;
+  if (build) GPP_TRY((*build)(h->stream, c, N, 0, N));
   if (N >= la_min) {
     GPP_TRY(potrf_lookahead(h, c, N, LOOKAHEAD_NB, T, ldt));
   } else if (panel_fits(h, N)) {
@@ -1099,6 +1130,33 @@
   return 0;
 }
 
+int gpp_potrf_ws(gpp_handle_t h, double* A, int64_t N, int64_t ld, double* Linv, int64_t ldi, double* T, int64_t ldt,
+                 int32_t* info_dev) {
+  return potrf_ws_impl(h, A, N, ld, Linv, ldi, T, ldt, info_dev, nullptr);
+}
+
+int gpp_build_potrf_ws(gpp_handle_t h, const double* U, int64_t N, int D, const double* w, const double* sf2, const double* tau,
+                       const int32_t* grp, int S, double jitter, int kind, int d_split, double* A, int64_t ld, double* Linv,
+                       int64_t ldi, double* T, int64_t ldt, int32_t* info_dev) {
+  if (!h) return -1;
+  if (!U) return -2;
+  if (N < 0) return -3;
+  if (D < 1 || D > 64) return -4;
+  if (!w) return -5;
+  if (!sf2) return -6;
+  if (tau && S < 1) return -9;
+  if (kind < 0 || kind > 2) return -11;
+  if (d_split < 0 || d_split > D) return -12;
+  if (int r = check_mat(A, ld, N, 13)) return r;
+  if (int r = check_mat(Linv, ldi, N, 15)) return r;
+  if (T) {
+    if (int r = check_mat(T, ldt, N, 17)) return r;
+  }
+  if (!info_dev) return -19;
+  const KyBuild build{U, w, sf2, tau, grp, D, S, kind, d_split, jitter};
+  return potrf_ws_impl(h, A, N, ld, Linv, ldi, T, ldt, info_dev, &build);
+}
+
 int gpp_potrf(gpp_handle_t h, double* A, int64_t N, int64_t ld, double* Linv, int64_t ldi, int32_t* info_dev) {
   const int r = gpp_potrf_ws(h, A, N, ld, Linv, ldi, nullptr, 0, info_dev);
   return r == -9 ? -7 : r;
@@ -1135,6 +1193,35 @@
   g.a_mask = 2; g.b_mask = 2; g.klo_mode = 3; g.c_lower = 1; g.tag = 1;
   const int t = N <= 2560 ? 32 : N <= 5120 ? 64 : NBLK;
   GPP_TRY(gpp_launch_gemm(h->stream, 2, g, 1, t, t));
+  return 0;
+}
+
+int gpp_lauum_grad(gpp_handle_t h, const double* Linv, int64_t N, int64_t ldi, const double* U, int D, const double* w,
+                   const double* sf2, const int32_t* grp, int S, int kind, int dU, const double* alpha, double* g_w,
+                   double* g_sf2, double* g_tau) {
+  if (!h) return -1;
+  if (N < 0) return -3;
+  if (int r = check_mat(Linv, ldi, N, 2)) return r;
+  if (!U) return -5;
+  if (D < 1 || D > 64) return -6;
+  if (!w) return -7;
+  if (!sf2) return -8;
+  if (S < 1 || S > 64) return -10;
+  if (kind < 0 || kind > 2) return -11;
+  if (dU < 0 || dU > D) return -12;
+  if (!alpha) return -13;
+  if (!g_w) return -14;
+  if (!g_sf2) return -15;
+  if (!g_tau) return -16;
+  if (kind != GPP_KIND_RBF || D > 16 || dU != 0) return GPP_NOT_SUPPORTED;
+  if (!h->ws || h->ws_bytes < gpp_lauum_grad_ws_bytes(N, D)) return GPP_NO_WORKSPACE;
+  GemmArgs g = mk(Linv, ldi, Linv, ldi, nullptr, ldi, N, N, N, 1.0, 0.0);
+  g.a_mask = 2; g.b_mask = 2; g.klo_mode = 3; g.c_lower = 1;
+  const int64_t tiles = (N + NBLK - 1) / NBLK, nrec = tiles * (tiles + 1) / 2;
+  double* rec = reinterpret_cast<double*>(h->ws);
+  double* wdiag = rec + nrec * (D + 1);
+  GPP_TRY(gpp_launch_lauum_grad(h->stream, g, GradEpiArgs{U, w, sf2, alpha, rec, wdiag, D}));
+  GPP_TRY(gpp_launch_grad_finish(h->stream, rec, nrec, D, S, wdiag, grp, N, g_w, g_sf2, g_tau));
   return 0;
 }
 
diff --git a/gp-plus_amd/csrc/gpp_build.hip b/gp-plus_amd/csrc/gpp_build.hip
--- a/gp-plus_amd/csrc/gpp_build.hip
+++ b/gp-plus_amd/csrc/gpp_build.hip
@@ -164,6 +164,13 @@
   int64_t nt;
   if (uplo) nt = tr1 * (tr1 + 1) / 2 - tr0 * (tr0 + 1) / 2;
   else nt = (tr1 - tr0) * tiles_n;
+  if (uplo == GPP_UPLO_UPPER && (row0 != 0 || nrows != N)) {
+    if (row0 % TB != 0 || ((row0 + nrows) % TB != 0 && row0 + nrows != N)) return hipErrorInvalidValue;
+    auto* fu = kind == 0 ? gpp_cov_tile<false> : gpp_cov_tile<true>;
+    hipLaunchKernelGGL(fu, dim3((unsigned)nt, (unsigned)batch), dim3(256), (size_t)2 * D * TB * sizeof(double), s, U, N, U, N, D, w, sf2, tau,
+                       grp, jitter, kind, d_split, uplo, 1, Ky, ld, (int64_t)0, tiles_n, tr0, sU, sK, S);
+    return hipGetLastError();
+  }
   auto* fn = kind == 0 ? gpp_cov_tile<false> : gpp_cov_tile<true>;
   hipLaunchKernelGGL(fn, dim3((unsigned)nt, (unsigned)batch), dim3(256), (size_t)2 * D * TB * sizeof(double), s, U, row0 + nrows, U, N, D, w, sf2, tau,
                      grp, jitter, kind, d_split, uplo, 1, Ky, ld, row0, tiles_n, tr0, sU, sK, S);
diff --git a/gp-plus_amd/csrc/gpp_gemm.hip b/gp-plus_amd/csrc/gpp_gemm.hip
--- a/gp-plus_amd/csrc/gpp_gemm.hip
+++ b/gp-plus_amd/csrc/gpp_gemm.hip
@@ -132,10 +132,11 @@
 struct GemmNoHook {
   __device__ __forceinline__ void operator()() const {}
 };
-template <int VAR, int WTM, int WTN, int TAG, int BK, int NBUF, int WR, class P, class H = GemmNoHook>
+struct GemmStoreC {};
+template <int VAR, int WTM, int WTN, int TAG, int BK, int NBUF, int WR, class P, class H = GemmNoHook, class E = GemmStoreC>
 __device__ __forceinline__ void gemm_tile(const P& p, const int tm, const int tn, const double* __restrict__ A,
                                           const double* __restrict__ B, double* __restrict__ C, double* C2,
-                                          double* __restrict__ smem, H before_epilogue = H()) {
+                                          double* __restrict__ smem, H before_epilogue = H(), const E& epi = E()) {
   static_assert(BK == 16 || VAR == 2, "wide K chunks are implemented for row-contiguous (TN) operands only");
   static_assert(BK % 16 == 0 && (NBUF == 1 || NBUF == 2), "bad staging parameters");
   static_assert(WR == 2 || (WR == 4 && VAR == 2 && BK == 16 && NBUF == 2 && WTM == 64 && WTN == 64), "the tall tile is TN only");
@@ -291,9 +292,9 @@
       const int kb = kpos(c + 1);
       load_fast<NVA>(ubaseA + (int64_t)kb * stepA, offa, ra);
       load_fast<NVB>(ubaseB + (int64_t)kb * stepB, offb, rb);
-      if constexpr (TAG == 1) __builtin_amdgcn_s_setprio(1);
+      if constexpr (TAG != 0) __builtin_amdgcn_s_setprio(1);
       compute(cur);
-      if constexpr (TAG == 1) __builtin_amdgcn_s_setprio(0);
+      if constexpr (TAG != 0) __builtin_amdgcn_s_setprio(0);
       if (NBUF == 1) __syncthreads();
       store_mc<TM, BK, false, NTH>(smem + nxt * (OPA + OPB), tid, ra, 0);
       store_mc<TN, BK, false, NTH>(smem + nxt * (OPA + OPB) + OPA, tid, rb, 0);
@@ -302,6 +303,11 @@
   }
   for (; c < nch; ++c) general_iter(c);
   before_epilogue();
+  if constexpr (!__is_same(E, GemmStoreC)) {
+    static_assert(VAR == 2 && WTM == 64 && WTN == 64 && WR == 2, "accumulator epilogues are written for the big TN tile");
+    epi(acc4, row0, col0, p.M, smem);
+    return;
+  }
 
   const double alpha = p.alpha, beta = p.beta;
   constexpr int GA = RB < 4 ? RB : 4;
@@ -400,6 +406,139 @@
 
 }
 
+__device__ __forceinline__ double wave_sum(double v) {
+#pragma unroll
+  for (int o = 32; o > 0; o >>= 1) v += __shfl_xor(v, o);
+  return v;
+}
+template <int DT>
+struct GradEpilogue {
+  GradEpiArgs e;
+  int tile;
+  static constexpr int T = 128;
+  static constexpr int FIXED = 2 * DT * T + 2 * T + DT + 4 * (DT + 1);
+  static constexpr int SLAB = (FIXED + 1) & ~1;
+  static_assert((SLAB + 16 * 256) * sizeof(double) <= 2 * 2 * BK16 * ldt_mc(T) * sizeof(double), "the epilogue lives in the main loop's LDS");
+  __device__ __forceinline__ void operator()(const v4d (&acc4)[4][4], int row0, int col0, int N, double* __restrict__ smem) const {
+    const int tid = threadIdx.x, wave = tid >> 6, lane = tid & 63;
+    const int wm = (wave >> 1) * 64, wn = (wave & 1) * 64, li = lane & 15, lk = lane >> 4;
+    const int D = e.D;
+    double* __restrict__ sa = smem;
+    double* __restrict__ sb = sa + DT * T;
+    double* __restrict__ sal_a = sb + DT * T;
+    double* __restrict__ sal_b = sal_a + T;
+    double* __restrict__ sw = sal_b + T;
+    double* __restrict__ red = sw + DT;
+    double* __restrict__ slab = smem + SLAB;
+    for (int x = tid; x < DT * T; x += 256) {
+      const int d = x / T, r = x - d * T;
+      sa[x] = (d < D && row0 + r < N) ? e.U[(int64_t)(row0 + r) * D + d] : 0.0;
+      sb[x] = (d < D && col0 + r < N) ? e.U[(int64_t)(col0 + r) * D + d] : 0.0;
+    }
+    if (tid < T) {
+      sal_a[tid] = (row0 + tid < N) ? e.alpha[row0 + tid] : 0.0;
+      sal_b[tid] = (col0 + tid < N) ? e.alpha[col0 + tid] : 0.0;
+    }
+    if (tid < DT) sw[tid] = (tid < D) ? e.w[tid] : 0.0;
+    __syncthreads();
+
+    const double sf2 = *e.sf2;
+    const GppExpConsts ec = gpp_exp_consts();
+    const bool diag_tile = (row0 == col0);
+    double my_sf2 = 0.0, my_w[DT];
+#pragma unroll
+    for (int d = 0; d < DT; ++d) my_w[d] = 0.0;
+#pragma unroll
+    for (int a4 = 0; a4 < 4; ++a4) {
+#pragma unroll
+      for (int v = 0; v < 4; ++v)
+#pragma unroll
+        for (int b = 0; b < 4; ++b) slab[(v * 4 + b) * 256 + tid] = acc4[a4][b][v];
+#pragma unroll 1
+      for (int h = 0; h < 2; ++h) {
+        const int ra = wm + 16 * a4 + 8 * h + lk;
+        const int cb = wn + li;
+        double r2[2][4];
+#pragma unroll
+        for (int a = 0; a < 2; ++a)
+#pragma unroll
+          for (int b = 0; b < 4; ++b) r2[a][b] = 0.0;
+#pragma unroll 2
+        for (int d = 0; d < DT; ++d) {
+          const double ua[2] = {sa[d * T + ra], sa[d * T + ra + 4]};
+          const double wd = sw[d];
+#pragma unroll
+          for (int b = 0; b < 4; ++b) {
+            const double ub = sb[d * T + cb + 16 * b];
+#pragma unroll
+            for (int a = 0; a < 2; ++a) {
+              const double df = ua[a] - ub;
+              r2[a][b] = fma(wd * df, df, r2[a][b]);
+            }
+          }
+        }
+        __asm__ volatile("" ::: "memory");
+        double g2[2][4];
+#pragma unroll
+        for (int a = 0; a < 2; ++a) {
+          const int i = row0 + ra + 4 * a;
+          const double al_i = sal_a[ra + 4 * a];
+#pragma unroll
+          for (int b = 0; b < 4; ++b) {
+            const int j = col0 + cb + 16 * b;
+            const bool ok = (i < N) & (j <= i);
+            const double kv = gpp_exp_nonpos(-r2[a][b], ec);
+            const double kin = slab[((2 * h + a) * 4 + b) * 256 + tid];
+            double Wij = 0.5 * (al_i * sal_b[cb + 16 * b] - kin);
+            Wij = ok ? Wij : 0.0;
+            const double mult = (i == j) ? 1.0 : 2.0;
+            my_sf2 = fma(mult * Wij, kv, my_sf2);
+            g2[a][b] = mult * Wij * sf2 * kv;
+            if (diag_tile && ok && i == j) e.wdiag[i] = Wij;
+          }
+        }
+#pragma unroll
+        for (int d = 0; d < DT; ++d) {
+          const double ua[2] = {sa[d * T + ra], sa[d * T + ra + 4]};
+          double s = 0.0;
+#pragma unroll
+          for (int b = 0; b < 4; ++b) {
+            const double ub = sb[d * T + cb + 16 * b];
+#pragma unroll
+            for (int a = 0; a < 2; ++a) {
+              const double df = ua[a] - ub;
+              s = fma(-g2[a][b] * df, df, s);
+            }
+          }
+          my_w[d] += s;
+          __builtin_amdgcn_sched_barrier(0);
+        }
+      }
+    }
+#pragma unroll
+    for (int q = 0; q <= DT; ++q) {
+      const double v = wave_sum(q < DT ? my_w[q < DT ? q : 0] : my_sf2);
+      if (lane == 0) red[wave * (DT + 1) + q] = v;
+    }
+    __syncthreads();
+    if (tid <= D) {
+      const int q = (tid == D) ? DT : tid;
+      e.rec[(int64_t)tile * (D + 1) + tid] = ((red[q] + red[(DT + 1) + q]) + red[2 * (DT + 1) + q]) + red[3 * (DT + 1) + q];
+    }
+  }
+};
+
+template <int DT>
+__global__ __launch_bounds__(256, 2) void gpp_lauum_grad_f64(GemmArgs p, GradEpiArgs e) {
+  extern __shared__ __attribute__((aligned(16))) double smem[];
+  const int t = (int)blockIdx.x;
+  int tm = (int)((sqrtf(8.f * (float)t + 1.f) - 1.f) * 0.5f);
+  while ((tm + 1) * (tm + 2) / 2 <= t) ++tm;
+  while (tm * (tm + 1) / 2 > t) --tm;
+  const int tn = t - tm * (tm + 1) / 2;
+  gemm_tile<2, 64, 64, 2, 16, 2, 2>(p, tm, tn, p.A, p.B, nullptr, nullptr, smem, GemmNoHook(), GradEpilogue<DT>{e, t});
+}
+
 constexpr size_t gemm_lds_bytes(int var, int tm, int tn, int bk, int nbuf) {
   const int tx = tm > tn ? tm : tn;
   const int mc = bk * ldt_mc(tx, bk), kc = tx * LDK;
@@ -660,6 +799,32 @@
   }
 }
 
+hipError_t gpp_launch_lauum_grad(hipStream_t s, const GemmArgs& a_in, const GradEpiArgs& e) {
+  GemmArgs a = a_in;
+  if (a.M <= 0) return hipSuccess;
+  if (a.M != a.N || a.c_lower != 1 || e.D < 1 || e.D > 16) return hipErrorInvalidValue;
+  a.tiles_m = a.tiles_n = (a.M + 127) / 128;
+  a.row_mod = 0;
+  a.swz = 0;
+  a.batch_fast = 0;
+  a.tile_base = 0;
+  const int64_t nt = (int64_t)a.tiles_m * (a.tiles_m + 1) / 2;
+  constexpr size_t bytes = gemm_lds_bytes(2, 128, 128, 16, 2);
+  auto* fn = e.D <= 8 ? gpp_lauum_grad_f64<8> : gpp_lauum_grad_f64<16>;
+  static std::atomic<bool> attr_set[2][64];
+  int dev = 0;
+  hipError_t err = hipGetDevice(&dev);
+  if (err != hipSuccess) return err;
+  const int which = e.D <= 8 ? 0 : 1;
+  if (dev < 0 || dev >= 64 || !attr_set[which][dev]) {
+    err = hipFuncSetAttribute(reinterpret_cast<const void*>(fn), hipFuncAttributeMaxDynamicSharedMemorySize, (int)bytes);
+    if (err != hipSuccess) return err;
+    if (dev >= 0 && dev < 64) attr_set[which][dev] = true;
+  }
+  hipLaunchKernelGGL(fn, dim3((unsigned)nt), dim3(256), bytes, s, a, e);
+  return hipGetLastError();
+}
+
 hipError_t gpp_launch_dag_bind(hipStream_t s, const GemmArgs* rel, GemmArgs* abs, int n, const DagBases& bases) {
   if (n <= 0) return hipSuccess;
   hipLaunchKernelGGL(gpp_dag_bind, dim3((unsigned)((n + 63) / 64)), dim3(64), 0, s, rel, abs, n, bases);
diff --git a/gp-plus_amd/csrc/gpp_internal.h b/gp-plus_amd/csrc/gpp_internal.h
--- a/gp-plus_amd/csrc/gpp_internal.h
+++ b/gp-plus_amd/csrc/gpp_internal.h
@@ -38,6 +38,7 @@
   int32_t* shard_info;
   hipEvent_t shard_ready;
   int dag_sched;
+  int split_builds;
   gpp_comm_t comm;
   int comm_rank, comm_nranks;
   void* rccl_comm;
@@ -138,6 +139,17 @@
 };
 hipError_t gpp_launch_gemm(hipStream_t s, int variant, const GemmArgs& a, int batch, int tile_m = 0, int tile_n = 0);
 
+struct GradEpiArgs {
+  const double* U;
+  const double* w;
+  const double* sf2;
+  const double* alpha;
+  double* rec;
+  double* wdiag;
+  int D;
+};
+hipError_t gpp_launch_lauum_grad(hipStream_t s, const GemmArgs& lauum, const GradEpiArgs& e);
+
 hipError_t gpp_launch_exec_gate(hipStream_t s, int* counters, int id, int target, int32_t* info, long long budget);
 hipError_t gpp_launch_exec_signal(hipStream_t s, int* counters, int id);
 
@@ -246,6 +258,9 @@
                                   double* g_U, void* ws, size_t ws_bytes, int shard_nb = 0, int shard_rank = 0,
                                   int shard_nranks = 1, int batch = 1, int64_t sU = 0, int64_t sK = 0, int64_t sv = 0,
                                   int shard_cols = 0);
+size_t gpp_lauum_grad_ws_bytes(int64_t N, int D);
+hipError_t gpp_launch_grad_finish(hipStream_t s, const double* rec, int64_t nrec, int D, int S, const double* wdiag,
+                                  const int32_t* grp, int64_t N, double* g_w, double* g_sf2, double* g_tau);
 hipError_t gpp_launch_trmv_lower_cols(hipStream_t s, const double* T, int64_t ldt, int64_t N, const double* x, double* y,
                                       int64_t nb, int rank, int nranks, int trans, void* ws, size_t ws_bytes, int compact = 0);
 size_t gpp_trmv_t_ws_bytes(int64_t N);
diff --git a/gp-plus_amd/csrc/gpp_reduce.hip b/gp-plus_amd/csrc/gpp_reduce.hip
--- a/gp-plus_amd/csrc/gpp_reduce.hip
+++ b/gp-plus_amd/csrc/gpp_reduce.hip
@@ -782,6 +782,18 @@
   return hipGetLastError();
 }
 
+size_t gpp_lauum_grad_ws_bytes(int64_t N, int D) {
+  const int64_t T = (N + 127) / 128;
+  return (size_t)(T * (T + 1) / 2) * (D + 1) * sizeof(double) + (size_t)N * sizeof(double) + 256;
+}
+hipError_t gpp_launch_grad_finish(hipStream_t s, const double* rec, int64_t nrec, int D, int S, const double* wdiag,
+                                  const int32_t* grp, int64_t N, double* g_w, double* g_sf2, double* g_tau) {
+  if (nrec < 0 || nrec > INT32_MAX || D < 1 || D > GD_MAX || S < 1 || S > GS_MAX) return hipErrorInvalidValue;
+  hipLaunchKernelGGL(gpp_grad_finish, dim3(D + 1 + S, 1), dim3(256), 0, s, rec, (int)nrec, D, S, wdiag, grp, N, g_w, g_sf2, g_tau,
+                     (int64_t)0);
+  return hipGetLastError();
+}
+
 size_t gpp_pgrad_ws_bytes(int64_t M, int64_t N, int D, int dA, int dB) {
   const PgradShape p = pgrad_shape(M, N);
   const int64_t nwg = p.MT * p.CN;
diff --git a/gp-plus_amd/linalg.py b/gp-plus_amd/linalg.py
--- a/gp-plus_amd/linalg.py
+++ b/gp-plus_amd/linalg.py
@@ -62,6 +62,8 @@
     return getattr(_tls, "slot", 0)
 
 LOOKAHEAD_MIN_N = 3840
+
+FUSED_GRAD_MIN_N = 5120
 
 STAGE_EVENTS = None
 
@@ -116,9 +118,9 @@
         if ws.N >= LOOKAHEAD_MIN_N:
             torch.cuda.current_stream(ctx.index).synchronize()
         with _stage("kernel_build"):
-            ctx.kernel_build(U, w, sf2, tau, grp, ws.A, jitter=jit, kind=kind, d_split=d_split, uplo=UPLO_UPPER)
+            pass
         with _stage("potrf"):
-            ctx.potrf(ws.A, ws.Li, ws.info, ws.Ki)
+            ctx.build_potrf(U, w, sf2, tau, grp, ws.A, ws.Li, ws.info, ws.Ki, jitter=jit, kind=kind, d_split=d_split)
         ws.info_host.copy_(ws.info, non_blocking=True)
         ws.info_event.record(torch.cuda.current_stream(ctx.index))
         if after is not None:
@@ -180,11 +182,16 @@
                 return
             with _stage("alpha"):
                 gctx.alpha(ws.Li, ws.z, ws.alpha)
+            fused = False
             with _stage("lauum"):
-                gctx.lauum(ws.Li, ws.Ki)
+                if N > FUSED_GRAD_MIN_N:
+                    fused = gctx.lauum_grad(ws.Li, Ud, wd, sd, grp, S, ws.alpha, dU if need_U else 0, g_w, g_s, g_t, kind=kind)
+                if not fused:
+                    gctx.lauum(ws.Li, ws.Ki)
             with _stage("grad_reduce"):
-                gctx.grad_reduce(Ud, wd, sd, grp, S, ws.alpha, ws.Ki, dU if need_U else 0, g_w, g_s, g_t, g_Ud, kind=kind,
-                                 d_split=d_split)
+                if not fused:
+                    gctx.grad_reduce(Ud, wd, sd, grp, S, ws.alpha, ws.Ki, dU if need_U else 0, g_w, g_s, g_t, g_Ud, kind=kind,
+                                     d_split=d_split)
 
         _factor(gctx, ws, Ud, wd, sd, td, grp, kind, d_split, after=rest)
         ctx.saved = (g_w, g_s, g_t, g_Ud, ws.alpha.clone() if need_grad else None, (N, D, dU))
diff --git a/include/gpp.h b/include/gpp.h
--- a/include/gpp.h
+++ b/include/gpp.h
@@ -50,9 +50,19 @@
 int gpp_potrf_ws(gpp_handle_t h, double* A, int64_t N, int64_t ld, double* Linv, int64_t ldi, double* T, int64_t ldt,
                  int32_t* info_dev);
 
+int gpp_build_potrf_ws(gpp_handle_t h, const double* U, int64_t N, int D, const double* w, const double* sf2, const double* tau,
+                       const int32_t* grp, int S, double jitter, int kind, int d_split, double* A, int64_t ld, double* Linv,
+                       int64_t ldi, double* T, int64_t ldt, int32_t* info_dev);
+
 int gpp_trtri(gpp_handle_t h, const double* U, int64_t N, int64_t ld, double* Linv, int64_t ldi, double* T, int64_t ldt);
 
 int gpp_lauum(gpp_handle_t h, const double* Linv, int64_t N, int64_t ldi, double* Kinv, int64_t ldk);
+
+#define GPP_NOT_SUPPORTED 2001
+#define GPP_NO_WORKSPACE 2002
+int gpp_lauum_grad(gpp_handle_t h, const double* Linv, int64_t N, int64_t ldi, const double* U, int D, const double* w,
+                   const double* sf2, const int32_t* grp, int S, int kind, int dU, const double* alpha, double* g_w,
+                   double* g_sf2, double* g_tau);
 
 int gpp_post_cov_train(gpp_handle_t h, const double* Kinv, int64_t N, int64_t ldk, const double* tau, const int32_t* grp, int S,
                        const double* d, double jitter, double* A, int64_t lda);
```

Result: faster. 7.960 evals/s, median of 6 (+1.6%).
